# voletiv/mcvd-pytorch

Hardware: AMD Instinct MI355X
Metric: sampled frames/sec (whole node), SMMNIST 64x64 DDPM 100-step (higher is better)
Workload: dtype f32-equivalent: f32 storage and accumulation; 58 of 58 3x3 convs, 41 of 41 1x1 convs and the attention products (head dims 32..128) as SIX bf16 piece products of operands split EXACTLY into three bf16 pieces (all 24 bits, fp32 exponent range, less than one fp32 rounding per product; tests/test_gpu_p

## Files before the change

### include/mcvd_hip.h

```cpp
#ifndef MCVD_HIP_H
#define MCVD_HIP_H

#include <stddef.h>
#include <stdint.h>

#ifdef __cplusplus
extern "C" {
#endif

#define MCVD_OK 0
#define MCVD_EINVAL (-1)
#define MCVD_EHIP (-2)
#define MCVD_ESTATE (-3)
#define MCVD_ENOMEM (-4)
#define MCVD_ERANGE (-5)

#define MCVD_MAX_LEVELS 8

typedef struct mcvd_ctx mcvd_ctx;
typedef struct mcvd_model mcvd_model;

typedef struct mcvd_unet_desc {
    int32_t image_size;
    int32_t channels;
// ... 63 lines not shown
int mcvd_model_set_gamma_tables(mcvd_model* m, const float* k_cum_host, const float* theta_t_host, int n);
int mcvd_model_prepare_cond(mcvd_model* m, const float* cond, int B);
int mcvd_model_invalidate_cond(mcvd_model* m);
int mcvd_model_get_tuning(mcvd_model* m, int B, int* shapes, int* cots, int cap);
int mcvd_model_set_tuning(mcvd_model* m, int B, const int* shapes, const int* cots, int n);
int mcvd_model_graph_stats(mcvd_model* m, int64_t* captures, int64_t* replays);
int mcvd_model_num_launches(mcvd_model* m, int B);

int mcvd_model_profile_read(mcvd_model* m, int* kinds, int* ks, double* ms, double* flops, double* bytes, int cap);

int mcvd_model_op_info(mcvd_model* m, int i, int info[8]);

int mcvd_model_op_kernel(mcvd_model* m, int i);

long mcvd_model_fused_launches(mcvd_model* m, int what);

int mcvd_model_module_output(mcvd_model* m, int module, int B, float* dst_device, int64_t capacity, int* C, int* H);

int mcvd_sampler_run(mcvd_model* m, int kind, float* x_inout, const float* cond, const float* noise, uint64_t seed,
                     uint64_t sample_offset, int subsample_steps, int flags, double t_min, int B);
int mcvd_fpndm_run(mcvd_model* m, float* x_inout, const float* cond, int subsample_steps, int flags, int B);
int mcvd_sampler_update(mcvd_ctx* ctx, int kind, float* x_inout, const float* eps, const float* noise, float c_x0a,
                        float c_x0b, float c_mean0, float c_mean1, float c_noise, int clip, int64_t n);
int mcvd_randn(mcvd_ctx* ctx, float* out, uint64_t seed, uint64_t sample_offset, uint64_t draw, int B,
               int64_t per_sample);
int mcvd_pack_frames_u8(mcvd_ctx* ctx, const float* frames01, uint8_t* out, int B, int T, int C, int H, int W);
#define MCVD_METRIC_ROUND_BINARY 1
int mcvd_frame_metrics(mcvd_ctx* ctx, const float* pred01, const float* real01, int B, int T, int C, int H, int W, int flags, float* mse_out,
                       double* ssim_out, uint8_t* grey_out);
#define MCVD_F32 0
#define MCVD_F64 1
int mcvd_fvd_clips(mcvd_ctx* ctx, const float* const* parts, const int* part_frames, const int64_t* part_batch_stride, int nparts, int B, int C,
                   int H, int W, int row_start, int row_step, float* out);
int mcvd_feature_stats(mcvd_ctx* ctx, const void* feats, int dtype, int64_t N, int d, int64_t ld, int64_t row_start, int64_t row_step,
                       double* mean_out, double* sigma_out);
int mcvd_knn_radii(mcvd_ctx* ctx, const void* feats, int dtype, int64_t N, int d, int64_t ld, int k, double* radii2_out);
int mcvd_manifold_hits(mcvd_ctx* ctx, const void* query, int q_dtype, int64_t Nq, int64_t ldq, const void* ref, int r_dtype, int64_t Nr,
                       int64_t ldr, int d, const double* ref_radii2, uint8_t* hit_out);
int mcvd_knn_search(mcvd_ctx* ctx, const void* query, int q_dtype, int64_t ldq, const void* query2, int q2_dtype, int64_t ldq2, int64_t Nq,
                    const void* ref, int r_dtype, int64_t ldr, int64_t Nr, int d, int k, int64_t index_base, int merge, double* dist2_io,
                    int64_t* index_io);
int mcvd_hflip_u8(mcvd_ctx* ctx, const float* images01, float* out, int64_t n, int C, int H, int W);
int mcvd_nn_collect(mcvd_ctx* ctx, const float* held, const int64_t* held_index, const int64_t* new_index, const float* piece, int64_t n,
                    int64_t index_base, int64_t Nq, int k, int C, int H, int W, float* out);
typedef struct mcvd_lpips mcvd_lpips;
int mcvd_lpips_create(mcvd_ctx* ctx, mcvd_lpips** out);
void mcvd_lpips_destroy(mcvd_lpips* net);
int mcvd_lpips_set_param(mcvd_lpips* net, const char* name, const void* ptr, const int64_t* shape, int ndim, int on_device);
int mcvd_lpips_finalize(mcvd_lpips* net);
int mcvd_lpips_frames(mcvd_lpips* net, const float* pred01, const float* real01, int B, int T, int C, int H, int W, float* lpips_out,
                      uint8_t* resized_out, float* per_tap_out);
typedef struct mcvd_inception mcvd_inception;
int mcvd_inception_create(mcvd_ctx* ctx, mcvd_inception** out);
void mcvd_inception_destroy(mcvd_inception* net);
int mcvd_inception_set_param(mcvd_inception* net, const char* name, const void* ptr, const int64_t* shape, int ndim, int on_device);
int mcvd_inception_finalize(mcvd_inception* net);
int mcvd_inception_chunk(void);
int mcvd_inception_forward(mcvd_inception* net, const float* images01, int64_t n, int H, int W, int resize_input, int normalize_input,
                           int block_mask, float* out0, float* out1, float* out2, float* out3);
#define MCVD_DSM_L1 1
#define MCVD_DSM_GAMMA 2
int mcvd_dsm_loss(mcvd_model* m, const float* x, const int64_t* labels, const float* cond, const int32_t* cond_mask, const float* z,
                  uint64_t seed, uint64_t sample_offset, int flags, float* loss_rows, float* z_out, float* perturbed_out, int B);
int mcvd_gamma_noise(mcvd_ctx* ctx, float* out, const float* raw, float k, float theta, float kt, float sd, uint64_t seed,
                     uint64_t sample_offset, uint64_t draw, int B, int64_t per_sample);
int mcvd_lincomb(mcvd_ctx* ctx, float* out, const float* in0, const float* in1, const float* in2, const float* in3, float w0,
                 float w1, float w2, float w3, float scale, int nin, int64_t n);
int mcvd_pndm_transfer(mcvd_ctx* ctx, float* out, const float* x, const float* e, float d, float c1, float c2, int clip,
                       int64_t n);

int mcvd_upfirdn2d(mcvd_ctx* ctx, const float* in, const float* kernel_host, int kh, int kw, int up, int down, int pad0,
                   int pad1, float* out, int N, int C, int H, int W);
int mcvd_op_conv2d(mcvd_ctx* ctx, const float* x0, int C0, const float* x1, int C1, const float* w, const float* bias,
                   int Cout, int ks, const float* coef, int act, const float* res, float out_scale, float* y, int B, int H,
                   int W);
int mcvd_op_conv2d_strided(mcvd_ctx* ctx, const float* x, const float* w, const float* bias, int B, int Cin, int H, int W, int Cout, int ks,
                           int stride, int pad, int relu, float* y);
int mcvd_op_conv2d_rect(mcvd_ctx* ctx, const float* x, const float* w, const float* alpha, const float* beta, int B, int Cin, int H, int W,
                        int Cout, int kh, int kw, int stride, int pad_h, int pad_w, int relu, float* y, int c0, int Ctot);
int mcvd_op_pool3(mcvd_ctx* ctx, const float* x, float* y, int64_t NC, int H, int W, int mode);
int mcvd_op_global_avg(mcvd_ctx* ctx, const float* x, float* y, int64_t NC, int HW);
int mcvd_op_resize299(mcvd_ctx* ctx, const float* x, int64_t n, int H, int W, int normalize, float* y);
int mcvd_last_conv_kernel(void);
int mcvd_ctx_set_spade_inputs(mcvd_ctx* ctx, const float* gb, const float* coef2);
int mcvd_ctx_set_stats_buffer(mcvd_ctx* ctx, float* device_floats);
int mcvd_last_conv_stats_np(void);
int mcvd_op_gn_finalize(mcvd_ctx* ctx, const float* st0, int C0, int np0, const float* st1, int C1, int np1, int groups, float eps,
                        int mode, const float* p0, const float* p1, int emb_stride, int emb_off, float* coef_out, int B, int HW);
int mcvd_op_gn_coef(mcvd_ctx* ctx, const float* x0, int C0, const float* x1, int C1, int groups, float eps, int mode,
                    const float* p0, const float* p1, int emb_stride, int emb_off, float* coef_out, int B, int HW);
int mcvd_op_attention(mcvd_ctx* ctx, const float* qkv, float* out, int B, int C, int heads, int HW);
int mcvd_op_fir2(mcvd_ctx* ctx, const float* x, const float* coef, int act, int up, float* y, int B, int C, int H, int W);

#ifdef __cplusplus
}
#endif
#endif
```

### mcvd_pytorch_amd/_lib.py

```python
import ctypes as C
import os

import torch

_HERE = os.path.dirname(os.path.abspath(__file__))
LIB_PATH = os.environ.get("MCVD_LIB_PATH") or os.path.join(_HERE, "libmcvd_hip.so")

MAX_LEVELS = 8


class UNetDesc(C.Structure):
    _fields_ = [("image_size", C.c_int32), ("channels", C.c_int32), ("num_frames", C.c_int32),
                ("num_frames_cond", C.c_int32), ("ngf", C.c_int32), ("n_levels", C.c_int32),
                ("ch_mult", C.c_int32 * MAX_LEVELS), ("num_res_blocks", C.c_int32), ("n_attn", C.c_int32),
                ("attn_resolutions", C.c_int32 * MAX_LEVELS), ("n_head_channels", C.c_int32), ("spade", C.c_int32),
                ("spade_dim", C.c_int32), ("num_classes", C.c_int32), ("sigma_dist", C.c_int32),
                ("sigma_begin", C.c_float), ("sigma_end", C.c_float), ("cond_emb", C.c_int32), ("noise_in_cond", C.c_int32),
                ("gamma", C.c_int32)]


SAMPLER_DDPM, SAMPLER_DDIM = 0, 1
FLAG_DENOISE, FLAG_CLIP_BEFORE, FLAG_JUST_BETA, FLAG_GAMMA = 1, 2, 4, 8
METRIC_ROUND_BINARY = 1
DSM_L1, DSM_GAMMA = 1, 2
F32, F64 = 0, 1

_vp, _i, _f, _i64, _u64 = C.c_void_p, C.c_int, C.c_float, C.c_int64, C.c_uint64
_PROTOS = {
    "mcvd_version": (C.c_char_p, []),
    "mcvd_last_error": (C.c_char_p, [_vp]),
    "mcvd_ctx_create": (_i, [_i, _vp, C.POINTER(_vp)]),
    "mcvd_ctx_destroy": (None, [_vp]),
    "mcvd_ctx_device_shared": (_i, [_vp]),
    "mcvd_ctx_set_stream": (_i, [_vp, _vp]),
    "mcvd_ctx_set_option": (_i, [_vp, C.c_char_p, _i]),
    "mcvd_ctx_check_range": (_i, [_vp]),
    "mcvd_ctx_clear_range": (_i, [_vp]),
    "mcvd_ctx_selftest": (_i, [_vp]),
    "mcvd_ctx_set_debug_buffer": (_i, [_vp, _vp]),
    "mcvd_model_create": (_i, [_vp, C.POINTER(UNetDesc), C.POINTER(_vp)]),
    "mcvd_model_destroy": (None, [_vp]),
    "mcvd_model_num_params": (_i, [_vp]),
    "mcvd_model_param_info": (_i, [_vp, _i, C.POINTER(C.c_char_p), C.POINTER(_i64), C.POINTER(_i), C.POINTER(_i64)]),
    "mcvd_model_set_param": (_i, [_vp, C.c_char_p, _vp, C.POINTER(_i64), _i, _i]),
    "mcvd_model_blob_floats": (_i, [_vp, C.POINTER(_i64)]),
    "mcvd_model_export_blob": (_i, [_vp, _vp]),
    "mcvd_model_import_blob": (_i, [_vp, _vp]),
    "mcvd_model_broadcast_params": (_i, [_vp, _vp, _i]),
    "mcvd_model_finalize": (_i, [_vp]),
    "mcvd_model_get_schedule": (_i, [_vp, _vp, _vp, _vp, _i]),
    "mcvd_model_set_schedule": (_i, [_vp, _vp, _vp, _vp, _i]),
    "mcvd_model_set_temb_freqs": (_i, [_vp, _vp, _i]),
    "mcvd_unet_forward": (_i, [_vp, _vp, _vp, _vp, _vp, _i]),
    "mcvd_unet_forward_ft": (_i, [_vp, _vp, _vp, _vp, _vp, _i]),
    "mcvd_unet_forward_masked": (_i, [_vp, _vp, _vp, _vp, _vp, _vp, _i]),
    "mcvd_model_set_cond_noise": (_i, [_vp, _vp, _u64, _u64, _u64]),
    "mcvd_model_set_gamma_tables": (_i, [_vp, _vp, _vp, _i]),
    "mcvd_model_prepare_cond": (_i, [_vp, _vp, _i]),
    "mcvd_model_invalidate_cond": (_i, [_vp]),
    "mcvd_model_num_launches": (_i, [_vp, _i]),
    "mcvd_model_get_tuning": (_i, [_vp, _i, _vp, _vp, _i]),
    "mcvd_model_set_tuning": (_i, [_vp, _i, _vp, _vp, _i]),
    "mcvd_model_graph_stats": (_i, [_vp, C.POINTER(_i64), C.POINTER(_i64)]),
    "mcvd_last_conv_kernel": (_i, []),
    "mcvd_last_conv_stats_np": (_i, []),
    "mcvd_ctx_set_stats_buffer": (_i, [_vp, _vp]),
    "mcvd_ctx_set_spade_inputs": (_i, [_vp, _vp, _vp]),
    "mcvd_op_gn_finalize": (_i, [_vp, _vp, _i, _i, _vp, _i, _i, _i, _f, _i, _vp, _vp, _i, _i, _vp, _i, _i]),
    "mcvd_model_profile_read": (_i, [_vp, _vp, _vp, _vp, _vp, _vp, _i]),
    "mcvd_model_op_info": (_i, [_vp, _i, C.POINTER(_i)]),
    "mcvd_model_op_kernel": (_i, [_vp, _i]),
    "mcvd_model_fused_launches": (C.c_long, [_vp, _i]),
    "mcvd_model_module_output": (_i, [_vp, _i, _i, _vp, _i64, C.POINTER(_i), C.POINTER(_i)]),
    "mcvd_sampler_run": (_i, [_vp, _i, _vp, _vp, _vp, _u64, _u64, _i, _i, C.c_double, _i]),
    "mcvd_fpndm_run": (_i, [_vp, _vp, _vp, _i, _i, _i]),
    "mcvd_sampler_update": (_i, [_vp, _i, _vp, _vp, _vp, _f, _f, _f, _f, _f, _i, _i64]),
    "mcvd_randn": (_i, [_vp, _vp, _u64, _u64, _u64, _i, _i64]),
    "mcvd_pack_frames_u8": (_i, [_vp, _vp, _vp, _i, _i, _i, _i, _i]),
    "mcvd_frame_metrics": (_i, [_vp, _vp, _vp, _i, _i, _i, _i, _i, _i, _vp, _vp, _vp]),
    "mcvd_lpips_create": (_i, [_vp, C.POINTER(_vp)]),
    "mcvd_lpips_destroy": (None, [_vp]),
    "mcvd_lpips_set_param": (_i, [_vp, C.c_char_p, _vp, C.POINTER(_i64), _i, _i]),
    "mcvd_lpips_finalize": (_i, [_vp]),
    "mcvd_lpips_frames": (_i, [_vp, _vp, _vp, _i, _i, _i, _i, _i, _vp, _vp, _vp]),
    "mcvd_inception_create": (_i, [_vp, C.POINTER(_vp)]),
    "mcvd_inception_destroy": (None, [_vp]),
    "mcvd_inception_set_param": (_i, [_vp, C.c_char_p, _vp, C.POINTER(_i64), _i, _i]),
    "mcvd_inception_finalize": (_i, [_vp]),
    "mcvd_inception_chunk": (_i, []),
    "mcvd_inception_forward": (_i, [_vp, _vp, _i64, _i, _i, _i, _i, _i, _vp, _vp, _vp, _vp]),
    "mcvd_op_conv2d_rect": (_i, [_vp, _vp, _vp, _vp, _vp, _i, _i, _i, _i, _i, _i, _i, _i, _i, _i, _i, _vp, _i, _i]),
    "mcvd_op_pool3": (_i, [_vp, _vp, _vp, _i64, _i, _i, _i]),
    "mcvd_op_global_avg": (_i, [_vp, _vp, _vp, _i64, _i]),
    "mcvd_op_resize299": (_i, [_vp, _vp, _i64, _i, _i, _i, _vp]),
    "mcvd_fvd_clips": (_i, [_vp, C.POINTER(_vp), C.POINTER(_i), C.POINTER(_i64), _i, _i, _i, _i, _i, _i, _i, _vp]),
    "mcvd_feature_stats": (_i, [_vp, _vp, _i, _i64, _i, _i64, _i64, _i64, _vp, _vp]),
    "mcvd_knn_radii": (_i, [_vp, _vp, _i, _i64, _i, _i64, _i, _vp]),
    "mcvd_manifold_hits": (_i, [_vp, _vp, _i, _i64, _i64, _vp, _i, _i64, _i64, _i, _vp, _vp]),
    "mcvd_knn_search": (_i, [_vp, _vp, _i, _i64, _vp, _i, _i64, _i64, _vp, _i, _i64, _i64, _i, _i, _i64, _i, _vp, _vp]),
    "mcvd_hflip_u8": (_i, [_vp, _vp, _vp, _i64, _i, _i, _i]),
    "mcvd_nn_collect": (_i, [_vp, _vp, _vp, _vp, _vp, _i64, _i64, _i64, _i, _i, _i, _i, _vp]),
    "mcvd_op_conv2d_strided": (_i, [_vp, _vp, _vp, _vp, _i, _i, _i, _i, _i, _i, _i, _i, _i, _vp]),
    "mcvd_gamma_noise": (_i, [_vp, _vp, _vp, _f, _f, _f, _f, _u64, _u64, _u64, _i, _i64]),
    "mcvd_dsm_loss": (_i, [_vp, _vp, _vp, _vp, _vp, _vp, _u64, _u64, _i, _vp, _vp, _vp, _i]),
    "mcvd_lincomb": (_i, [_vp, _vp, _vp, _vp, _vp, _vp, _f, _f, _f, _f, _f, _i, _i64]),
    "mcvd_pndm_transfer": (_i, [_vp, _vp, _vp, _vp, _f, _f, _f, _i, _i64]),
    "mcvd_upfirdn2d": (_i, [_vp, _vp, _vp, _i, _i, _i, _i, _i, _i, _vp, _i, _i, _i, _i]),
    "mcvd_op_conv2d": (_i, [_vp, _vp, _i, _vp, _i, _vp, _vp, _i, _i, _vp, _i, _vp, _f, _vp, _i, _i, _i]),
    "mcvd_op_gn_coef": (_i, [_vp, _vp, _i, _vp, _i, _i, _f, _i, _vp, _vp, _i, _i, _vp, _i, _i]),
    "mcvd_op_attention": (_i, [_vp, _vp, _vp, _i, _i, _i, _i]),
    "mcvd_op_fir2": (_i, [_vp, _vp, _vp, _i, _i, _vp, _i, _i, _i, _i]),
}

EXPORTS = tuple(_PROTOS.keys())


def _load():
    if not os.path.exists(LIB_PATH):
        raise ImportError(
            f"{LIB_PATH} not found: the HIP extension is not built. Run `python mcvd_pytorch_amd/csrc/build.py` "
            "(needs hipcc; cross-compiles for gfx950 without a GPU). There is no CPU fallback.")
    lib = C.CDLL(LIB_PATH)
    for name, (res, args) in _PROTOS.items():
        fn = getattr(lib, name)
        fn.restype = res
        fn.argtypes = args
    return lib


lib = _load()


def last_error():
    return (lib.mcvd_last_error(None) or b"").decode()


def check(rc, what=""):
    if rc != 0:
        raise RuntimeError(f"libmcvd_hip: {what} failed (code {rc}): {last_error()}")
```

### mcvd_pytorch_amd/csrc/api.cpp

```cpp
#include <dlfcn.h>
#include <errno.h>
#include <fcntl.h>
#include <pthread.h>
#include <math.h>
#include <sys/file.h>
#include <sys/stat.h>
#include <unistd.h>
#include <stdio.h>
#include <stdlib.h>
#include <string.h>

#include <algorithm>
#include <cmath>
#include <mutex>
#include <new>
#include <vector>

#include "model.h"
#include "conv_kernels.h"
#include "inception.h"
#include "lpips.h"

using namespace mcvd;

// ... 263 lines not shown
        unsigned long long* dbg;
        explicit Saved(mcvd_ctx* c_) : c(c_), conv_shape(c_->conv_shape), naive_conv(c_->naive_conv), f16x2(c_->f16x2), f16x1(c_->f16x1), bf16x3(c_->bf16x3),
                                       spade_fuse(c_->spade_fuse), stats_buf(c_->stats_buf), spade_gb(c_->spade_gb), spade_coef2(c_->spade_coef2),
                                       dbg(c_->dbg) {
            c->naive_conv = 0; c->f16x2 = 0; c->f16x1 = 0; c->bf16x3 = 1; c->spade_fuse = 0;
            c->stats_buf = nullptr; c->spade_gb = nullptr; c->spade_coef2 = nullptr; c->dbg = nullptr;
        }
        ~Saved() {
            c->conv_shape = conv_shape; c->naive_conv = naive_conv; c->f16x2 = f16x2; c->f16x1 = f16x1; c->spade_fuse = spade_fuse;
            if (c->wino_selftest >= 0) c->bf16x3 = bf16x3;
            c->stats_buf = stats_buf; c->spade_gb = spade_gb; c->spade_coef2 = spade_coef2; c->dbg = dbg;
        }
    };
    const int shapes[3] = {CK_WINO, CK_WINO3, CK_WINO3P};
    int rc = 0, ran[3] = {-1, -1, -1};
    std::vector<float> out(3 * ny);
    {
        Saved saved(ctx);
        for (int k = 0; k < 3 && rc == 0; ++k) {
            ctx->conv_shape = shapes[k];
            rc = mcvd_op_conv2d(ctx, x, Cin, nullptr, 0, w, bias, Cout, 3, coef, 1, res, 0.70710678f, y + k * ny, B, H, H);
            ran[k] = last_conv_kernel();
        }
    }
    if (rc) return rc;
    MCVD_HIP_CHECK(hipMemcpyAsync(out.data(), y, 3 * ny * sizeof(float), hipMemcpyDeviceToHost, ctx->stream));
    MCVD_HIP_CHECK(hipStreamSynchronize(ctx->stream));
    float scale = 0.0f, d10 = 0.0f;
    size_t diff16 = 0;
    for (size_t i = 0; i < ny; ++i) {
        scale = std::max(scale, std::fabs(out[i]));
        d10 = std::max(d10, std::fabs(out[ny + i] - out[i]));
        diff16 += memcmp(&out[2 * ny + i], &out[ny + i], sizeof(float)) != 0;
    }
    const bool ok = ran[0] == shapes[0] && ran[1] == shapes[1] && ran[2] == shapes[2] && scale > 0.1f && d10 <= 1e-4f * scale && diff16 == 0 && std::isfinite(d10);
    if (ok) { ctx->wino_selftest = 1; return 0; }
    ctx->wino_selftest = -1;
    ctx->bf16x3 = 0;
    ++ctx->epoch;
    set_error("self-test of the hand-scheduled Winograd kernels FAILED on this device (kernels that ran: %d %d %d; |bf16x3 - fp32 MFMA| = %.3e at "
              "scale %.3e; %zu values of the persistent form differ from the per-item form): the option bf16x3 was switched off for this context",
              ran[0], ran[1], ran[2], (double)d10, (double)scale, diff16);
    return MCVD_ESELFTEST;
    API_CATCH
}

int mcvd_ctx_clear_range(mcvd_ctx* ctx) {
    API_TRY
    MCVD_REQUIRE(ctx, "ctx is NULL");
    if (ctx->range_flag) MCVD_HIP_CHECK(hipMemsetAsync(ctx->range_flag, 0, sizeof(int), ctx->stream));
    return 0;
    API_CATCH
}

int mcvd_ctx_set_option(mcvd_ctx* ctx, const char* key, int value) {
    MCVD_REQUIRE(ctx && key, "ctx/key is NULL");
    ++ctx->epoch;
    if (!strcmp(key, "naive_conv")) ctx->naive_conv = value;
    else if (!strcmp(key, "naive_attn")) ctx->naive_attn = value;
    else if (!strcmp(key, "fir_form")) ctx->fir_form = value;
    else if (!strcmp(key, "dbg_skip_finalize")) ctx->dbg_skip_finalize = value;
    else if (!strcmp(key, "gn_producer")) ctx->gn_producer = value;
    else if (!strcmp(key, "graph")) ctx->graph = value;
    else if (!strcmp(key, "conv_shape")) ctx->conv_shape = value;
    else if (!strcmp(key, "conv_shape1")) ctx->conv_shape1 = value;
    else if (!strcmp(key, "profile")) ctx->profile = value;
    else if (!strcmp(key, "conv_wdma")) ctx->conv_wdma = value;
    else if (!strcmp(key, "autotune")) ctx->autotune = value;
    else if (!strcmp(key, "side_stream")) ctx->side_stream = value;
    else if (!strcmp(key, "share_fence")) ctx->share_fence = value;
    else if (!strcmp(key, "winograd")) ctx->winograd = value;
    else if (!strcmp(key, "conv_dma1")) ctx->conv_dma1 = value;
    else if (!strcmp(key, "bf16x3")) ctx->bf16x3 = value;
    else if (!strcmp(key, "f16x2")) {
        if (ctx->f16x2 != value) (void)mcvd_ctx_clear_range(ctx);
        ctx->f16x2 = value;
    }
    else if (!strcmp(key, "f16x1")) {
        if (ctx->f16x1 != value) (void)mcvd_ctx_clear_range(ctx);
        ctx->f16x1 = value;
    }
    else if (!strcmp(key, "conv_cot")) ctx->conv_cot = value;
    else if (!strcmp(key, "persist_grid")) ctx->persist_grid = value;
    else if (!strcmp(key, "temb_table")) ctx->temb_table = value;
    else if (!strcmp(key, "im2col_lds")) ctx->im2col_lds = value;
    else if (!strcmp(key, "gn_stats")) ctx->gn_stats = value;
    else if (!strcmp(key, "spade_fuse")) ctx->spade_fuse = value;
    else if (!strcmp(key, "attn_presplit")) ctx->attn_presplit = value;
    else {
        set_error("unknown option '%s'", key);
        return MCVD_EINVAL;
    }
    return 0;
}

static void default_schedule(mcvd_model* m) {
    const int T = m->d.num_classes;
    m->betas.assign(T, 0.f);
    m->alphas.assign(T, 0.f);
    m->alphas_prev.assign(T, 0.f);
    if (m->d.sigma_dist == 0) {
        const float start = m->d.sigma_begin, end = m->d.sigma_end;
        const float step = (end - start) / (float)(T - 1);
        for (int i = 0; i < T; ++i) m->betas[i] = (i < T / 2) ? start + step * (float)i : end - step * (float)(T - 1 - i);
        float p = 1.0f;
        for (int i = T - 1; i >= 0; --i) {
            p = p * (1.0f - m->betas[i]);
            m->alphas[i] = p;
        }
        for (int i = 0; i < T; ++i) m->alphas_prev[i] = (i + 1 < T) ? m->alphas[i + 1] : 1.0f;
    } else {
        std::vector<float> f(T + 1);
        const float s = 0.008f;
        for (int i = 0; i <= T; ++i) {
            const float t = (float)(T - i) / (float)T;
            const float c = cosf((t + s) / (1.0f + s) * (float)(M_PI / 2));
            f[i] = c * c;
        }
        for (int i = 0; i < T; ++i) m->alphas[i] = f[i] / f[T];
        for (int i = 0; i < T; ++i) m->alphas_prev[i] = (i + 1 < T) ? m->alphas[i + 1] : 1.0f;
        for (int i = 0; i < T; ++i) m->betas[i] = 1.0f - m->alphas[i] / m->alphas_prev[i];
    }
    const int half = m->d.ngf / 2;
    m->freqs.assign(half, 0.f);
    const float e = (float)(-(log(10000.0) / (double)(half - 1)));
    for (int k = 0; k < half; ++k) m->freqs[k] = expf((float)k * e);
}

int mcvd_model_create(mcvd_ctx* ctx, const mcvd_unet_desc* desc, mcvd_model** out) {
    API_TRY
    MCVD_REQUIRE(desc && out, "model_create: NULL argument");
    MCVD_REQUIRE(desc->sigma_dist == 0 || desc->sigma_dist == 1, "desc: sigma_dist=%d", desc->sigma_dist);
    mcvd_model* m = new mcvd_model();
    m->ctx = ctx;
    m->d = *desc;
    if (m->build_plan()) {
        delete m;
        return MCVD_EINVAL;
    }
    default_schedule(m);
    if (ctx) {
        hipError_t e = hipMalloc((void**)&m->blob, (size_t)m->blob_floats * sizeof(float));
        if (e != hipSuccess) {
            set_error("hipMalloc(param blob, %lld floats): %s", (long long)m->blob_floats, hipGetErrorString(e));
            delete m;
            return MCVD_EHIP;
        }
        MCVD_HIP_CHECK(hipMemsetAsync(m->blob, 0, (size_t)m->blob_floats * sizeof(float), ctx->stream));
    }
    *out = m;
    return 0;
    API_CATCH
}

void mcvd_model_destroy(mcvd_model* m) {
    if (!m) return;
    if (m->ctx) (void)hipStreamSynchronize(m->ctx->stream);
    m->drop_graph();
    if (m->blob) (void)hipFree(m->blob);
    if (m->packed) (void)hipFree(m->packed);
    if (m->packed_h) (void)hipFree(m->packed_h);
    if (m->coef2_desc_dev) (void)hipFree(m->coef2_desc_dev);
    if (m->arena) (void)hipFree(m->arena);
    if (m->labels) (void)hipFree(m->labels);
    if (m->eps_buf) (void)hipFree(m->eps_buf);
    if (m->ksplit_buf) (void)hipFree(m->ksplit_buf);
// ... 898 lines not shown
    if (gam) {
        if (!m->gamma_dev) MCVD_HIP_CHECK(hipMalloc((void**)&m->gamma_dev, (size_t)2 * T * sizeof(float)));
        if (!m->gamma_dev_valid) {
            MCVD_HIP_CHECK(hipMemcpyAsync(m->gamma_dev, m->k_cum.data(), (size_t)T * sizeof(float), hipMemcpyHostToDevice, s));
            MCVD_HIP_CHECK(hipMemcpyAsync(m->gamma_dev + T, m->theta_t.data(), (size_t)T * sizeof(float), hipMemcpyHostToDevice, s));
            m->gamma_dev_valid = true;
        }
    }
    if (int rc = launch_dsm_perturb(x, z, labels, m->alphas_dev, gam ? m->gamma_dev : nullptr, gam ? m->gamma_dev + T : nullptr, T,
                                    gam ? 1 : 0, seed, sample_offset, B, per, zb, pb, s))
        return rc;
    struct MaskGuard { mcvd_model* m; ~MaskGuard() { m->cond_mask = nullptr; } } mask_guard{m};
    m->cond_mask = cond_mask;
    if (int rc = m->forward(pb, labels, cond, m->eps_buf, B)) return rc;
    if (int rc = launch_dsm_loss(zb, m->eps_buf, B, per, (flags & MCVD_DSM_L1) ? 1 : 0, part, loss_rows, s)) return rc;
    return (m->ctx->f16x2 || m->ctx->f16x1) ? mcvd_ctx_check_range(m->ctx) : 0;
    API_CATCH
}

int mcvd_gamma_noise(mcvd_ctx* ctx, float* out, const float* raw, float k, float theta, float kt, float sd, uint64_t seed,
                     uint64_t sample_offset, uint64_t draw, int B, int64_t per_sample) {
    MCVD_REQUIRE(ctx && out, "gamma_noise: NULL argument");
    return launch_gamma_noise(out, raw, k, theta, kt, sd, seed, sample_offset, draw, B, per_sample, ctx->stream);
}

int mcvd_randn(mcvd_ctx* ctx, float* out, uint64_t seed, uint64_t sample_offset, uint64_t draw, int B, int64_t per_sample) {
    MCVD_REQUIRE(ctx && out, "randn: NULL argument");
    return launch_randn(out, seed, sample_offset, draw, B, per_sample, ctx->stream);
}

int mcvd_upfirdn2d(mcvd_ctx* ctx, const float* in, const float* kernel_host, int kh, int kw, int up, int down, int pad0,
                   int pad1, float* out, int N, int C, int H, int W) {
    API_TRY
    MCVD_REQUIRE(ctx && in && kernel_host && out, "upfirdn2d: NULL argument");
    MCVD_REQUIRE(up >= 1 && down >= 1 && kh >= 1 && kw >= 1, "upfirdn2d: up/down/kernel");
    const int oh = (H * up + pad0 + pad1 - kh) / down + 1, ow = (W * up + pad0 + pad1 - kw) / down + 1;
    MCVD_REQUIRE(oh > 0 && ow > 0, "upfirdn2d: empty output");
    if (int rc = ctx->ensure_scratch((size_t)kh * kw * sizeof(float))) return rc;
    MCVD_HIP_CHECK(hipMemcpyAsync(ctx->scratch, kernel_host, (size_t)kh * kw * sizeof(float), hipMemcpyHostToDevice, ctx->stream));
    MCVD_HIP_CHECK(hipStreamSynchronize(ctx->stream));
    return launch_upfirdn2d(in, ctx->scratch, kh, kw, up, down, pad0, pad1, out, N * C, H, W, oh, ow, ctx->stream);
    API_CATCH
}

int mcvd_op_conv2d(mcvd_ctx* ctx, const float* x0, int C0, const float* x1, int C1, const float* w, const float* bias,
                   int Cout, int ks, const float* coef, int act, const float* res, float out_scale, float* y, int B, int H,
                   int W) {
    API_TRY
    MCVD_REQUIRE(ctx && x0 && w && bias && y, "op_conv2d: NULL argument");
    MCVD_REQUIRE(ks == 1 || ks == 3, "op_conv2d: ks=%d", ks);
    ConvArgs a{};
    a.x0 = x0; a.x1 = x1; a.C0 = C0; a.C1 = x1 ? C1 : 0;
    a.coef = coef; a.act = act; a.res = res; a.out_scale = out_scale; a.y = y;
    a.B = B; a.Cin = a.C0 + a.C1; a.Cout = Cout; a.H = H; a.W = W; a.ks = ks;
    a.cot = conv_cout_tile(Cout);
    a.CinP = round_up(a.Cin, conv_chunk(ks));
    a.CoutP = round_up(Cout, 32 * a.cot);
    const size_t wfloats = (size_t)a.CinP * ks * ks * a.CoutP;
    const ConvKernelDesc& k = conv_kernel(ctx->conv_shape);
    const bool wino = is_winograd(k.id) && conv_wino_supported(ks, H, W);
    const bool wino_h = wino && k.weights == CW_WPH;
    const bool wino_b = wino && k.weights == CW_WPB;
    const int np1 = (ks == 1 && k.family == CF_SPLIT1) ? k.pieces : 0;
    const size_t ufloats = wino ? (size_t)a.CinP * 16 * a.CoutP : 0;
    const size_t hfloats = wino_h ? (size_t)((conv_wino2h_weight_floats(a.CinP, a.CoutP) + 3) / 4 * 4)
                           : wino_b ? (size_t)((conv_wino3_weight_floats(a.CinP, a.CoutP) + 3) / 4 * 4)
                           : np1 ? (size_t)((conv1x1_h2_weight_floats(a.CinP, a.CoutP, np1) + 3) / 4 * 4) : 0;
    const size_t pfloats = wino ? (size_t)k.kparts * B * Cout * H * W : 0;
    if (int rc = ctx->ensure_scratch((wfloats + a.CoutP + ufloats + hfloats + pfloats) * sizeof(float))) return rc;
    MCVD_HIP_CHECK(hipMemsetAsync(ctx->scratch, 0, (wfloats + a.CoutP + ufloats + hfloats) * sizeof(float), ctx->stream));
    if (wino) {
        if (int rc = launch_pack_wino_weight(w, ctx->scratch + wfloats + a.CoutP, Cout, a.Cin, a.CinP, a.CoutP, ctx->stream)) return rc;
        a.wpw = ctx->scratch + wfloats + a.CoutP;
        if (wino_h) {
            if (int rc = launch_pack_wino2h_weight(w, ctx->scratch + wfloats + a.CoutP + ufloats, Cout, a.Cin, a.CinP, a.CoutP, ctx->stream)) return rc;
            a.wph = ctx->scratch + wfloats + a.CoutP + ufloats;
        }
        if (wino_b) {
            if (int rc = launch_pack_wino3_weight(w, ctx->scratch + wfloats + a.CoutP + ufloats, Cout, a.Cin, a.CinP, a.CoutP, ctx->stream)) return rc;
            a.wpb = ctx->scratch + wfloats + a.CoutP + ufloats;
        }
        if (pfloats) { a.part = ctx->scratch + wfloats + a.CoutP + ufloats + hfloats; a.part_floats = pfloats; }
    }
    if (int rc = launch_pack_conv_weight(w, ctx->scratch, Cout, a.Cin, ks, a.CinP, a.CoutP, 0, 0, ctx->stream)) return rc;
    if (np1) {
        if (int rc = launch_pack_conv1x1_h2(ctx->scratch, ctx->scratch + wfloats + a.CoutP, a.CinP, a.CoutP, ctx->stream, np1)) return rc;
        (np1 == 2 ? a.wph : a.wpb) = ctx->scratch + wfloats + a.CoutP;
    }
    MCVD_HIP_CHECK(hipMemcpyAsync(ctx->scratch + wfloats, bias, (size_t)Cout * sizeof(float), hipMemcpyDeviceToDevice, ctx->stream));
    a.wp = ctx->scratch;
    a.bias = ctx->scratch + wfloats;
    a.shape_hint = ctx->conv_shape;
    if (k.own_cot && ctx->conv_cot > 0) a.cot = ctx->conv_cot;
    a.wdma = ctx->conv_wdma;
    a.pgrid = ctx->persist_grid;
    a.dbg = ctx->dbg;
    a.stats = ctx->naive_conv ? nullptr : ctx->stats_buf;
    if (ctx->spade_gb) {
        MCVD_REQUIRE(wino && !ctx->naive_conv && coef && act, "op_conv2d: the SPADE prologue exists in the Winograd kernel only (conv_shape 4 / 8, "
                     "3x3, coef and act given)");
        a.gb = ctx->spade_gb;
        a.coef2 = ctx->spade_coef2;
        ConvArgs t = a;
        t.ksplit = k.family == CF_WINO ? k.kparts : 0;
        MCVD_REQUIRE(conv_wino_usable(t) || (t.ksplit = 0, conv_wino_usable(t)), "op_conv2d: shape not served by the Winograd kernel");
    }
    return ctx->naive_conv ? launch_conv_naive(a, ctx->stream) : launch_conv_mfma(a, ctx->stream);
    API_CATCH
}

int mcvd_last_conv_kernel(void) { return last_conv_kernel(); }

int mcvd_last_conv_stats_np(void) { return last_conv_stats_np(); }

int mcvd_op_gn_finalize(mcvd_ctx* ctx, const float* st0, int C0, int np0, const float* st1, int C1, int np1, int groups, float eps,
                        int mode, const float* p0, const float* p1, int emb_stride, int emb_off, float* coef_out, int B, int HW) {
    MCVD_REQUIRE(ctx && st0 && coef_out, "op_gn_finalize: NULL argument");
    GnArgs a{};
    a.C0 = C0; a.C1 = st1 ? C1 : 0; a.groups = groups; a.eps = eps; a.mode = mode; a.p0 = p0; a.p1 = p1;
    a.emb_stride = emb_stride; a.emb_off = emb_off; a.coef = coef_out; a.B = B; a.HW = HW;
    return launch_gn_finalize(a, st0, np0, st1, np1, ctx->stream);
}

int mcvd_model_graph_stats(mcvd_model* m, int64_t* captures, int64_t* replays) {
    MCVD_REQUIRE(m, "graph_stats: NULL model");
    if (captures) *captures = m->graph_captures;
    if (replays) *replays = m->graph_replays;
    return 0;
}

int mcvd_op_gn_coef(mcvd_ctx* ctx, const float* x0, int C0, const float* x1, int C1, int groups, float eps, int mode,
                    const float* p0, const float* p1, int emb_stride, int emb_off, float* coef_out, int B, int HW) {
    MCVD_REQUIRE(ctx && x0 && coef_out, "op_gn_coef: NULL argument");
    GnArgs a{};
    a.x0 = x0; a.x1 = x1; a.C0 = C0; a.C1 = x1 ? C1 : 0; a.groups = groups; a.eps = eps; a.mode = mode; a.p0 = p0; a.p1 = p1;
    a.emb_stride = emb_stride; a.emb_off = emb_off; a.coef = coef_out; a.B = B; a.HW = HW;
    return launch_gn_coef(a, ctx->stream);
}

int mcvd_op_attention(mcvd_ctx* ctx, const float* qkv, float* out, int B, int C, int heads, int HW) {
    MCVD_REQUIRE(ctx && qkv && out, "op_attention: NULL argument");
    const bool shared = ctx->share_fence && mcvd_ctx_shares_device(ctx);
    return launch_attention(ctx->naive_attn, shared ? 0 : ctx->f16x2, shared ? 0 : ctx->bf16x3, qkv, out, B, C, heads, HW, ctx->stream);
}

int mcvd_op_fir2(mcvd_ctx* ctx, const float* x, const float* coef, int act, int up, float* y, int B, int C, int H, int W) {
    MCVD_REQUIRE(ctx && x && y, "op_fir2: NULL argument");
    return launch_fir2(x, coef, act, up, y, B, C, H, W, nullptr, nullptr, nullptr, nullptr, ctx->stream, ctx->fir_form);
}

}
```

### mcvd_pytorch_amd/csrc/common.h

```cpp
#pragma once
#include <hip/hip_runtime.h>
#include <stdint.h>
#include <atomic>
#include <string>


namespace mcvd {

__device__ __forceinline__ float fma_unpacked(float x, float a, float b) {
    float r;
    asm("v_fma_f32 %0, %1, %2, %3" : "=v"(r) : "v"(x), "v"(a), "v"(b));
    return r;
}

void set_error(const char* fmt, ...);
const char* get_error();

#define MCVD_HIP_CHECK(expr)                                                                  \
    do {                                                                                      \
        hipError_t _e = (expr);                                                               \
        if (_e != hipSuccess) {                                                               \
            mcvd::set_error("%s failed: %s (%s:%d)", #expr, hipGetErrorString(_e), __FILE__, __LINE__); \
            return -2;                                                                        \
        }                                                                                     \
    } while (0)

#define MCVD_REQUIRE(cond, ...)            \
    do {                                   \
        if (!(cond)) {                     \
            mcvd::set_error(__VA_ARGS__);  \
            return -1;                     \
        }                                  \
    } while (0)

struct PerDeviceOnce {
    std::atomic<unsigned long long> mask{0};
    bool first_use() {
        int dev = 0;
        if (hipGetDevice(&dev) != hipSuccess || dev < 0 || dev >= 64) return true;
        const unsigned long long bit = 1ull << dev;
        return (mask.load(std::memory_order_acquire) & bit) == 0;
    }
    void done() {
        int dev = 0;
        if (hipGetDevice(&dev) == hipSuccess && dev >= 0 && dev < 64) mask.fetch_or(1ull << dev, std::memory_order_release);
    }
};

static inline int ceil_div(int a, int b) { return (a + b - 1) / b; }
static inline int round_up(int a, int b) { return ceil_div(a, b) * b; }

struct GnOut {
    float* coef;
    int groups;
    float eps;
    int mode;
    const float* p0;
    const float* p1;
    int emb_stride, emb_off;
};

struct ConvArgs {
    const float* x0;
    const float* x1;
    int C0, C1;
    const float* coef;
    int act;
    const float* wp;
    const float* wpw;
    const float* wph;
    const float* wpb;
    const float* bias;
    const float* res;
    float out_scale;
    float* y;
    int B, Cin, CinP, Cout, CoutP, H, W;
    int ks;
    int cot;
    int shape_hint;
    int ksplit;
    float* part;
    size_t part_floats;
    int wdma;
    int pgrid;
    unsigned long long* dbg;
    float* stats;
    const float* gb;
    const float* coef2;
    float* kv_img;
    int kv_C, kv_D;
    int im2col;
    GnOut gno;
};
int last_conv_gn_fused();
void set_last_conv_gn_fused(int v);
inline bool conv_part_fits(const ConvArgs& a) {
    return a.part != nullptr && (size_t)(a.ksplit < 2 ? 2 : a.ksplit) * a.B * a.Cout * a.H * a.W <= a.part_floats;
}
bool ksplit_reduce_gn_usable(const ConvArgs& a);
int launch_ksplit_reduce_gn(const ConvArgs& a, hipStream_t s);
bool conv1x1_h2_kv_supported(const ConvArgs& a, int cot);
void set_last_conv_stats_np(int np);
int last_conv_stats_np();
int conv_cout_tile(int Cout);
int conv_chunk(int ks);
int launch_conv_mfma(const ConvArgs& a, hipStream_t s);
int launch_conv_naive(const ConvArgs& a, hipStream_t s);
int last_conv_kernel();
bool conv_kernel_usable(int id, const ConvArgs& a);
int conv_kernel_launch(int id, const ConvArgs& a, hipStream_t s);
int launch_im2col3x3(const float* x0, int C0, const float* x1, int C1, float* col, int B, int H, int W, int K, hipStream_t s);
int launch_taps_shift_add(const float* z, const float* bias, const float* res, float scale, float* y, int B, int Cout, int H, int W, hipStream_t s);
int launch_pack_conv_gemm_form(const float* w, float* wp, int Cout, int Cin, int form, int CoutP, hipStream_t s);
bool conv_wino_supported(int ks, int H, int W);
int conv_wino_cout_tile(int Cout);
bool conv_wino_usable(const ConvArgs& a);
int launch_conv_wino(const ConvArgs& a, hipStream_t s);
int launch_wino_ksplit_reduce(const ConvArgs& a, hipStream_t s);
bool conv_wino3_usable(const ConvArgs& a);
int launch_conv_wino3(const ConvArgs& a, hipStream_t s);
long conv_wino3_weight_floats(int CinP, int CoutP);
bool conv_wino3p_usable(const ConvArgs& a);
int launch_conv_wino3p(const ConvArgs& a, hipStream_t s);
int launch_pack_wino3_weight(const float* w, float* wb, int Cout, int Cin, int CinP, int CoutP, hipStream_t s);
bool conv_wino2h_usable(const ConvArgs& a);
int launch_conv_wino2h(const ConvArgs& a, hipStream_t s);
long conv_wino2h_weight_floats(int CinP, int CoutP);
int launch_pack_wino2h_weight(const float* w, float* wh, int Cout, int Cin, int CinP, int CoutP, hipStream_t s);
bool conv_wino1h_usable(const ConvArgs& a);
int launch_conv_wino1h(const ConvArgs& a, hipStream_t s);
bool conv1x1_h2_supported(const ConvArgs& a, int cot, int np);
int launch_conv1x1_h2(const ConvArgs& a, int cot, hipStream_t s, int np);
long conv1x1_h2_weight_floats(int CinP, int CoutP, int np);
int launch_pack_conv1x1_h2(const float* wp, float* wh, int CinP, int CoutP, hipStream_t s, int np);
bool conv1x1_dma_supported(const ConvArgs& a, int ck, int pxw = 1);
int conv1x1_dma_cout_tile(int CoutP);
int launch_conv1x1_dma(const ConvArgs& a, int cot_req, int ck, hipStream_t s, int pxw = 1);
int launch_pack_wino_weight(const float* w, float* up, int Cout, int Cin, int CinP, int CoutP, hipStream_t s);
int launch_pack_conv_weight(const float* w, float* wp, int Cout, int Cin, int ks, int CinP, int CoutP, int nin,
                            int cout_off, hipStream_t s);

struct GnArgs {
    const float* x0;
    const float* x1;
    int C0, C1;
    int groups;
    float eps;
    int mode;
    const float* p0;
    const float* p1;
    int emb_stride, emb_off;
    float* coef;
    int B, HW;
};
int launch_gn_coef(const GnArgs& a, hipStream_t s);
int launch_gn_finalize(const GnArgs& a, const float* st0, int np0, const float* st1, int np1, hipStream_t s);

bool attention_mfma_supported(int C, int heads, int HW);
int launch_attention_mfma(const float* qkv, float* out, int B, int C, int heads, int HW, hipStream_t s);
int launch_attention_naive(const float* qkv, float* out, int B, int C, int heads, int HW, hipStream_t s);
bool attention_h2_supported(int C, int heads, int HW);
int launch_attention_h2(const float* qkv, float* out, int B, int C, int heads, int HW, hipStream_t s, int np);
bool attn_h2p_supported(int C, int heads, int HW);
int launch_attention_h2p(const float* qkv, const float* kv_img, float* out, int B, int C, int heads, int HW, hipStream_t s);
int launch_attention(int mode, int f16x2, int bf16x3, const float* qkv, float* out, int B, int C, int heads, int HW, hipStream_t s);

int launch_fir2(const float* x, const float* coef, int act, int up, float* y, int B, int C, int H, int W,
// ... 62 lines not shown
```

### mcvd_pytorch_amd/csrc/kernels/conv_wino3.cpp

```cpp
#include <stdlib.h>

#include "../common.h"

namespace mcvd {

typedef float f32x16 __attribute__((ext_vector_type(16)));
typedef float f32x4 __attribute__((ext_vector_type(4)));
typedef float f32x2 __attribute__((ext_vector_type(2)));
typedef __bf16 bf16x2 __attribute__((ext_vector_type(2)));
typedef unsigned u32x4 __attribute__((ext_vector_type(4)));

__device__ __forceinline__ float silu_w3(float v) { return v * __builtin_amdgcn_rcpf(1.0f + __expf(-v)); }

constexpr int W3_CK = 16;
constexpr int W3_T = 32;
constexpr int W3_NT = 512;
#ifndef MCVD_W3_PP
#define MCVD_W3_PP 24
#endif
constexpr int W3_PP = MCVD_W3_PP;
constexpr int W3_PW = 16 * 2 * 4 * W3_T;
constexpr int W3_VW = 3 * W3_PW;

__device__ __forceinline__ unsigned w3_cvt_pk(float lo, float hi) {
    const f32x2 v = {lo, hi};
    return __builtin_bit_cast(unsigned, __builtin_convertvector(v, bf16x2));
}
__device__ __forceinline__ void w3_split3(f32x2 v, unsigned& w1, unsigned& w2, unsigned& w3) {
    w1 = w3_cvt_pk(v.x, v.y);
    const f32x2 h = {__builtin_bit_cast(float, w1 << 16), __builtin_bit_cast(float, w1 & 0xffff0000u)};
    v = v - h;
    w2 = w3_cvt_pk(v.x, v.y);
    const f32x2 g = {__builtin_bit_cast(float, w2 << 16), __builtin_bit_cast(float, w2 & 0xffff0000u)};
    v = v - g;
    w3 = w3_cvt_pk(v.x, v.y);
}

template <int COT, int PRO, bool G8, int EXP = 0>
__global__ __launch_bounds__(512) __attribute__((amdgpu_num_vgpr(86))) void conv_wino3_kernel(ConvArgs a) {
    constexpr int NT = W3_NT, CK = W3_CK, T = W3_T, BCO = 32 * COT, PP = W3_PP, VW = W3_VW, PW = W3_PW;
    constexpr int PSZ = CK * 10 * PP;
    constexpr int PBUF = PSZ + 8;
    constexpr int NPL = G8 ? 1 : 3;
    constexpr int NPV = G8 ? 4 : 9;
    constexpr int NQ = 3 * COT;
    constexpr int NA = 2 * NQ;
    constexpr int VM_A = NQ + NPL;
    constexpr int PQ = 5;
    static_assert(NA <= 18 && NA > PQ, "named-register map below: v172-v180 patch, v184-v255 eighteen weight quads");
    extern __shared__ __attribute__((aligned(16))) float smem[];
    unsigned* sV = reinterpret_cast<unsigned*>(smem);
    float* sP = smem + 2 * VW;
    float* sCo = sP + 2 * PBUF;
    unsigned* sOff = reinterpret_cast<unsigned*>(sCo + (G8 ? 4 : 2) * a.Cin);

    {
        float top;
        asm volatile("" : "={v255}"(top));
    }
    asm volatile("" :: "s"(a.x0), "s"(a.x1), "s"(a.coef), "s"(a.wpb), "s"(a.B), "s"(a.H), "s"(a.W), "s"(a.Cin), "s"(a.CinP), "s"(a.C0),
                 "s"(a.C1), "s"(a.CoutP), "s"(a.ksplit), "s"(a.dbg), "s"(a.wdma));
    const unsigned long long t_start = a.dbg ? __builtin_amdgcn_s_memtime() : 0ull;
    const int tid = threadIdx.x, lane = tid & 63, wave = tid >> 6, l31 = lane & 31, half = lane >> 5;
    const int H = a.H, W = a.W, HW = H * W, Cin = a.Cin;
    const int rx_n = G8 ? 1 : W >> 4, ry_n = G8 ? 1 : H >> 3;
    const int nreg = G8 ? (a.B + 1) >> 1 : a.B * rx_n * ry_n;
    const int nct = a.CoutP / BCO;
    const int xcd = blockIdx.x & 7, slot = blockIdx.x >> 3;
    const int reg_id = (slot / nct) * 8 + xcd;
    const int cotile = slot - (slot / nct) * nct;
    if (reg_id >= nreg) return;
    const int b = G8 ? 2 * reg_id : reg_id / (rx_n * ry_n);
    const int rr = G8 ? 0 : reg_id - b * (rx_n * ry_n);
    const int oy0 = (rr / rx_n) * 8, ox0 = (rr % rx_n) * 16;
    const int co0 = cotile * BCO;
    const int rg = __builtin_amdgcn_readfirstlane(wave >> 2);

    const float* co_src[G8 ? 4 : 2];
#pragma unroll
    for (int k = 0; k < 2; ++k) {
        co_src[k] = a.coef + ((long)b * Cin + min(tid + k * NT, Cin - 1)) * 2;
        if (G8) co_src[2 + k] = a.coef + ((long)min(b + 1, a.B - 1) * Cin + min(tid + k * NT, Cin - 1)) * 2;
    }
    if (PRO) {
        asm volatile("global_load_dwordx2 v[172:173], %0, off\n\tglobal_load_dwordx2 v[174:175], %1, off"
                     :: "v"(co_src[0]), "v"(co_src[1]) : "memory");
        if constexpr (G8)
            asm volatile("global_load_dwordx2 v[176:177], %0, off\n\tglobal_load_dwordx2 v[178:179], %1, off"
                         :: "v"(co_src[2]), "v"(co_src[3]) : "memory");
    }

    const int s_tile = tid & 31, s_cp = (tid & 255) >> 5;
    const int s_ty = G8 ? (s_tile >> 2) & 3 : s_tile >> 3, s_tx = G8 ? (s_tile & 3) + 5 * (s_tile >> 4) : s_tile & 7;
    const int p_rd = ((s_cp * 10 + 2 * s_ty + rg) * PP + 2 * s_tx) * 2;
    const int v_wr = ((8 * rg * 2 + (s_cp & 1)) * 4 + (s_cp >> 1)) * T + s_tile;

    unsigned p_pk[NPL];
#pragma unroll
    for (int sl = 0; sl < NPL; ++sl) {
        p_pk[sl] = (unsigned)PSZ | ((unsigned)CK << 12);
        unsigned off = 0;
        if (G8) {
            const int e = tid, ci = e >> 5, img = (e >> 4) & 1, r = (e >> 1) & 7, c = (e & 1) * 4;
            const bool valid = b + img < a.B;
            const int cp = (ci >> 2) * 2 + (ci & 1), ce = (ci >> 1) & 1;
            p_pk[sl] = (unsigned)(((cp * 10 + r + 1) * PP + img * 10 + c + 1) * 2 + ce) | ((unsigned)(ci + (valid ? 0 : CK)) << 12) |
                       ((unsigned)(valid ? img : 0) << 20);
            off = (unsigned)(ci * HW + r * 8 + c) * 4u;
        } else if (sl < 2) {
            const int e = sl * NT + tid;
            if (e < CK * 40) {
                const int ci = e / 40, rem = e - ci * 40, r = rem >> 2, c = (rem & 3) * 4;
                const int y = oy0 - 1 + r;
                const bool inside = y >= 0 && y < H;
                const int cp = (ci >> 2) * 2 + (ci & 1), ce = (ci >> 1) & 1;
                p_pk[sl] = (unsigned)(((cp * 10 + r) * PP + c + 1) * 2 + ce) | ((unsigned)(ci + (inside ? 0 : CK)) << 12);
                off = (unsigned)(ci * HW + min(max(y, 0), H - 1) * W + ox0 + c) * 4u;
            }
        } else if (tid < CK * 20) {
            const int e = tid, ci = e / 20, rem = e - ci * 20, r = rem >> 1, c = (rem & 1) * 17;
            const int y = oy0 - 1 + r, x = ox0 - 1 + c;
            const bool inside = y >= 0 && y < H && x >= 0 && x < W;
            const int cp = (ci >> 2) * 2 + (ci & 1), ce = (ci >> 1) & 1;
            p_pk[sl] = (unsigned)(((cp * 10 + r) * PP + c) * 2 + ce) | ((unsigned)(ci + (inside ? 0 : CK)) << 12);
            off = (unsigned)(ci * HW + min(max(y, 0), H - 1) * W + min(max(x, 0), W - 1)) * 4u;
        }
        sOff[sl * NT + tid] = off;
    }

    const int wave_u = __builtin_amdgcn_readfirstlane(wave);
    const unsigned* wr_base = reinterpret_cast<const unsigned*>(a.wpb) + ((long)cotile * (a.CinP / CK) * 16 + 2 * wave_u) * (NQ * 256);
    const unsigned wr_voff = (unsigned)lane * 16u;

#define W3_QUADS(X, q, A1, A2) X(0, "v[184:187]", q, A1, A2) X(1, "v[188:191]", q, A1, A2) X(2, "v[192:195]", q, A1, A2) X(3, "v[196:199]", q, A1, A2) X(4, "v[200:203]", q, A1, A2) X(5, "v[204:207]", q, A1, A2) X(6, "v[208:211]", q, A1, A2) X(7, "v[212:215]", q, A1, A2) X(8, "v[216:219]", q, A1, A2) X(9, "v[220:223]", q, A1, A2) X(10, "v[224:227]", q, A1, A2) X(11, "v[228:231]", q, A1, A2) X(12, "v[232:235]", q, A1, A2) X(13, "v[236:239]", q, A1, A2) X(14, "v[240:243]", q, A1, A2) X(15, "v[244:247]", q, A1, A2) X(16, "v[248:251]", q, A1, A2) X(17, "v[252:255]", q, A1, A2)
#define W3_LD1(K, R, q, P, UNUSED) if ((q) == K) asm volatile("global_load_dwordx4 " R ", %0, %1" :: "v"(wr_voff), "s"(P) : "memory");
#define W3_MF1(K, R, q, ACC, BV) if ((q) == K) asm volatile("v_mfma_f32_32x32x16_bf16 %0, " R ", %1, %0" : "+v"(ACC) : "v"(BV));
#define W3_LOAD_A(ch, i)                                                                                        \
    {                                                                                                           \
        const unsigned* ua = wr_base + (long)(ch) * (16 * NQ * 256) + (i) * (NQ * 256);                         \
        _Pragma("unroll") for (int qq = 0; qq < NQ; ++qq) { W3_QUADS(W3_LD1, (i) * NQ + qq, ua + qq * 256, 0) } \
    }
                \
#define W3_LOAD_A_PIECE(ch, i, pc)                                                                              \
    {                                                                                                           \
        const unsigned* ua = wr_base + (long)(ch) * (16 * NQ * 256) + (i) * (NQ * 256);                         \
        _Pragma("unroll") for (int ct = 0; ct < COT; ++ct) { W3_QUADS(W3_LD1, (i) * NQ + ct * 3 + (pc), ua + (ct * 3 + (pc)) * 256, 0) } \
    }
#define W3_LD1D(K, R, q, P, DEP) if ((q) == K) asm volatile("global_load_dwordx4 " R ", %0, %1" :: "v"(wr_voff), "s"(P), "v"(DEP) : "memory");
#define W3_LOAD_A_RANGE(ch, Q0, Q1, DEP)                                                                        \
    {                                                                                                           \
        const unsigned* ua = wr_base + (long)(ch) * (16 * NQ * 256);                                            \
        _Pragma("unroll") for (int qq = (Q0); qq < (Q1); ++qq) { W3_QUADS(W3_LD1D, qq, ua + qq * 256, DEP) }    \
    }
#define W3_WAIT(N) asm volatile("s_waitcnt vmcnt(%1)\n\ts_mov_b32 %0, 0" : "=s"(vtok) : "n"(N) : "memory");
#define W3_READ_OFF(OFS) { _Pragma("unroll") for (int sl = 0; sl < NPL; ++sl) OFS[sl] = sOff[sl * NT + tid]; }
#define W3_LOAD_P(ch, DEP, OFS) W3_LOAD_PR(ch, DEP, OFS, "v[172:175]", "v[176:179]", "v180")
#define W3_LOAD_PR(ch, DEP, OFS, RA, RB, RH)                                                                    \
    {                                                                                                           \
        const int cb = min((ch) * CK, Cin - 1);                                                                 \
        const unsigned lim4 = (unsigned)((Cin - cb) * HW - 4) * 4u, lim1 = (unsigned)((Cin - cb) * HW - 1) * 4u; \
        const bool second = cb >= a.C0;                                                                         \
        const float* srcb = second ? a.x1 + ((long)b * a.C1 + (cb - a.C0)) * HW : a.x0 + ((long)b * a.C0 + cb) * HW; \
        const unsigned istride = (unsigned)((second ? a.C1 : a.C0) * HW) * 4u;       \
         \
        if constexpr (G8) {                                                                                     \
            const unsigned o0 = min(OFS[0], lim4) + ((p_pk[0] >> 20) & 1u) * istride;                           \
            asm volatile("global_load_dwordx4 " RA ", %0, %1" :: "v"(o0), "s"(srcb), "v"(DEP) : "memory");     \
        } else {                                                                                                \
            const unsigned o0 = min(OFS[0], lim4), o1 = min(OFS[NPL > 1 ? 1 : 0], lim4), o2 = min(OFS[NPL > 2 ? 2 : 0], lim1); \
            asm volatile("global_load_dwordx4 " RA ", %0, %3\n\tglobal_load_dwordx4 " RB ", %1, %3\n\tglobal_load_dword " RH ", %2, %3" \
                         :: "v"(o0), "v"(o1), "v"(o2), "s"(srcb), "v"(DEP) : "memory");                           \
        }                                                                                                       \
    }
                                                                    \
#define W3_READ_C(ch, cfv)                                                                                      \
    {                                                                                                           \
        _Pragma("unroll") for (int sl = 0; sl < NPL; ++sl) {                                                    \
            cfv[sl] = f32x2{1.0f, 0.0f};                                                                        \
            if (PRO >= 1) {                                                                                     \
                const int cch = min((ch) * CK + (int)((p_pk[sl] >> 12) & (CK - 1)), Cin - 1) + (G8 ? (int)((p_pk[sl] >> 20) & 1u) * Cin : 0); \
                cfv[sl] = *reinterpret_cast<const f32x2*>(sCo + cch * 2);                                       \
            }                                                                                                   \
        }                                                                                                       \
    }
#define W3_NOHOOK(e, v)
#define W3_WRITE_P(ch, PV, cfv) W3_WRITE_PR(ch, PV, cfv, "v172", "v173", "v174", "v175", "v176", "v177", "v178", "v179", "v180", W3_NOHOOK)
     \
#define W3_WRITE_PR(ch, PV, cfv, A0, A1, A2, A3, B0, B1, B2, B3, H0, HOOK)                                      \
    {                                                                                                           \
        float* sPw = sP + (((ch) & 1) ? PBUF : 0);                                                              \
        const int nvalid = Cin - (ch) * CK;                                                                     \
         \
        if constexpr (G8) {                                                                                     \
            asm("v_fma_f32 %0, " A0 ", %4, %5\n\tv_fma_f32 %1, " A1 ", %4, %5\n\tv_fma_f32 %2, " A2 ", %4, %5\n\tv_fma_f32 %3, " A3 ", %4, %5" \
                : "=&v"(PV[0]), "=&v"(PV[1]), "=&v"(PV[2]), "=&v"(PV[3]) : "v"(cfv[0].x), "v"(cfv[0].y), "s"(vtok)); \
        } else {                                                                                                \
            asm("v_fma_f32 %0, " A0 ", %9, %10\n\tv_fma_f32 %1, " A1 ", %9, %10\n\tv_fma_f32 %2, " A2 ", %9, %10\n\tv_fma_f32 %3, " A3 ", %9, %10\n\t" \
                "v_fma_f32 %4, " B0 ", %11, %12\n\tv_fma_f32 %5, " B1 ", %11, %12\n\tv_fma_f32 %6, " B2 ", %11, %12\n\tv_fma_f32 %7, " B3 ", %11, %12\n\t" \
                "v_fma_f32 %8, " H0 ", %13, %14"                                                                  \
                : "=&v"(PV[0]), "=&v"(PV[1]), "=&v"(PV[2]), "=&v"(PV[3]), "=&v"(PV[4]), "=&v"(PV[5]), "=&v"(PV[6]), "=&v"(PV[7]), "=&v"(PV[NPV > 8 ? 8 : 0]) \
                : "v"(cfv[0].x), "v"(cfv[0].y), "v"(cfv[NPL > 1 ? 1 : 0].x), "v"(cfv[NPL > 1 ? 1 : 0].y), "v"(cfv[NPL > 2 ? 2 : 0].x), \
                  "v"(cfv[NPL > 2 ? 2 : 0].y), "s"(vtok));                                                        \
        }                                                                                                       \
        _Pragma("unroll") for (int e = 0; e < NPV; ++e) {                                                       \
            const int sl = e >> 2;                               \
            float v = PV[e];                                                                                    \
            if (PRO >= 2) v = silu_w3(v);                                                                       \
            sPw[(p_pk[sl] & 0xfff) + 2 * (e & 3)] = ((int)((p_pk[sl] >> 12) & 0xff) < min(nvalid, CK)) ? v : 0.0f; \
            HOOK(e, v)                                                                                          \
        }                                                                                                       \
    }
          \
#define W3_READ_R(ch, RW)                                                                                       \
    {                                                                                                           \
        const f32x2* sPr = reinterpret_cast<const f32x2*>(sP + (((ch) & 1) ? PBUF : 0) + p_rd);                 \
        _Pragma("unroll") for (int j = 0; j < 4; ++j) { RW[0][j] = sPr[j]; RW[1][j] = sPr[PP + j]; RW[2][j] = sPr[2 * PP + j]; } \
    }
#define W3_WRITE_V(ch, RG, RW)                                                                                  \
    {                                                                                                           \
// ... 5 lines not shown
            else { mx[j] = r1 - r0; my[j] = r0 - r2; }                                                          \
        }                                                                                                       \
        _Pragma("unroll") for (int row = 0; row < 2; ++row) {                                                   \
            const f32x2 m0 = row ? my[0] : mx[0], m1 = row ? my[1] : mx[1], m2 = row ? my[2] : mx[2], m3 = row ? my[3] : mx[3]; \
            const f32x2 v0 = m0 - m2, v1 = m1 + m2, v2 = m2 - m1, v3 = m1 - m3;                                 \
            _Pragma("unroll") for (int q = 0; q < 4; ++q) {                                                     \
                unsigned w1, w2, w3;                                                                            \
                w3_split3(q == 0 ? v0 : q == 1 ? v1 : q == 2 ? v2 : v3, w1, w2, w3);                            \
                vdst[(row * 4 + q) * 256] = w1;                                                                 \
                vdst[(row * 4 + q) * 256 + PW] = w2;                                                            \
                vdst[(row * 4 + q) * 256 + 2 * PW] = w3;                                                        \
            }                                                                                                   \
        }                                                                                                       \
    }
#define W3_LOAD_B(i, BQ)                                                                                        \
    {                                                                                                           \
        const unsigned* q = sVc + (((2 * wave + (i)) * 2 + half) * 4) * T + l31;                                \
        _Pragma("unroll") for (int jp = 0; jp < 4; ++jp) {                                                      \
            BQ[0][jp] = q[jp * T]; BQ[1][jp] = q[PW + jp * T]; BQ[2][jp] = q[2 * PW + jp * T];                  \
        }                                                                                                       \
    }
#define W3_PRODUCT(i, PA, PB)                                                                                   \
    { _Pragma("unroll") for (int ct = 0; ct < COT; ++ct) { W3_QUADS(W3_MF1, 3 * ((i) * COT + ct) + (PA), acc[i][ct], bq[i][PB]) } }
          \
#define W3_MFMA_PHASE(ch, NEXT)                                                                                 \
    {                                                                                                           \
        const unsigned* sVc = sV + (((ch) & 1) ? VW : 0);                                                       \
        u32x4 bq[2][3];                                                                                         \
        W3_TS(7)                                                                                                \
        if (!(EXP & 8)) { W3_LOAD_B(0, bq[0]) W3_LOAD_B(1, bq[1]) }                                             \
        else { _Pragma("unroll") for (int p = 0; p < 3; ++p) { bq[0][p] = u32x4{1, 2, 3, 4}; bq[1][p] = u32x4{5, 6, 7, 8}; } } \
        _Pragma("unroll") for (int i = 0; i < 2; ++i) {                                                         \
            if (NEXT && !(EXP & 4)) W3_WAIT(VM_A)                                                               \
            if (!(EXP & 16)) {                                                                                  \
                 \
                W3_PRODUCT(i, 2, 0)                                                                             \
                if (NEXT && !(EXP & 4)) W3_LOAD_A_PIECE((ch) + 1, i, 2)                                         \
                W3_PRODUCT(i, 1, 1) W3_PRODUCT(i, 0, 2) W3_PRODUCT(i, 1, 0)                                     \
                if (NEXT && !(EXP & 4)) W3_LOAD_A_PIECE((ch) + 1, i, 1)                                         \
                W3_PRODUCT(i, 0, 1) W3_PRODUCT(i, 0, 0)                                                         \
                if (NEXT && !(EXP & 4)) W3_LOAD_A_PIECE((ch) + 1, i, 0)                                         \
            } else {                                                                                            \
                _Pragma("unroll") for (int ct = 0; ct < COT; ++ct)                                              \
                    acc[i][ct][0] += __builtin_bit_cast(float, bq[i][0][0] ^ bq[i][1][1] ^ bq[i][2][2] ^ bq[i][1][3]); \
                if (NEXT && !(EXP & 4)) W3_LOAD_A((ch) + 1, i)                                                  \
            }                                                                                                   \
            W3_TS(4 + i)                                                                                        \
        }                                                                                                       \
    }
                                                                                         \
#define W3_VALU_PHASE(ch, RG)                                                                                   \
    {                                                                                                           \
        {                                                                                                       \
            f32x2 cfv[NPL];                                                                                     \
            unsigned ofs[NPL];                                                                                  \
            W3_TS(7)                                                                                            \
            if (!(EXP & 2)) W3_READ_C((ch) + 2, cfv)                                                            \
            if (!(EXP & 4)) W3_READ_OFF(ofs)                                                                    \
            if (!(EXP & 4)) W3_WAIT(NA)                                                                         \
            W3_TS(0)                                                                                            \
            float pv[NPV];                                                                                      \
            _Pragma("unroll") for (int e = 0; e < NPV; ++e) pv[e] = 0.0f;                                       \
            if (!(EXP & 2)) W3_WRITE_P((ch) + 2, pv, cfv)                                                       \
            W3_TS(1)                                                                                            \
            if (!(EXP & 4)) W3_LOAD_P((ch) + 3, pv[0], ofs)                                                     \
            W3_TS(2)                                                                                            \
        }                                                                                                       \
        if (!(EXP & 1)) {                                                                                       \
            f32x2 rw[3][4];                                                                                     \
            W3_READ_R((ch) + 1, rw)                                                                             \
            W3_WRITE_V((ch) + 1, RG, rw)                                                                        \
        }                                                                                                       \
        W3_TS(3)                                                                                                \
    }

    f32x16 acc[2][COT];
#pragma unroll
    for (int i = 0; i < 2; ++i)
#pragma unroll
        for (int ct = 0; ct < COT; ++ct)
#pragma unroll
            for (int r = 0; r < 16; ++r) acc[i][ct][r] = 0.0f;

    const bool rec = a.dbg != nullptr && wave == (a.wdma & 7);
    const bool sub = (a.wdma & 64) != 0;
    unsigned long long sp[5] = {0, 0, 0, 0, 0};
    unsigned long long tk0 = 0, tprev = 0, dt[2] = {0, 0}, rt0 = 0;
    if (rec) {
        rt0 = __builtin_amdgcn_s_memrealtime();
        tk0 = tprev = t_start;
    }
#define W3_STAMP(i)                                                                                             \
    if (rec) {                                                                                                  \
        const unsigned long long now = __builtin_amdgcn_s_memtime();                                            \
        dt[i] += now - tprev;                                                                                   \
        tprev = now;                                                                                            \
    }
#ifdef MCVD_DIAG
    const bool tsub = rec && (a.wdma & 128) != 0;
    unsigned long long ts[8] = {0, 0, 0, 0, 0, 0, 0, 0}, tsp = 0;
#define W3_TS(i)                                                                                                \
    if (tsub) {                                                                                                 \
        const unsigned long long now = __builtin_amdgcn_s_memtime();                                            \
        ts[i] += now - tsp;                                                                                     \
        tsp = now;                                                                                              \
    }
#else
#define W3_TS(i)
#endif

    const int nch_all = a.CinP / CK;
    const int ksp = a.ksplit >= 2 ? a.ksplit : 1, kh = ksp >= 2 ? (int)blockIdx.y : 0;
    const int c_begin = kh * (nch_all / ksp), c_end = c_begin + nch_all / ksp;

    int vtok = 0;
    {
        const float nodep = 0.0f;
        unsigned ofs[NPL];
        W3_READ_OFF(ofs)
        if (rec) sp[3] = __builtin_amdgcn_s_memtime() - tk0;
        W3_LOAD_PR(c_begin, nodep, ofs, "v[184:187]", "v[188:191]", "v192")
        W3_LOAD_PR(c_begin + 1, nodep, ofs, "v[194:197]", "v[198:201]", "v202")
        if (G8)
            for (int i = tid; i < 2 * PBUF; i += NT) sP[i] = 0.0f;
        if (rec) sp[0] = __builtin_amdgcn_s_memtime() - tk0;
        W3_WAIT(0)
        if (rec) sp[1] = __builtin_amdgcn_s_memtime() - tk0;
        float cdep = 0.0f;
        if (PRO) {
            f32x2 cpre[G8 ? 4 : 2];
            asm volatile("v_mov_b32 %0, v172\n\tv_mov_b32 %1, v173\n\tv_mov_b32 %2, v174\n\tv_mov_b32 %3, v175"
                         : "=v"(cpre[0].x), "=v"(cpre[0].y), "=v"(cpre[1].x), "=v"(cpre[1].y) : "s"(vtok));
            if constexpr (G8)
                asm volatile("v_mov_b32 %0, v176\n\tv_mov_b32 %1, v177\n\tv_mov_b32 %2, v178\n\tv_mov_b32 %3, v179"
                             : "=v"(cpre[2].x), "=v"(cpre[2].y), "=v"(cpre[3].x), "=v"(cpre[3].y) : "s"(vtok));
#pragma unroll
            for (int k = 0; k < 2; ++k)
                if (tid + k * NT < Cin) {
                    *reinterpret_cast<f32x2*>(sCo + (tid + k * NT) * 2) = cpre[k];
                    if constexpr (G8) *reinterpret_cast<f32x2*>(sCo + (Cin + tid + k * NT) * 2) = cpre[2 + k];
                }
            cdep = cpre[0].x + cpre[1].x + (G8 ? cpre[2].x + cpre[3].x : 0.0f);
        }
        W3_LOAD_P(c_begin + 2, cdep, ofs)
        if (PRO || G8) __syncthreads();
        if (rec) sp[4] = __builtin_amdgcn_s_memtime() - tk0;
        {
            constexpr int QR = (NA - PQ + 2 * NPV - 1) / (2 * NPV);
#define W3_HOOK0(e, v) W3_LOAD_A_RANGE(c_begin, PQ + (e) * QR, (PQ + ((e) + 1) * QR < NA ? PQ + ((e) + 1) * QR : NA), v)
#define W3_HOOK1(e, v) W3_LOAD_A_RANGE(c_begin, (PQ + (NPV + (e)) * QR < NA ? PQ + (NPV + (e)) * QR : NA), (PQ + (NPV + (e) + 1) * QR < NA ? PQ + (NPV + (e) + 1) * QR : NA), v)
            float pv0[NPV], pv1[NPV];
            f32x2 cf0[NPL], cf1[NPL];
            W3_READ_C(c_begin, cf0)
            W3_READ_C(c_begin + 1, cf1)
            W3_WRITE_PR(c_begin, pv0, cf0, "v184", "v185", "v186", "v187", "v188", "v189", "v190", "v191", "v192", W3_HOOK0)
            W3_WRITE_PR(c_begin + 1, pv1, cf1, "v194", "v195", "v196", "v197", "v198", "v199", "v200", "v201", "v202", W3_HOOK1)
#undef W3_HOOK0
#undef W3_HOOK1
            const float dep = pv0[0] + pv1[0];
            W3_LOAD_A_RANGE(c_begin, 0, PQ, dep)
        }
    }
    __syncthreads();
    if (rec) sp[2] = __builtin_amdgcn_s_memtime() - tk0;
    {
        f32x2 rw[3][4];
        W3_READ_R(c_begin, rw)
        W3_WRITE_V(c_begin, rg, rw)
    }
    __syncthreads();
    W3_STAMP(0)

    W3_WAIT(0)
    const int ph = rg;
    if (ph == 0) {
        for (int c = c_begin; c + 1 < c_end; ++c) {
            W3_VALU_PHASE(c, rg)
            W3_MFMA_PHASE(c, true)
            asm volatile("s_waitcnt lgkmcnt(0)\n\ts_barrier" ::: "memory");
            W3_TS(6)
        }
    } else {
        for (int c = c_begin; c + 1 < c_end; ++c) {
            W3_MFMA_PHASE(c, true)
            W3_VALU_PHASE(c, rg)
            asm volatile("s_waitcnt lgkmcnt(0)\n\ts_barrier" ::: "memory");
            W3_TS(6)
        }
    }
    W3_WAIT(0)
    {
        const int c = c_end - 1;
        W3_MFMA_PHASE(c, false)
    }
    asm volatile("s_waitcnt vmcnt(0)" ::: "memory");
    if constexpr (COT == 3)
        asm volatile("s_nop 15\n\ts_nop 15" : "+v"(acc[0][0]), "+v"(acc[0][1]), "+v"(acc[0][2]), "+v"(acc[1][0]), "+v"(acc[1][1]), "+v"(acc[1][2]) :: "memory");
    else if constexpr (COT == 2)
        asm volatile("s_nop 15\n\ts_nop 15" : "+v"(acc[0][0]), "+v"(acc[0][1]), "+v"(acc[1][0]), "+v"(acc[1][1]) :: "memory");
    else
        asm volatile("s_nop 15\n\ts_nop 15" : "+v"(acc[0][0]), "+v"(acc[1][0]) :: "memory");

    float* sM = smem;
    const int e_tile = tid & 31, e_col0 = tid >> 5;
    const int e_ty = G8 ? (e_tile >> 2) & 3 : e_tile >> 3, e_tx = G8 ? e_tile & 3 : e_tile & 7;
    const int e_b = min(b + (G8 ? e_tile >> 4 : 0), a.B - 1);
    const bool e_valid = !G8 || b + (e_tile >> 4) < a.B;
    const long pix = (long)(oy0 + 2 * e_ty) * W + ox0 + 2 * e_tx;
    const bool fin = ksp == 1;
    float* const ydst = fin ? a.y : a.part + (long)kh * a.B * a.Cout * HW;
    float e_bias[COT][2];
    f32x2 e_r0[COT][2], e_r1[COT][2];
#pragma unroll
    for (int ct = 0; ct < COT; ++ct)
#pragma unroll
        for (int t2 = 0; t2 < 2; ++t2) {
            const int co = co0 + ct * 32 + e_col0 + 16 * t2;
            e_bias[ct][t2] = fin ? a.bias[co] : 0.0f;
            e_r0[ct][t2] = e_r1[ct][t2] = f32x2{0.0f, 0.0f};
            if (a.res && fin) {
                const long o = ((long)e_b * a.Cout + min(co, a.Cout - 1)) * HW + pix;
                e_r0[ct][t2] = *reinterpret_cast<const f32x2*>(a.res + o);
                e_r1[ct][t2] = *reinterpret_cast<const f32x2*>(a.res + o + W);
            }
        }
    asm volatile("s_waitcnt lgkmcnt(0)\n\ts_barrier" ::: "memory");
    W3_STAMP(1)
#pragma unroll
    for (int ct = 0; ct < COT; ++ct) {
#pragma unroll
        for (int i = 0; i < 2; ++i)
#pragma unroll
            for (int r = 0; r < 16; ++r) {
                const int col = (r & 3) + 8 * (r >> 2) + 4 * half;
                sM[((2 * wave + i) * 32 + col) * T + l31] = acc[i][ct][r];
            }
        asm volatile("s_waitcnt lgkmcnt(0)\n\ts_barrier" ::: "memory");
#pragma unroll
        for (int t2 = 0; t2 < 2; ++t2) {
            const int e_col = e_col0 + 16 * t2;
            const int co = co0 + ct * 32 + e_col;
            const f32x2 r0 = e_r0[ct][t2], r1 = e_r1[ct][t2];
            float mm[16];
#pragma unroll
            for (int xi = 0; xi < 16; ++xi) mm[xi] = sM[(xi * 32 + e_col) * T + e_tile];
            float t0[4], t1[4];
#pragma unroll
            for (int l = 0; l < 4; ++l) {
                t0[l] = mm[0 * 4 + l] + mm[1 * 4 + l] + mm[2 * 4 + l];
                t1[l] = mm[1 * 4 + l] - mm[2 * 4 + l] - mm[3 * 4 + l];
            }
            const float y00 = t0[0] + t0[1] + t0[2], y01 = t0[1] - t0[2] - t0[3];
            const float y10 = t1[0] + t1[1] + t1[2], y11 = t1[1] - t1[2] - t1[3];
            const float bvv = e_bias[ct][t2];
            const float osc = fin ? a.out_scale : 1.0f;
            const float v00 = (y00 + bvv + r0.x) * osc, v01 = (y01 + bvv + r0.y) * osc;
            const float v10 = (y10 + bvv + r1.x) * osc, v11 = (y11 + bvv + r1.y) * osc;
            if (co < a.Cout && e_valid) {
                const long o = ((long)e_b * a.Cout + co) * HW + pix;
                *reinterpret_cast<float2*>(ydst + o) = make_float2(v00, v01);
                *reinterpret_cast<float2*>(ydst + o + W) = make_float2(v10, v11);
            }
            if (a.stats && fin) {
                float pil;
                {
                    const int pv = __builtin_bit_cast(int, v00);
                    const int s0 = __builtin_amdgcn_readlane(pv, 0), s2 = __builtin_amdgcn_readlane(pv, 32);
                    if (G8) {
                        const int s1 = __builtin_amdgcn_readlane(pv, 16), s3 = __builtin_amdgcn_readlane(pv, 48);
                        pil = __builtin_bit_cast(float, (lane & 32) ? ((lane & 16) ? s3 : s2) : ((lane & 16) ? s1 : s0));
                    } else {
                        pil = __builtin_bit_cast(float, (lane & 32) ? s2 : s0);
                    }
                }
                const float d0 = v00 - pil, d1 = v01 - pil, d2 = v10 - pil, d3 = v11 - pil;
                float sm = (d0 + d1) + (d2 + d3);
                float qm = (d0 * d0 + d1 * d1) + (d2 * d2 + d3 * d3);
#define W3_MERGE(CTRL, ROWMASK)                                                                                     \
                {                                                                                                   \
                    sm += __builtin_bit_cast(float, __builtin_amdgcn_update_dpp(0, __builtin_bit_cast(int, sm), CTRL, ROWMASK, 0xf, false)); \
                    qm += __builtin_bit_cast(float, __builtin_amdgcn_update_dpp(0, __builtin_bit_cast(int, qm), CTRL, ROWMASK, 0xf, false)); \
                }
                W3_MERGE(0xB1, 0xf)
                W3_MERGE(0x4E, 0xf)
                W3_MERGE(0x124, 0xf)
                W3_MERGE(0x128, 0xf)
                if (!G8) W3_MERGE(0x142, 0xa)
#undef W3_MERGE
                const bool writer = G8 ? (e_tile & 15) == 0 : e_tile == 31;
                if (writer && co < a.Cout && e_valid) {
                    constexpr float NPIX = G8 ? 64.0f : 128.0f;
                    float* q = a.stats + (((long)e_b * a.Cout + co) * (rx_n * ry_n) + rr) * 2;
                    q[0] = sm + NPIX * pil;
                    q[1] = fmaxf(qm - sm * sm * (1.0f / NPIX), 0.0f);
                }
            }
        }
        if (ct + 1 < COT) asm volatile("s_waitcnt lgkmcnt(0)\n\ts_barrier" ::: "memory");
    }
    if (rec) {
        const unsigned long long now = __builtin_amdgcn_s_memtime();
        if (lane == 0) {
            unsigned long long* d = a.dbg + ((long)blockIdx.y * gridDim.x + blockIdx.x) * 8;
            unsigned hwid, xcc;
            asm volatile("s_getreg_b32 %0, hwreg(HW_REG_HW_ID)" : "=s"(hwid));
            asm volatile("s_getreg_b32 %0, hwreg(HW_REG_XCC_ID)" : "=s"(xcc));
            d[0] = dt[0]; d[1] = dt[1]; d[2] = rt0; d[3] = __builtin_amdgcn_s_memrealtime();
            d[4] = ((unsigned long long)xcc << 32) | hwid;
            d[5] = now - tprev;
            d[6] = (unsigned long long)(c_end - c_begin);
            d[7] = now - tk0;
            if (sub) { d[1] = sp[3]; d[2] = sp[0]; d[3] = sp[1]; d[4] = sp[4]; d[5] = sp[2]; }
#ifdef MCVD_DIAG
            if (tsub) { d[0] = ts[0]; d[1] = ts[1]; d[2] = ts[2]; d[3] = ts[3]; d[4] = ts[4]; d[5] = ts[5]; d[7] = ts[6]; }
#endif
        }
    }
#undef W3_STAMP
#undef W3_TS
#undef W3_LOAD_A
#undef W3_LOAD_A_PIECE
#undef W3_QUADS
#undef W3_LD1
#undef W3_MF1
#undef W3_PRODUCT
#undef W3_LOAD_P
#undef W3_LOAD_PR
#undef W3_WRITE_PR
#undef W3_LD1D
#undef W3_LOAD_A_RANGE
#undef W3_WAIT
#undef W3_WRITE_P
#undef W3_WRITE_V
#undef W3_READ_R
#undef W3_READ_C
#undef W3_READ_OFF
#undef W3_LOAD_B
#undef W3_MFMA_PHASE
#undef W3_VALU_PHASE
}

static size_t wino3_lds_bytes(int Cin, bool g8) {
    return (size_t)(2 * W3_VW + 2 * (W3_CK * 10 * W3_PP + 8) + (g8 ? 4 : 2) * Cin + (g8 ? 1 : 3) * W3_NT) * sizeof(float);
}

int launch_wino_ksplit_reduce(const ConvArgs& a, hipStream_t s);

template <int COT, int PRO, bool G8, int EXP>
static int wino3_launch_k(const ConvArgs& k, dim3 grid, size_t lds, hipStream_t s) {
    static PerDeviceOnce raised;
    if (raised.first_use()) {
        MCVD_HIP_CHECK(hipFuncSetAttribute(reinterpret_cast<const void*>(&conv_wino3_kernel<COT, PRO, G8, EXP>),
                                           hipFuncAttributeMaxDynamicSharedMemorySize, 160 * 1024));
        raised.done();
    }
    hipLaunchKernelGGL((conv_wino3_kernel<COT, PRO, G8, EXP>), grid, dim3(W3_NT), lds, s, k);
    return 0;
}

template <int COT, int PRO, bool G8>
static int wino3_launch2(const ConvArgs& a, hipStream_t s) {
    constexpr int BCO = 32 * COT;
    const size_t lds = wino3_lds_bytes(a.Cin, G8);
    const int nreg = G8 ? (a.B + 1) / 2 : a.B * (a.H / 8) * (a.W / 16);
    const int ksp = a.ksplit >= 2 ? a.ksplit : 1;
    dim3 grid(((nreg + 7) / 8) * 8 * (a.CoutP / BCO), ksp);
    ConvArgs k = a;
    int rc = 0;
    if (k.dbg) k.wdma = 0;
#ifdef MCVD_DIAG
    if (k.dbg) {
        const char* w = getenv("MCVD_DBG_WAVE");
        k.wdma = w ? atoi(w) : 0;
    }
    const char* exp_s = getenv("MCVD_WINO3_EXP");
    const int e = exp_s ? atoi(exp_s) : 0;
    if (COT == 3 && PRO == 2 && !G8 && e != 0) {
        switch (e) {
            case 1: rc = wino3_launch_k<3, 2, false, 1>(k, grid, lds, s); break;
            case 2: rc = wino3_launch_k<3, 2, false, 2>(k, grid, lds, s); break;
            case 3: rc = wino3_launch_k<3, 2, false, 3>(k, grid, lds, s); break;
            case 4: rc = wino3_launch_k<3, 2, false, 4>(k, grid, lds, s); break;
            case 16: rc = wino3_launch_k<3, 2, false, 16>(k, grid, lds, s); break;
            case 15: rc = wino3_launch_k<3, 2, false, 15>(k, grid, lds, s); break;
            case 27: rc = wino3_launch_k<3, 2, false, 27>(k, grid, lds, s); break;
            case 11: rc = wino3_launch_k<3, 2, false, 11>(k, grid, lds, s); break;
            default: mcvd::set_error("MCVD_WINO3_EXP=%d is not a built ablation", e); return -1;
        }
    } else
#endif
    {
        rc = wino3_launch_k<COT, PRO, G8, 0>(k, grid, lds, s);
    }
    if (rc) return rc;
    MCVD_HIP_CHECK(hipGetLastError());
    if (ksp >= 2) return launch_wino_ksplit_reduce(a, s);
    if (a.stats) set_last_conv_stats_np(G8 ? 1 : (a.H / 8) * (a.W / 16));
    return 0;
}

template <int COT, bool G8>
static int wino3_launch1(const ConvArgs& a, hipStream_t s) {
    if (!a.coef && !a.act) return wino3_launch2<COT, 0, G8>(a, s);
    if (!a.act) return wino3_launch2<COT, 1, G8>(a, s);
    return wino3_launch2<COT, 2, G8>(a, s);
}

template <int COT>
static int wino3_launch(const ConvArgs& a, hipStream_t s) {
    return (a.H == 8 && a.W == 8) ? wino3_launch1<COT, true>(a, s) : wino3_launch1<COT, false>(a, s);
}

bool conv_wino3_usable(const ConvArgs& a) {
    const bool g8 = a.H == 8 && a.W == 8;
    return a.ks == 3 && ((a.H % 8 == 0 && a.W % 16 == 0 && a.H >= 8 && a.W >= 16) || g8) && a.wpb && !a.gb && a.Cin <= 1024 &&
           a.CinP % W3_CK == 0 && (a.C1 == 0 || a.C0 % W3_CK == 0) && a.H * a.W <= 16384 &&
           (long)a.B * (a.C0 > a.C1 ? a.C0 : a.C1) * a.H * a.W < (1L << 29) && wino3_lds_bytes(a.Cin, g8) <= 160 * 1024 &&
           (a.ksplit < 2 || ((a.ksplit == 2 || a.ksplit == 4 || a.ksplit == 8) && (a.CinP / W3_CK) % a.ksplit == 0 &&
                             a.CinP / W3_CK >= 2 * a.ksplit && conv_part_fits(a)));
}

int launch_conv_wino3(const ConvArgs& a, hipStream_t s) {
    MCVD_REQUIRE(conv_wino3_usable(a), "winograd bf16x3 conv: unsupported (ks=%d H=%d W=%d Cin=%d C0=%d ksplit=%d, packed weight pieces %s)",
                 a.ks, a.H, a.W, a.Cin, a.C0, a.ksplit, a.wpb ? "present" : "missing");
    const int cot = conv_wino_cout_tile(a.Cout);
    MCVD_REQUIRE(a.CoutP % (32 * cot) == 0, "winograd bf16x3 conv: CoutP=%d vs tile %d", a.CoutP, 32 * cot);
    switch (cot) {
        case 1: return wino3_launch<1>(a, s);
        case 2: return wino3_launch<2>(a, s);
        default: return wino3_launch<3>(a, s);
    }
}

__device__ __forceinline__ unsigned short w3_bf16_rne(float v) {
    unsigned u = __float_as_uint(v);
    u += 0x7fffu + ((u >> 16) & 1u);
    return (unsigned short)(u >> 16);
}
__device__ __forceinline__ float w3_bf16_f32(unsigned short h) { return __uint_as_float((unsigned)h << 16); }

__global__ void pack_wino3_weight_kernel(const float* w, unsigned short* dst, int Cout, int Cin, int CinP, int CoutP, int COT) {
    const long n = (long)Cout * Cin;
    const int BCO = 32 * COT, nch = CinP / 16;
    for (long i = blockIdx.x * (long)blockDim.x + threadIdx.x; i < n; i += (long)gridDim.x * blockDim.x) {
        const int ci = (int)(i % Cin), co = (int)(i / Cin);
        const float* g = w + i * 9;
        float t[4][3];
#pragma unroll
        for (int j = 0; j < 3; ++j) {
            t[0][j] = g[0 * 3 + j];
            t[1][j] = 0.5f * (g[0 * 3 + j] + g[1 * 3 + j] + g[2 * 3 + j]);
            t[2][j] = 0.5f * (g[0 * 3 + j] - g[1 * 3 + j] + g[2 * 3 + j]);
            t[3][j] = g[2 * 3 + j];
        }
        const int cotile = co / BCO, ct = (co % BCO) / 32, cc = ci & 15, h = cc & 1, el = cc >> 1;
        const int lane = h * 32 + (co & 31);
        const long base = ((((long)cotile * nch + (ci >> 4)) * 16) * COT + ct) * 1536 + (lane * 4 + (el >> 1)) * 2 + (el & 1);
#pragma unroll
        for (int r = 0; r < 4; ++r) {
            float u[4];
            u[0] = t[r][0];
            u[1] = 0.5f * (t[r][0] + t[r][1] + t[r][2]);
            u[2] = 0.5f * (t[r][0] - t[r][1] + t[r][2]);
            u[3] = t[r][2];
#pragma unroll
            for (int c = 0; c < 4; ++c) {
                const unsigned short h1 = w3_bf16_rne(u[c]);
                const float r1 = u[c] - w3_bf16_f32(h1);
                const unsigned short h2 = w3_bf16_rne(r1);
                const float r2 = r1 - w3_bf16_f32(h2);
                const unsigned short h3 = w3_bf16_rne(r2);
                const long o = base + (long)(r * 4 + c) * COT * 1536;
                dst[o] = h1;
                dst[o + 512] = h2;
                dst[o + 1024] = h3;
// ... 20 lines not shown
```

### mcvd_pytorch_amd/csrc/kernels/conv_wino3p.cpp

```cpp
#include <stdlib.h>

#include "../common.h"

namespace mcvd {

typedef float f32x16 __attribute__((ext_vector_type(16)));
typedef float f32x4 __attribute__((ext_vector_type(4)));
typedef float f32x2 __attribute__((ext_vector_type(2)));
typedef __bf16 bf16x2 __attribute__((ext_vector_type(2)));
typedef unsigned u32x4 __attribute__((ext_vector_type(4)));

__device__ __forceinline__ float silu_w3p(float v) { return v * __builtin_amdgcn_rcpf(1.0f + __expf(-v)); }

constexpr int WP_CK = 16;
constexpr int WP_T = 32;
constexpr int WP_NT = 512;
#ifndef MCVD_W3_PP
#define MCVD_W3_PP 24
#endif
constexpr int WP_PP = MCVD_W3_PP;
constexpr int WP_PW = 16 * 2 * 4 * WP_T;
constexpr int WP_VW = 3 * WP_PW;
constexpr int WP_NPL = 3;
constexpr int WP_MINCH = 4;

__device__ __forceinline__ unsigned wp_cvt_pk(float lo, float hi) {
    const f32x2 v = {lo, hi};
    return __builtin_bit_cast(unsigned, __builtin_convertvector(v, bf16x2));
}
__device__ __forceinline__ void wp_split3(f32x2 v, unsigned& w1, unsigned& w2, unsigned& w3) {
    w1 = wp_cvt_pk(v.x, v.y);
    const f32x2 h = {__builtin_bit_cast(float, w1 << 16), __builtin_bit_cast(float, w1 & 0xffff0000u)};
    v = v - h;
    w2 = wp_cvt_pk(v.x, v.y);
    const f32x2 g = {__builtin_bit_cast(float, w2 << 16), __builtin_bit_cast(float, w2 & 0xffff0000u)};
    v = v - g;
    w3 = wp_cvt_pk(v.x, v.y);
}

template <int COT, int PRO>
__global__ __launch_bounds__(512) __attribute__((amdgpu_num_vgpr(86))) void conv_wino3p_kernel(ConvArgs a) {
    constexpr int NT = WP_NT, CK = WP_CK, T = WP_T, BCO = 32 * COT, PP = WP_PP, VW = WP_VW, PW = WP_PW;
    constexpr int PSZ = CK * 10 * PP;
    constexpr int PBUF = 4096;
    static_assert(PBUF >= PSZ + 8 && PBUF >= 4 * 32 * WP_T, "patch buffer: patch + dump space, and 4 positions x 32 couts x 32 tiles of the epilogue");
    constexpr int NPL = WP_NPL, NPV = 9;
    constexpr int NQ = 3 * COT;
    constexpr int NA = 2 * NQ;
    constexpr int VM_A = NQ + NPL;
    constexpr int PQ = 5;
    constexpr long WSTR = 16L * NQ * 256;
    static_assert(NA <= 18 && NA > PQ, "named-register map below: v172-v180 patch, v184-v255 eighteen weight quads");
    extern __shared__ __attribute__((aligned(16))) float smem[];
    unsigned* sV = reinterpret_cast<unsigned*>(smem);
    float* sP = smem + 2 * VW;
    float* sCo = sP + 2 * PBUF;
    unsigned* sOff = reinterpret_cast<unsigned*>(sCo + 2 * a.Cin);
    {
        float top;
        asm volatile("" : "={v255}"(top));
    }
    asm volatile("" :: "s"(a.x0), "s"(a.x1), "s"(a.coef), "s"(a.wpb), "s"(a.B), "s"(a.H), "s"(a.W), "s"(a.Cin), "s"(a.CinP), "s"(a.C0),
                 "s"(a.C1), "s"(a.CoutP), "s"(a.ksplit), "s"(a.dbg), "s"(a.wdma));
    const unsigned long long t_start = a.dbg ? __builtin_amdgcn_s_memtime() : 0ull;
    const int tid = threadIdx.x, lane = tid & 63, wave = tid >> 6, l31 = lane & 31, half = lane >> 5;
    const int H = a.H, W = a.W, HW = H * W, Cin = a.Cin;
    const int rx_n = W >> 4, rpi = rx_n * (H >> 3);
    const int nct = a.CoutP / BCO;
    const int ksp = a.ksplit >= 2 ? a.ksplit : 1;
    const int nch = (a.CinP / CK) / ksp;
    const int ips = rpi * nct * ksp;
    const int n_items = a.B * ips;
    const int it0 = (int)((long)blockIdx.x * n_items / gridDim.x), it1 = (int)((long)(blockIdx.x + 1) * n_items / gridDim.x);
    if (it0 >= it1) return;
    const int rg = __builtin_amdgcn_readfirstlane(wave >> 2);
    const int wave_u = __builtin_amdgcn_readfirstlane(wave);
#ifdef MCVD_DIAG
    if ((a.wdma >> 8) != 0 && (blockIdx.x & 1)) {
        const unsigned long long until = __builtin_amdgcn_s_memtime() + ((unsigned long long)(a.wdma >> 8) << 8);
        while (__builtin_amdgcn_s_memtime() < until) __builtin_amdgcn_s_sleep(8);
    }
#endif

    const int s_tile = tid & 31, s_cp = (tid & 255) >> 5;
    const int s_ty = s_tile >> 3, s_tx = s_tile & 7;
    const int p_rd = ((s_cp * 10 + 2 * s_ty + rg) * PP + 2 * s_tx) * 2;
    const int v_wr = ((8 * rg * 2 + (s_cp & 1)) * 4 + (s_cp >> 1)) * T + s_tile;

    unsigned p_pk[NPL];
#pragma unroll
    for (int sl = 0; sl < NPL; ++sl) {
        p_pk[sl] = (unsigned)PSZ | ((unsigned)CK << 12);
        if (sl < 2) {
            const int e = sl * NT + tid;
            if (e < CK * 40) {
                const int ci = e / 40, rem = e - ci * 40, r = rem >> 2, c = (rem & 3) * 4;
                const int cp = (ci >> 2) * 2 + (ci & 1), ce = (ci >> 1) & 1;
                p_pk[sl] = (unsigned)(((cp * 10 + r) * PP + c + 1) * 2 + ce) | ((unsigned)ci << 12);
            }
        } else if (tid < CK * 20) {
            const int e = tid, ci = e / 20, rem = e - ci * 20, r = rem >> 1, c = (rem & 1) * 17;
            const int cp = (ci >> 2) * 2 + (ci & 1), ce = (ci >> 1) & 1;
            p_pk[sl] = (unsigned)(((cp * 10 + r) * PP + c) * 2 + ce) | ((unsigned)ci << 12);
        }
    }
#define WP_SLOT_TABLE(tab, oy0, ox0, OUT)                                                                       \
    {                                                                                                           \
        int tid_s;        \
        asm volatile("v_mov_b32 %0, %1" : "=v"(tid_s) : "v"(tid));                                              \
        _Pragma("unroll") for (int sl = 0; sl < NPL; ++sl) {                                                    \
            unsigned off = 1u;                                                                                  \
            if (sl < 2) {                                                                                       \
                const int e = sl * NT + tid_s;                                                                  \
                if (e < CK * 40) {                                                                              \
                    const int ci = e / 40, rem = e - ci * 40, r = rem >> 2, c = (rem & 3) * 4;                  \
                    const int y = (oy0) - 1 + r;                                                                \
                    const bool inside = y >= 0 && y < H;                                                        \
                    off = (unsigned)(ci * HW + min(max(y, 0), H - 1) * W + (ox0) + c) * 4u + (inside ? 0u : 1u); \
                }                                                                                               \
            } else if (tid_s < CK * 20) {                                                                       \
                const int e = tid_s, ci = e / 20, rem = e - ci * 20, r = rem >> 1, c = (rem & 1) * 17;          \
                const int y = (oy0) - 1 + r, x = (ox0) - 1 + c;                                                 \
                const bool inside = y >= 0 && y < H && x >= 0 && x < W;                                         \
                off = (unsigned)(ci * HW + min(max(y, 0), H - 1) * W + min(max(x, 0), W - 1)) * 4u + (inside ? 0u : 1u); \
            }                                                                                                   \
            sOff[((tab) * NPL + sl) * NT + tid] = off;                                                          \
            OUT[sl] = off;                                                                                      \
        }                                                                                                       \
    }

    const unsigned wr_voff = (unsigned)lane * 16u;

#define WP_QUADS(X, q, A1, A2) X(0, "v[184:187]", q, A1, A2) X(1, "v[188:191]", q, A1, A2) X(2, "v[192:195]", q, A1, A2) X(3, "v[196:199]", q, A1, A2) X(4, "v[200:203]", q, A1, A2) X(5, "v[204:207]", q, A1, A2) X(6, "v[208:211]", q, A1, A2) X(7, "v[212:215]", q, A1, A2) X(8, "v[216:219]", q, A1, A2) X(9, "v[220:223]", q, A1, A2) X(10, "v[224:227]", q, A1, A2) X(11, "v[228:231]", q, A1, A2) X(12, "v[232:235]", q, A1, A2) X(13, "v[236:239]", q, A1, A2) X(14, "v[240:243]", q, A1, A2) X(15, "v[244:247]", q, A1, A2) X(16, "v[248:251]", q, A1, A2) X(17, "v[252:255]", q, A1, A2)
#define WP_LD1(K, R, q, P, UNUSED) if ((q) == K) asm volatile("global_load_dwordx4 " R ", %0, %1" :: "v"(wr_voff), "s"(P) : "memory");
#define WP_MF1(K, R, q, ACC, BV) if ((q) == K) asm volatile("v_mfma_f32_32x32x16_bf16 %0, " R ", %1, %0" : "+v"(ACC) : "v"(BV));
#define WP_LOAD_A_PIECE(WPTR, i, pc)                                                                            \
    {                                                                                                           \
        const unsigned* ua = (WPTR) + (i) * (NQ * 256);                                                         \
        _Pragma("unroll") for (int ct = 0; ct < COT; ++ct) { WP_QUADS(WP_LD1, (i) * NQ + ct * 3 + (pc), ua + (ct * 3 + (pc)) * 256, 0) } \
    }
#define WP_LD1D(K, R, q, P, DEP) if ((q) == K) asm volatile("global_load_dwordx4 " R ", %0, %1" :: "v"(wr_voff), "s"(P), "v"(DEP) : "memory");
#define WP_LOAD_A_RANGE(WPTR, Q0, Q1, DEP)                                                                      \
    {                                                                                                           \
        const unsigned* ua = (WPTR);                                                                            \
        _Pragma("unroll") for (int qq = (Q0); qq < (Q1); ++qq) { WP_QUADS(WP_LD1D, qq, ua + qq * 256, DEP) }    \
    }
#define WP_WAIT(N) asm volatile("s_waitcnt vmcnt(%1)\n\ts_mov_b32 %0, 0" : "=s"(vtok) : "n"(N) : "memory");
#define WP_LOAD_P(bb, ch, DEP, OFS) WP_LOAD_PR(bb, ch, DEP, OFS, "v[172:175]", "v[176:179]", "v180")
#define WP_LOAD_PR(bb, ch, DEP, OFS, RA, RB, RH)                                                                \
    {                                                                                                           \
        const int cb = min((ch) * CK, Cin - 1);                                                                 \
        const unsigned lim4 = (unsigned)((Cin - cb) * HW - 4) * 4u, lim1 = (unsigned)((Cin - cb) * HW - 1) * 4u; \
        const bool second = cb >= a.C0;                                                                         \
        const float* srcb = second ? a.x1 + ((long)(bb) * a.C1 + (cb - a.C0)) * HW : a.x0 + ((long)(bb) * a.C0 + cb) * HW; \
        const unsigned o0 = min(OFS[0] & ~3u, lim4), o1 = min(OFS[1] & ~3u, lim4), o2 = min(OFS[2] & ~3u, lim1); \
        asm volatile("global_load_dwordx4 " RA ", %0, %3\n\tglobal_load_dwordx4 " RB ", %1, %3\n\tglobal_load_dword " RH ", %2, %3" \
                     :: "v"(o0), "v"(o1), "v"(o2), "s"(srcb), "v"(DEP) : "memory");                               \
    }
#define WP_READ_C(ch, cfv)                                                                                      \
    {                                                                                                           \
        _Pragma("unroll") for (int sl = 0; sl < NPL; ++sl) {                                                    \
            cfv[sl] = f32x2{1.0f, 0.0f};                                                                        \
            if (PRO >= 1) {                                                                                     \
                const int cch = min((ch) * CK + (int)((p_pk[sl] >> 12) & (CK - 1)), Cin - 1);                   \
                cfv[sl] = *reinterpret_cast<const f32x2*>(sCo + cch * 2);                                       \
            }                                                                                                   \
        }                                                                                                       \
    }
#define WP_NOHOOK(e, v)
#define WP_WRITE_P(par, ch, FL, PV, cfv) WP_WRITE_PR(par, ch, FL, PV, cfv, "v172", "v173", "v174", "v175", "v176", "v177", "v178", "v179", "v180", WP_NOHOOK)
#define WP_WRITE_PR(par, ch, FL, PV, cfv, A0, A1, A2, A3, B0, B1, B2, B3, H0, HOOK)                             \
    {                                                                                                           \
        float* sPw = sP + ((par) ? PBUF : 0);                                                                   \
        const int nvalid = min(Cin - (ch) * CK, CK);                                                            \
        asm("v_fma_f32 %0, " A0 ", %9, %10\n\tv_fma_f32 %1, " A1 ", %9, %10\n\tv_fma_f32 %2, " A2 ", %9, %10\n\tv_fma_f32 %3, " A3 ", %9, %10\n\t" \
            "v_fma_f32 %4, " B0 ", %11, %12\n\tv_fma_f32 %5, " B1 ", %11, %12\n\tv_fma_f32 %6, " B2 ", %11, %12\n\tv_fma_f32 %7, " B3 ", %11, %12\n\t" \
            "v_fma_f32 %8, " H0 ", %13, %14"                                                                      \
            : "=&v"(PV[0]), "=&v"(PV[1]), "=&v"(PV[2]), "=&v"(PV[3]), "=&v"(PV[4]), "=&v"(PV[5]), "=&v"(PV[6]), "=&v"(PV[7]), "=&v"(PV[8]) \
            : "v"(cfv[0].x), "v"(cfv[0].y), "v"(cfv[1].x), "v"(cfv[1].y), "v"(cfv[2].x), "v"(cfv[2].y), "s"(vtok)); \
        _Pragma("unroll") for (int e = 0; e < NPV; ++e) {                                                       \
            const int sl = e >> 2;                               \
            float v = PV[e];                                                                                    \
            if (PRO >= 2) v = silu_w3p(v);                                                                      \
            const bool keep = (((FL) >> sl) & 1u) == 0u && (int)((p_pk[sl] >> 12) & 0xff) < nvalid;             \
            sPw[(p_pk[sl] & 0xfff) + 2 * (e & 3)] = keep ? v : 0.0f;                                            \
            HOOK(e, v)                                                                                          \
        }                                                                                                       \
    }
#define WP_READ_R(par, RW)                                                                                      \
    {                                                                                                           \
        const f32x2* sPr = reinterpret_cast<const f32x2*>(sP + ((par) ? PBUF : 0) + p_rd);                      \
        _Pragma("unroll") for (int j = 0; j < 4; ++j) { RW[0][j] = sPr[j]; RW[1][j] = sPr[PP + j]; RW[2][j] = sPr[2 * PP + j]; } \
    }
#define WP_WRITE_V(par, RG, RW)                                                                                 \
    {                                                                                                           \
        unsigned* vdst = sV + ((par) ? VW : 0) + v_wr;                                                          \
        f32x2 mx[4], my[4];                                                                                     \
        _Pragma("unroll") for (int j = 0; j < 4; ++j) {                                                         \
            const f32x2 r0 = RW[0][j], r1 = RW[1][j], r2 = RW[2][j];                                            \
            if ((RG) == 0) { mx[j] = r0 - r2; my[j] = r1 + r2; }                                                \
            else { mx[j] = r1 - r0; my[j] = r0 - r2; }                                                          \
        }                                                                                                       \
        _Pragma("unroll") for (int row = 0; row < 2; ++row) {                                                   \
            const f32x2 m0 = row ? my[0] : mx[0], m1 = row ? my[1] : mx[1], m2 = row ? my[2] : mx[2], m3 = row ? my[3] : mx[3]; \
            const f32x2 v0 = m0 - m2, v1 = m1 + m2, v2 = m2 - m1, v3 = m1 - m3;                                 \
            _Pragma("unroll") for (int q = 0; q < 4; ++q) {                                                     \
                unsigned w1, w2, w3;                                                                            \
                wp_split3(q == 0 ? v0 : q == 1 ? v1 : q == 2 ? v2 : v3, w1, w2, w3);                            \
                vdst[(row * 4 + q) * 256] = w1;                                                                 \
                vdst[(row * 4 + q) * 256 + PW] = w2;                                                            \
                vdst[(row * 4 + q) * 256 + 2 * PW] = w3;                                                        \
            }                                                                                                   \
        }                                                                                                       \
    }
#define WP_LOAD_B(i, BQ)                                                                                        \
    {                                                                                                           \
        const unsigned* q = sVc + (((2 * wave + (i)) * 2 + half) * 4) * T + l31;                                \
        _Pragma("unroll") for (int jp = 0; jp < 4; ++jp) {                                                      \
            BQ[0][jp] = q[jp * T]; BQ[1][jp] = q[PW + jp * T]; BQ[2][jp] = q[2 * PW + jp * T];                  \
        }                                                                                                       \
    }
#define WP_PRODUCT(i, PA, PB)                                                                                   \
    { _Pragma("unroll") for (int ct = 0; ct < COT; ++ct) { WP_QUADS(WP_MF1, 3 * ((i) * COT + ct) + (PA), acc[i][ct], bq[i][PB]) } }
#define WP_MFMA_PHASE(par, WNX)                                                                                 \
    {                                                                                                           \
        const unsigned* sVc = sV + ((par) ? VW : 0);                                                            \
        u32x4 bq[2][3];                                                                                         \
        WP_LOAD_B(0, bq[0]) WP_LOAD_B(1, bq[1])                                                                 \
        _Pragma("unroll") for (int i = 0; i < 2; ++i) {                                                         \
            WP_WAIT(VM_A)                                                                                       \
            WP_PRODUCT(i, 2, 0)                                                                                 \
            WP_LOAD_A_PIECE(WNX, i, 2)                                                                          \
            WP_PRODUCT(i, 1, 1) WP_PRODUCT(i, 0, 2) WP_PRODUCT(i, 1, 0)                                         \
            WP_LOAD_A_PIECE(WNX, i, 1)                                                                          \
            WP_PRODUCT(i, 0, 1) WP_PRODUCT(i, 0, 0)                                                             \
            WP_LOAD_A_PIECE(WNX, i, 0)                                                                          \
        }                                                                                                       \
    }
#define WP_VALU_PHASE(par, CH2, CH3, TAB3, RG)                                                                  \
    {                                                                                                           \
        {                                                                                                       \
            f32x2 cfv[NPL];                                                                                     \
            unsigned ofs[NPL];                                                                                  \
            WP_READ_C(CH2, cfv)                                                                                 \
            _Pragma("unroll") for (int sl = 0; sl < NPL; ++sl) ofs[sl] = sOff[((TAB3) * NPL + sl) * NT + tid];  \
            WP_WAIT(NA)                                                                                         \
            float pv[NPV];                                                                                      \
            _Pragma("unroll") for (int e = 0; e < NPV; ++e) pv[e] = 0.0f;                                       \
            WP_WRITE_P(par, CH2, pfl, pv, cfv)                                                                  \
            pfl = (ofs[0] & 1u) | ((ofs[1] & 1u) << 1) | ((ofs[2] & 1u) << 2);                                  \
            WP_LOAD_P(b, CH3, pv[0], ofs)                                                                       \
        }                                                                                                       \
        {                                                                                                       \
            f32x2 rw[3][4];                                                                                     \
            WP_READ_R((par) ^ 1, rw)                                                                            \
            WP_WRITE_V((par) ^ 1, RG, rw)                                                                       \
        }                                                                                                       \
    }

    f32x16 acc[2][COT];
#pragma unroll
    for (int i = 0; i < 2; ++i)
#pragma unroll
        for (int ct = 0; ct < COT; ++ct)
#pragma unroll
            for (int r = 0; r < 16; ++r) acc[i][ct][r] = 0.0f;

    const bool rec = a.dbg != nullptr && wave == (a.wdma & 7);
    unsigned long long tprev = t_start, dt[3] = {0, 0, 0}, rt0 = 0;
    if (rec) rt0 = __builtin_amdgcn_s_memrealtime();
#define WP_STAMP(i)                                                                                             \
    if (rec) {                                                                                                  \
        const unsigned long long now = __builtin_amdgcn_s_memtime();                                            \
        dt[i] += now - tprev;                                                                                   \
        tprev = now;                                                                                            \
    }

    const unsigned* const wpb_u = reinterpret_cast<const unsigned*>(a.wpb);
    const bool fin = ksp == 1;
    int vtok = 0;
    unsigned pfl = 0;
    int chunks_done = 0;

    int it = it0;
    while (it < it1) {
        const int b = it / ips;
        const int run_end = min(it1, (b + 1) * ips);
        {
            const int q0 = it - b * ips, kh = q0 % ksp, q1 = q0 / ksp, cotile = q1 % nct, rr = q1 / nct;
            const int oy0 = (rr / rx_n) * 8, ox0 = (rr % rx_n) * 16, cbeg = kh * nch;
            const unsigned* w0 = wpb_u + (((long)cotile * (nch * ksp) + cbeg) * 16 + 2 * wave_u) * (NQ * 256);
            const float* co_src[2];
#pragma unroll
            for (int k = 0; k < 2; ++k) co_src[k] = a.coef + ((long)b * Cin + min(tid + k * NT, Cin - 1)) * 2;
            if (PRO)
                asm volatile("global_load_dwordx2 v[172:173], %0, off\n\tglobal_load_dwordx2 v[174:175], %1, off"
                             :: "v"(co_src[0]), "v"(co_src[1]) : "memory");
            const float nodep = 0.0f;
            unsigned ofs[NPL];
            WP_SLOT_TABLE(it & 1, oy0, ox0, ofs)
            const unsigned fl0 = (ofs[0] & 1u) | ((ofs[1] & 1u) << 1) | ((ofs[2] & 1u) << 2);
            WP_LOAD_PR(b, cbeg, nodep, ofs, "v[184:187]", "v[188:191]", "v192")
            WP_LOAD_PR(b, cbeg + 1, nodep, ofs, "v[194:197]", "v[198:201]", "v202")
            WP_WAIT(0)
            float cdep = 0.0f;
            if (PRO) {
                f32x2 cpre[2];
                asm volatile("v_mov_b32 %0, v172\n\tv_mov_b32 %1, v173\n\tv_mov_b32 %2, v174\n\tv_mov_b32 %3, v175"
                             : "=v"(cpre[0].x), "=v"(cpre[0].y), "=v"(cpre[1].x), "=v"(cpre[1].y) : "s"(vtok));
#pragma unroll
                for (int k = 0; k < 2; ++k)
                    if (tid + k * NT < Cin) *reinterpret_cast<f32x2*>(sCo + (tid + k * NT) * 2) = cpre[k];
                cdep = cpre[0].x + cpre[1].x;
            }
            WP_LOAD_P(b, cbeg + 2, cdep, ofs)
            pfl = fl0;
            if (PRO) asm volatile("s_waitcnt lgkmcnt(0)\n\ts_barrier" ::: "memory");
            {
                constexpr int QR = (NA - PQ + 2 * NPV - 1) / (2 * NPV);
#define WP_HOOK0(e, v) WP_LOAD_A_RANGE(w0, PQ + (e) * QR, (PQ + ((e) + 1) * QR < NA ? PQ + ((e) + 1) * QR : NA), v)
#define WP_HOOK1(e, v) WP_LOAD_A_RANGE(w0, (PQ + (NPV + (e)) * QR < NA ? PQ + (NPV + (e)) * QR : NA), (PQ + (NPV + (e) + 1) * QR < NA ? PQ + (NPV + (e) + 1) * QR : NA), v)
                float pv0[NPV], pv1[NPV];
                f32x2 cf0[NPL], cf1[NPL];
                WP_READ_C(cbeg, cf0)
                WP_READ_C(cbeg + 1, cf1)
                WP_WRITE_PR(0, cbeg, fl0, pv0, cf0, "v184", "v185", "v186", "v187", "v188", "v189", "v190", "v191", "v192", WP_HOOK0)
                WP_WRITE_PR(1, cbeg + 1, fl0, pv1, cf1, "v194", "v195", "v196", "v197", "v198", "v199", "v200", "v201", "v202", WP_HOOK1)
#undef WP_HOOK0
#undef WP_HOOK1
                const float dep = pv0[0] + pv1[0];
                WP_LOAD_A_RANGE(w0, 0, PQ, dep)
            }
            asm volatile("s_waitcnt lgkmcnt(0)\n\ts_barrier" ::: "memory");
            {
                f32x2 rw[3][4];
                WP_READ_R(0, rw)
                WP_WRITE_V(0, rg, rw)
            }
            asm volatile("s_waitcnt lgkmcnt(0)\n\ts_barrier" ::: "memory");
            WP_WAIT(0)
        }
        WP_STAMP(0)
        int par = 0;
        for (; it < run_end; ++it) {
            const int q0 = it - b * ips, kh = q0 % ksp, q1 = q0 / ksp, cotile = q1 % nct, rr = q1 / nct;
            const int nx = it + 1 < run_end ? it + 1 : it;
            const int n0 = nx - b * ips, nkh = n0 % ksp, n1 = n0 / ksp, ncotile = n1 % nct, nrr = n1 / nct;
            const int cbeg = kh * nch, ncbeg = nkh * nch;
            const unsigned* wb_cur = wpb_u + (((long)cotile * (nch * ksp) + cbeg) * 16 + 2 * wave_u) * (NQ * 256);
            const unsigned* wb_nx = wpb_u + (((long)ncotile * (nch * ksp) + ncbeg) * 16 + 2 * wave_u) * (NQ * 256);
            const int tab_cur = it & 1, tab_nx = nx & 1;
            {
                unsigned dummy[NPL];
                WP_SLOT_TABLE(tab_nx, (nrr / rx_n) * 8, (nrr % rx_n) * 16, dummy)
                (void)dummy;
            }
#define WP_CHUNK_SCALARS                                                                                        \
            const int l2 = c + 2, l3 = c + 3;                                                                   \
            const int ch2 = l2 < nch ? cbeg + l2 : ncbeg + l2 - nch;                                            \
            const int ch3 = l3 < nch ? cbeg + l3 : ncbeg + l3 - nch;                                            \
            const int tab3 = l3 < nch ? tab_cur : tab_nx;                                                       \
            const unsigned* wnx = c + 1 < nch ? wb_cur + (long)(c + 1) * WSTR : wb_nx;
            if (rg == 0) {
                for (int c = 0; c < nch; ++c) {
                    WP_CHUNK_SCALARS
                    WP_VALU_PHASE(par, ch2, ch3, tab3, rg)
                    WP_MFMA_PHASE(par, wnx)
                    asm volatile("s_waitcnt lgkmcnt(0)\n\ts_barrier" ::: "memory");
                    par ^= 1;
                }
                asm volatile("s_waitcnt vmcnt(0) ; staging-first loop left" ::: "memory");
            } else {
                for (int c = 0; c < nch; ++c) {
                    WP_CHUNK_SCALARS
                    WP_MFMA_PHASE(par, wnx)
                    WP_VALU_PHASE(par, ch2, ch3, tab3, rg)
                    asm volatile("s_waitcnt lgkmcnt(0)\n\ts_barrier" ::: "memory");
                    par ^= 1;
                }
                asm volatile("s_waitcnt vmcnt(0) ; matrix-first loop left" ::: "memory");
            }
#undef WP_CHUNK_SCALARS
            chunks_done += nch;
            if constexpr (COT == 3)
                asm volatile("s_nop 15\n\ts_nop 15" : "+v"(acc[0][0]), "+v"(acc[0][1]), "+v"(acc[0][2]), "+v"(acc[1][0]), "+v"(acc[1][1]), "+v"(acc[1][2]) :: "memory");
            else if constexpr (COT == 2)
                asm volatile("s_nop 15\n\ts_nop 15" : "+v"(acc[0][0]), "+v"(acc[0][1]), "+v"(acc[1][0]), "+v"(acc[1][1]) :: "memory");
            else
                asm volatile("s_nop 15\n\ts_nop 15" : "+v"(acc[0][0]), "+v"(acc[1][0]) :: "memory");
            WP_STAMP(1)

            float* sM0 = smem + ((par ^ 1) ? VW : 0);
            float* sM1 = sP + (par ? PBUF : 0);
            int tid_e;
            asm volatile("v_mov_b32 %0, %1" : "=v"(tid_e) : "v"(tid));
            const int e_tile = tid_e & 31, e_col0 = tid_e >> 5;
            const int e_ty = e_tile >> 3, e_tx = e_tile & 7;
            const int oy0 = (rr / rx_n) * 8, ox0 = (rr % rx_n) * 16, co0 = cotile * BCO;
            const long pix = (long)(oy0 + 2 * e_ty) * W + ox0 + 2 * e_tx;
            float* const ydst = fin ? a.y : a.part + (long)kh * a.B * a.Cout * HW;
            float e_bias[COT][2];
            f32x2 e_r0[COT][2], e_r1[COT][2];
#define WP_EPI_FETCH(ct)                                                                                        \
            {                                                                                                   \
                _Pragma("unroll") for (int t2 = 0; t2 < 2; ++t2) {                                              \
                    const int co = co0 + (ct) * 32 + e_col0 + 16 * t2;                                          \
                    e_bias[ct][t2] = fin ? a.bias[co] : 0.0f;                          \
                    e_r0[ct][t2] = e_r1[ct][t2] = f32x2{0.0f, 0.0f};                                            \
                    if (a.res && fin) {                                                                         \
                        const long o = ((long)b * a.Cout + min(co, a.Cout - 1)) * HW + pix;                     \
                        e_r0[ct][t2] = *reinterpret_cast<const f32x2*>(a.res + o);                              \
                        e_r1[ct][t2] = *reinterpret_cast<const f32x2*>(a.res + o + W);                          \
                    }                                                                                           \
                }                                                                                               \
            }
            WP_EPI_FETCH(0)
            float* const sMw = wave_u < 6 ? sM0 + (2 * wave_u) * (32 * T) : sM1 + (2 * wave_u - 12) * (32 * T);
#pragma unroll
            for (int ct = 0; ct < COT; ++ct) {
#pragma unroll
                for (int i = 0; i < 2; ++i)
#pragma unroll
                    for (int r = 0; r < 16; ++r) {
                        const int col = (r & 3) + 8 * (r >> 2) + 4 * half;
                        sMw[(i * 32 + col) * T + l31] = acc[i][ct][r];
                    }
                if (ct + 1 < COT) WP_EPI_FETCH(ct + 1 < COT ? ct + 1 : ct)
                asm volatile("s_waitcnt lgkmcnt(0)\n\ts_barrier" ::: "memory");
#pragma unroll
                for (int t2 = 0; t2 < 2; ++t2) {
                    const int e_col = e_col0 + 16 * t2;
                    const int co = co0 + ct * 32 + e_col;
                    const f32x2 r0 = e_r0[ct][t2], r1 = e_r1[ct][t2];
                    float mm[16];
#pragma unroll
                    for (int xi = 0; xi < 16; ++xi) mm[xi] = xi < 12 ? sM0[(xi * 32 + e_col) * T + e_tile] : sM1[((xi - 12) * 32 + e_col) * T + e_tile];
                    float t0[4], t1[4];
#pragma unroll
                    for (int l = 0; l < 4; ++l) {
                        t0[l] = mm[0 * 4 + l] + mm[1 * 4 + l] + mm[2 * 4 + l];
                        t1[l] = mm[1 * 4 + l] - mm[2 * 4 + l] - mm[3 * 4 + l];
                    }
                    const float y00 = t0[0] + t0[1] + t0[2], y01 = t0[1] - t0[2] - t0[3];
                    const float y10 = t1[0] + t1[1] + t1[2], y11 = t1[1] - t1[2] - t1[3];
                    const float bvv = e_bias[ct][t2];
                    const float osc = fin ? a.out_scale : 1.0f;
                    const float v00 = (y00 + bvv + r0.x) * osc, v01 = (y01 + bvv + r0.y) * osc;
                    const float v10 = (y10 + bvv + r1.x) * osc, v11 = (y11 + bvv + r1.y) * osc;
                    if (co < a.Cout) {
                        const long o = ((long)b * a.Cout + co) * HW + pix;
                        *reinterpret_cast<float2*>(ydst + o) = make_float2(v00, v01);
                        *reinterpret_cast<float2*>(ydst + o + W) = make_float2(v10, v11);
                    }
                    if (a.stats && fin) {
                        float pil;
                        {
                            const int pv = __builtin_bit_cast(int, v00);
                            const int s0 = __builtin_amdgcn_readlane(pv, 0), s2 = __builtin_amdgcn_readlane(pv, 32);
                            pil = __builtin_bit_cast(float, (lane & 32) ? s2 : s0);
                        }
                        const float d0 = v00 - pil, d1 = v01 - pil, d2 = v10 - pil, d3 = v11 - pil;
                        float sm = (d0 + d1) + (d2 + d3);
                        float qm = (d0 * d0 + d1 * d1) + (d2 * d2 + d3 * d3);
#define WP_MERGE(CTRL, ROWMASK)                                                                                     \
                        {                                                                                           \
                            sm += __builtin_bit_cast(float, __builtin_amdgcn_update_dpp(0, __builtin_bit_cast(int, sm), CTRL, ROWMASK, 0xf, false)); \
                            qm += __builtin_bit_cast(float, __builtin_amdgcn_update_dpp(0, __builtin_bit_cast(int, qm), CTRL, ROWMASK, 0xf, false)); \
                        }
                        WP_MERGE(0xB1, 0xf)
                        WP_MERGE(0x4E, 0xf)
                        WP_MERGE(0x124, 0xf)
                        WP_MERGE(0x128, 0xf)
                        WP_MERGE(0x142, 0xa)
#undef WP_MERGE
                        if (e_tile == 31 && co < a.Cout) {
                            float* q = a.stats + (((long)b * a.Cout + co) * rpi + rr) * 2;
                            q[0] = sm + 128.0f * pil;
                            q[1] = fmaxf(qm - sm * sm * (1.0f / 128.0f), 0.0f);
                        }
                    }
                }
                asm volatile("s_waitcnt lgkmcnt(0)\n\ts_barrier" ::: "memory");
            }
#pragma unroll
            for (int i = 0; i < 2; ++i)
#pragma unroll
                for (int ct = 0; ct < COT; ++ct)
#pragma unroll
                    for (int r = 0; r < 16; ++r) acc[i][ct][r] = 0.0f;
            WP_STAMP(2)
        }
    }
    if (rec) {
        const unsigned long long now = __builtin_amdgcn_s_memtime();
        if (lane == 0) {
            unsigned long long* d = a.dbg + (long)blockIdx.x * 8;
            unsigned hwid, xcc;
            asm volatile("s_getreg_b32 %0, hwreg(HW_REG_HW_ID)" : "=s"(hwid));
            asm volatile("s_getreg_b32 %0, hwreg(HW_REG_XCC_ID)" : "=s"(xcc));
            d[0] = dt[0]; d[1] = dt[1]; d[2] = rt0; d[3] = __builtin_amdgcn_s_memrealtime();
            d[4] = ((unsigned long long)xcc << 32) | hwid;
            d[5] = dt[2];
            d[6] = (unsigned long long)chunks_done | ((unsigned long long)(it1 - it0) << 32);
            d[7] = now - t_start;
        }
    }
#undef WP_STAMP
#undef WP_EPI_FETCH
#undef WP_SLOT_TABLE
#undef WP_QUADS
#undef WP_LD1
#undef WP_MF1
#undef WP_LOAD_A_PIECE
#undef WP_LD1D
#undef WP_LOAD_A_RANGE
#undef WP_WAIT
#undef WP_LOAD_P
#undef WP_LOAD_PR
#undef WP_READ_C
#undef WP_NOHOOK
#undef WP_WRITE_P
#undef WP_WRITE_PR
#undef WP_READ_R
#undef WP_WRITE_V
#undef WP_LOAD_B
#undef WP_PRODUCT
#undef WP_MFMA_PHASE
#undef WP_VALU_PHASE
}

static size_t wino3p_lds_bytes(int Cin) {
    return (size_t)(2 * WP_VW + 2 * 4096 + 2 * Cin + 2 * WP_NPL * WP_NT) * sizeof(float);
}

static int wino3p_num_cus() {
    static std::atomic<int> cus[64];
    int dev = 0;
    if (hipGetDevice(&dev) != hipSuccess || dev < 0 || dev >= 64) return 256;
    int n = cus[dev].load(std::memory_order_acquire);
    if (n > 0) return n;
    if (hipDeviceGetAttribute(&n, hipDeviceAttributeMultiprocessorCount, dev) != hipSuccess || n <= 0) n = 256;
    cus[dev].store(n, std::memory_order_release);
    return n;
}

template <int COT, int PRO>
static int wino3p_launch2(const ConvArgs& a, hipStream_t s) {
    constexpr int BCO = 32 * COT;
    static PerDeviceOnce raised;
    if (raised.first_use()) {
        MCVD_HIP_CHECK(hipFuncSetAttribute(reinterpret_cast<const void*>(&conv_wino3p_kernel<COT, PRO>),
                                           hipFuncAttributeMaxDynamicSharedMemorySize, 160 * 1024));
        raised.done();
    }
    const int ksp = a.ksplit >= 2 ? a.ksplit : 1;
    const long n_items = (long)a.B * (a.H / 8) * (a.W / 16) * (a.CoutP / BCO) * ksp;
    const int cus = a.pgrid > 0 ? a.pgrid : wino3p_num_cus();
    dim3 grid((unsigned)(n_items < cus ? n_items : cus));
    ConvArgs k = a;
    if (k.dbg) k.wdma = 0;
#ifdef MCVD_DIAG
    if (k.dbg) {
        const char* w = getenv("MCVD_DBG_WAVE");
        k.wdma = w ? atoi(w) : 0;
    }
    k.wdma &= 0xff;
    if (const char* st = getenv("MCVD_W3P_STAGGER")) k.wdma |= atoi(st) << 8;
#else
    k.wdma &= 0xff;
#endif
    hipLaunchKernelGGL((conv_wino3p_kernel<COT, PRO>), grid, dim3(WP_NT), wino3p_lds_bytes(a.Cin), s, k);
    MCVD_HIP_CHECK(hipGetLastError());
    if (ksp >= 2) return launch_wino_ksplit_reduce(a, s);
    if (a.stats) set_last_conv_stats_np((a.H / 8) * (a.W / 16));
    return 0;
}

template <int COT>
static int wino3p_launch1(const ConvArgs& a, hipStream_t s) {
    if (!a.coef && !a.act) return wino3p_launch2<COT, 0>(a, s);
    if (!a.act) return wino3p_launch2<COT, 1>(a, s);
    return wino3p_launch2<COT, 2>(a, s);
}

bool conv_wino3p_usable(const ConvArgs& a) {
    const int nchunks = a.CinP / WP_CK;
    return a.ks == 3 && a.H % 8 == 0 && a.W % 16 == 0 && a.H >= 8 && a.W >= 16 && a.wpb && !a.gb && a.Cin <= 1024 &&
           a.CinP % WP_CK == 0 && (a.C1 == 0 || a.C0 % WP_CK == 0) && a.H * a.W <= 16384 &&
           (long)a.B * (a.C0 > a.C1 ? a.C0 : a.C1) * a.H * a.W < (1L << 29) && wino3p_lds_bytes(a.Cin) <= 160 * 1024 &&
           (long)a.B * (a.H / 8) * (a.W / 16) * (a.CoutP / 32) * 8 < (1L << 31) &&
           (a.ksplit >= 2 ? ((a.ksplit == 2 || a.ksplit == 4 || a.ksplit == 8) && nchunks % a.ksplit == 0 && nchunks / a.ksplit >= WP_MINCH &&
                             conv_part_fits(a))
                          : nchunks >= WP_MINCH);
}

int launch_conv_wino3p(const ConvArgs& a, hipStream_t s) {
    MCVD_REQUIRE(conv_wino3p_usable(a), "persistent winograd bf16x3 conv: unsupported (ks=%d H=%d W=%d Cin=%d C0=%d ksplit=%d, packed weight pieces %s)",
                 a.ks, a.H, a.W, a.Cin, a.C0, a.ksplit, a.wpb ? "present" : "missing");
    const int cot = conv_wino_cout_tile(a.Cout);
    MCVD_REQUIRE(a.CoutP % (32 * cot) == 0, "persistent winograd bf16x3 conv: CoutP=%d vs tile %d", a.CoutP, 32 * cot);
    switch (cot) {
        case 1: return wino3p_launch1<1>(a, s);
        case 2: return wino3p_launch1<2>(a, s);
        default: return wino3p_launch1<3>(a, s);
    }
}

}
```

### mcvd_pytorch_amd/csrc/model.cpp

```cpp
#include "model.h"
#include "conv_kernels.h"

#include <math.h>
#include <stdarg.h>
#include <stdio.h>
#include <string.h>

#include <algorithm>
#include <tuple>

namespace mcvd {

static thread_local char g_err[1024] = "";
void set_error(const char* fmt, ...) {
    va_list ap;
    va_start(ap, fmt);
    vsnprintf(g_err, sizeof(g_err), fmt, ap);
    va_end(ap);
}
const char* get_error() { return g_err; }

static int gn_groups(int ch) {
    int g = std::min(ch / 4, 32);
    while (g > 1 && ch % g != 0) --g;
// ... 654 lines not shown
    if (op.alt_kind == CK_GEMM3_TAPS) {
        g.Cout = 9 * a.Cout;
        g.bias = packed + op.alt_bias;
        g.res = nullptr; g.out_scale = 1.0f; g.stats = nullptr;
        g.y = buf;
    } else {
        g.Cin = op.alt_CinP;
        g.im2col = 1;
        bool lds_form = ctx->im2col_lds != 0;
        if (lds_form) {
            lds_form = false;
            for (int c = 4; c >= 1 && !lds_form; --c) lds_form = conv1x1_h2_supported(g, c, 3);
        }
        if (!lds_form) {
            g.im2col = 0;
            g.x0 = buf; g.x1 = nullptr;
            g.C0 = op.alt_CinP; g.C1 = 0;
        }
    }
    int cot = a.cot;
    if (cot < 1 || cot > 4 || !conv1x1_h2_supported(g, cot, 3))
        for (cot = 4; cot > 1 && !conv1x1_h2_supported(g, cot, 3); --cot) {}
    g.cot = cot;
    return g;
}

int mcvd_model::launch_gemm_form(const Op& op, const ConvArgs& a, float* buf, hipStream_t s) {
    const ConvArgs g = gemm_form_args(op, a, buf);
    if (op.alt_kind == CK_GEMM3_IM2COL && !g.im2col)
        if (int rc = launch_im2col3x3(a.x0, a.C0, a.x1, a.C1, buf, a.B, a.H, a.W, op.alt_CinP, s)) return rc;
    if (int rc = launch_conv_mfma(g, s)) return rc;
    if (op.alt_kind == CK_GEMM3_TAPS) return launch_taps_shift_add(buf, a.bias, a.res, a.out_scale, a.y, a.B, a.Cout, a.H, a.W, s);
    return 0;
}

int mcvd_model::launch_op(const Op& op, const float* x, const void* lab, const float* cond, float* out, int B) {
    hipStream_t s = op_stream ? op_stream : ctx->stream;
    switch (op.kind) {
        case OP_TEMB: {
            if (temb_row_live) return 0;
            const float* w0 = blob + params[find_param("unet.all_modules.0.weight")].off;
            const float* b0 = blob + params[find_param("unet.all_modules.0.bias")].off;
            const float* w1 = blob + params[find_param("unet.all_modules.1.weight")].off;
            const float* b1 = blob + params[find_param("unet.all_modules.1.bias")].off;
            const float* emb = d.cond_emb ? blob + params[find_param("unet.all_modules.2.weight")].off : nullptr;
            return launch_temb_mlp(lab, labels_f32, packed + freqs_off, w0, b0, w1, b1, resolve(op.dst, x, cond, out, B),
                                   (uniform_labels && !d.cond_emb) ? 1 : B, d.ngf, T, emb, cond_mask, s);
        }
        case OP_DENSE:
            if (temb_row_live) return 0;
            return launch_dense_all(resolve(op.src0, x, cond, out, B), packed + dense_wt, packed + dense_bias,
                                    resolve(op.dst, x, cond, out, B), (uniform_labels && !d.cond_emb) ? 1 : B, T, NE, s);
        case OP_GN:
            return launch_gn(op, x, lab, cond, out, B);
        case OP_CONV: {
            ConvArgs a{};
            a.x0 = resolve(op.src0, x, cond, out, B);
            a.x1 = resolve(op.src1, x, cond, out, B);
            a.C0 = op.src0.C;
            a.C1 = op.src1.kind == REF_NONE ? 0 : op.src1.C;
            MCVD_REQUIRE(a.x0 && (a.C1 == 0 || a.x1), "forward: module %d needs a conditioning tensor (cond is NULL)", op.module);
            a.coef = op.coef.kind == REF_NONE ? nullptr : resolve(op.coef, x, cond, out, B);
            a.act = op.act;
            a.wp = packed + op.wp;
            a.wpw = op.wpw >= 0 ? packed + op.wpw : nullptr;
            a.wph = (op.wph >= 0 && packed_h_valid) ? packed_h + op.wph : nullptr;
            a.wpb = op.wpb >= 0 ? packed + op.wpb : nullptr;
            a.bias = packed + op.bias;
            a.res = op.res.kind == REF_NONE ? nullptr : resolve(op.res, x, cond, out, B);
            a.out_scale = op.out_scale;
            a.y = resolve(op.dst, x, cond, out, B);
            a.B = B;
            a.Cin = a.C0 + a.C1;
            a.CinP = op.CinP;
            a.Cout = op.Cout;
            a.CoutP = op.CoutP;
            a.H = op.H;
            a.W = op.W;
            a.ks = op.ks;
            a.cot = op.cot;
            a.shape_hint = (op.ks == 1 && ctx->conv_shape1 >= 0) ? ctx->conv_shape1 : ctx->conv_shape;
            a.wdma = ctx->conv_wdma;
            a.pgrid = ctx->persist_grid;
            a.part = (op.ks == 3 && op.H * op.W <= 256) ? ksplit_buf : nullptr;
            a.part_floats = a.part ? ksplit_floats : 0;
            const size_t oi = (size_t)(&op - ops.data());
            if (conv_kernel(a.shape_hint).family == CF_SPLIT1) {
                const int np = pieces(a.shape_hint);
                for (int c = 4; c >= 1 && !conv1x1_h2_supported(a, a.cot, np); --c)
                    if (conv1x1_h2_supported(a, c, np)) a.cot = c;
            }
            if (a.shape_hint < 0 && tuned_B == B && oi < tuned_shape.size() && tuned_shape[oi] >= 0) {
                a.shape_hint = tuned_shape[oi];
                a.cot = tuned_cot[oi];
                const bool raw_in = conv_input_raw(op);
                if ((!ctx->f16x1 || raw_in) && without_f16x1(a.shape_hint) != a.shape_hint) a.shape_hint = without_f16x1(a.shape_hint);
                if ((!ctx->f16x2 || raw_in) && without_f16x2(a.shape_hint) != a.shape_hint) {
                    a.shape_hint = without_f16x2(a.shape_hint);
                    if (conv_kernel(a.shape_hint).own_cot && !conv_kernel_usable(a.shape_hint, a)) a.cot = op.cot;
                }
                if (!ctx->bf16x3 && without_bf16x3(a.shape_hint) != a.shape_hint) {
                    a.shape_hint = without_bf16x3(a.shape_hint);
                    a.cot = op.cot;
                }
            }
            if (op.gb.kind != REF_NONE) {
                a.gb = resolve(op.gb, x, cond, out, B);
                a.coef2 = op.coef2.kind == REF_NONE ? nullptr : resolve(op.coef2, x, cond, out, B);
                if (a.shape_hint == CK_RETIRED_SPADE_WINO || a.shape_hint == CK_RETIRED_SPADE_WINO_K2) a.shape_hint = CK_AUTO;
                const bool want_fused = ctx->spade_fuse && !ctx->naive_conv && ctx->winograd;
                ConvArgs t = a;
                t.shape_hint = a.shape_hint == CK_WINO_K2 ? CK_WINO_K2 : CK_WINO;
                t.ksplit = k_parts(t.shape_hint);
                bool fused = want_fused && conv_wino_usable(t);
                if (!fused && t.ksplit == 2) { t.ksplit = 0; t.shape_hint = CK_WINO; fused = want_fused && conv_wino_usable(t); }
                if (fused) {
                    a.shape_hint = t.shape_hint;
                    ++fused_launches[2];
                } else {
                    float* tmp = resolve(op.tmp, x, cond, out, B);
                    if (int rc = launch_spade_apply(a.x0, a.C0, a.x1, a.C1, a.coef, a.gb, a.coef2, tmp, B, op.H * op.W, s)) return rc;
                    a.x0 = tmp; a.x1 = nullptr; a.C0 = a.Cin; a.C1 = 0; a.coef = nullptr; a.act = 0; a.gb = nullptr; a.coef2 = nullptr;
                }
            }
            a.stats = (ctx->gn_stats && op.stats.kind != REF_NONE && !ctx->naive_conv && (op.ks == 3 || ctx->gn_stats >= 2 || conv_kernel(a.shape_hint).family == CF_SPLIT1))
                          ? resolve(op.stats, x, cond, out, B) : nullptr;
            if (ran_kernel.size() != ops.size()) ran_kernel.assign(ops.size(), -1);
            if (kv_live.size() != ops.size()) kv_live.assign(ops.size(), 0);
            if (gn_done.size() != ops.size()) gn_done.assign(ops.size(), 0);
            if (op.gn_next >= 0) {
                gn_done[op.gn_next] = 0;
                const Op& g = ops[op.gn_next];
                if (ctx->gn_producer && ctx->gn_stats && a.stats && op.ks == 3 && !ctx->dbg_skip_finalize) {
                    a.gno.coef = resolve(g.coef, x, cond, out, B);
                    a.gno.groups = g.groups;
                    a.gno.eps = g.eps;
                    a.gno.mode = g.gn_mode;
                    if (g.gn_mode == 1) {
                        a.gno.p0 = resolve(ops[1].dst, x, cond, out, B);
                        a.gno.emb_stride = (uniform_labels && !d.cond_emb) ? 0 : NE;
                        a.gno.emb_off = g.emb_off;
                    } else if (g.gn_mode == 2) {
                        a.gno.p0 = blob + g.p0;
                        a.gno.p1 = blob + g.p1;
                    }
                }
            }
            if (op.attn_op >= 0) {
                kv_live[op.attn_op] = 0;
                const Op& at = ops[op.attn_op];
                const bool want = ctx->attn_presplit && !ctx->naive_conv && ctx->bf16x3 && !ctx->f16x2 && (ctx->naive_attn == 0 || ctx->naive_attn == 4) &&
                                  !(ctx->share_fence && mcvd_ctx_shares_device(ctx)) && attn_h2p_supported(at.Cout, at.heads, at.H * at.W) && a.shape_hint == CK_GEMM1_BF16X3;
                if (want) {
                    ConvArgs t = a;
                    t.kv_img = resolve(op.kv, x, cond, out, B);
                    t.kv_C = at.Cout;
                    t.kv_D = at.Cout / at.heads;
                    if (conv1x1_h2_kv_supported(t, t.cot)) {
                        a = t;
                        kv_live[op.attn_op] = 1;
                    }
                }
            }
            if (ctx->naive_conv) {
                stats_np[oi] = 0;
                ran_kernel[oi] = -2;
// ... 52 lines not shown
                    MCVD_REQUIRE(!d.gamma, "forward: a gamma model draws its conditioning noise per row (k_cum[labels]); pass z through "
                                           "mcvd_model_set_cond_noise or use mcvd_sampler_run");
                    if (int rc = launch_randn(cond_z, cond_noise_seed, cond_noise_offset, (1ull << 32) + cond_noise_draw, B, per, s)) return rc;
                }
                ++cond_noise_draw;
                z = cond_z;
            }
            return launch_cond_noise(cond, z, alphas_dev, static_cast<const int64_t*>(lab), d.num_classes,
                                     resolve(op.dst, x, cond, out, B), B, per, s);
        }
        case OP_COEF2: {
            const int self = (int)(&op - ops.data());
            if (coef2_desc_dev && coef2_count > 1) {
                if (self != coef2_first) return 0;
                return launch_coef2_all(resolve(ops[1].dst, x, cond, out, B), (uniform_labels && !d.cond_emb) ? 0 : NE, coef2_desc_dev,
                                        coef2_count, coef2_cmax, arena, B, s);
            }
            return launch_coef2(resolve(ops[1].dst, x, cond, out, B), (uniform_labels && !d.cond_emb) ? 0 : NE, op.emb_off,
                                resolve(op.dst, x, cond, out, B), B, op.Cout, s);
        }
        case OP_APPLY:
            return launch_spade_apply(resolve(op.src0, x, cond, out, B), op.src0.C, resolve(op.src1, x, cond, out, B),
                                      op.src1.kind == REF_NONE ? 0 : op.src1.C, resolve(op.coef, x, cond, out, B),
                                      resolve(op.gb, x, cond, out, B),
                                      op.coef2.kind == REF_NONE ? nullptr : resolve(op.coef2, x, cond, out, B),
                                      resolve(op.dst, x, cond, out, B), B, op.H * op.W, s);
        case OP_ATTN:
        {
            const bool shared = ctx->share_fence && mcvd_ctx_shares_device(ctx);
            const size_t ai = (size_t)(&op - ops.data());
            if (ai < kv_live.size() && kv_live[ai]) {
                kv_live[ai] = 0;
                ++fused_launches[0];
                return launch_attention_h2p(resolve(op.src0, x, cond, out, B), resolve(op.kv, x, cond, out, B), resolve(op.dst, x, cond, out, B), B,
                                            op.Cout, op.heads, op.H * op.W, s);
            }
            return launch_attention(ctx->naive_attn, shared ? 0 : ctx->f16x2, shared ? 0 : ctx->bf16x3, resolve(op.src0, x, cond, out, B), resolve(op.dst, x, cond, out, B), B,
                                    op.Cout, op.heads, op.H * op.W, s);
        }
        default:
            set_error("forward: unknown op kind %d", (int)op.kind);
            return -1;
    }
}

int mcvd_model::autotune(int B) {
    hipStream_t s = ctx->stream;
    tuned_shape.assign(ops.size(), -1);
    tuned_cot.assign(ops.size(), 0);
    hipEvent_t e0, e1;
    MCVD_HIP_CHECK(hipEventCreate(&e0));
    MCVD_HIP_CHECK(hipEventCreate(&e1));
    MCVD_HIP_CHECK(hipMemsetAsync(arena, 0x3c, (size_t)arena_per_sample * B * sizeof(float), s));
    struct Key { int ks, H, cin, cout, coef, res; bool operator<(const Key& o) const {
        return std::tie(ks, H, cin, cout, coef, res) < std::tie(o.ks, o.H, o.cin, o.cout, o.coef, o.res); } };
    std::map<Key, std::pair<int, int>> best;
    float* scratch_io = arena;
    for (size_t i = 0; i < ops.size(); ++i) {
        const Op& op = ops[i];
        if (op.kind != OP_CONV) continue;
        const int cin = op.src0.C + (op.src1.kind == REF_NONE ? 0 : op.src1.C);
        Key k{op.ks, op.H, cin, op.Cout, (op.coef.kind != REF_NONE ? 1 : 0) + (op.gb.kind != REF_NONE ? 2 : 0) + (op.coef2.kind != REF_NONE ? 4 : 0),
              op.res.kind != REF_NONE};
        auto it = best.find(k);
        if (it == best.end()) {
            ConvArgs a{};
            a.x0 = resolve(op.src0, scratch_io, scratch_io, scratch_io, B);
            a.x1 = resolve(op.src1, scratch_io, scratch_io, scratch_io, B);
            a.C0 = op.src0.C;
            a.C1 = op.src1.kind == REF_NONE ? 0 : op.src1.C;
            a.coef = op.coef.kind == REF_NONE ? nullptr : resolve(op.coef, scratch_io, scratch_io, scratch_io, B);
            a.act = op.act;
            a.wp = packed + op.wp;
            a.wpw = op.wpw >= 0 ? packed + op.wpw : nullptr;
            a.wph = (op.wph >= 0 && packed_h_valid) ? packed_h + op.wph : nullptr;
            a.wpb = op.wpb >= 0 ? packed + op.wpb : nullptr;
            a.bias = packed + op.bias;
            a.res = op.res.kind == REF_NONE ? nullptr : resolve(op.res, scratch_io, scratch_io, scratch_io, B);
            a.out_scale = op.out_scale;
            a.y = resolve(op.dst, scratch_io, scratch_io, scratch_io, B);
            a.B = B; a.Cin = cin; a.CinP = op.CinP; a.Cout = op.Cout; a.CoutP = op.CoutP; a.H = op.H; a.W = op.W; a.ks = op.ks;
            a.wdma = ctx->conv_wdma;
            a.pgrid = ctx->persist_grid;
            a.part = (op.ks == 3 && op.H * op.W <= 256) ? ksplit_buf : nullptr;
            a.part_floats = a.part ? ksplit_floats : 0;
            const bool spade_fused = op.gb.kind != REF_NONE && ctx->spade_fuse && ctx->winograd;
            if (spade_fused) {
                a.gb = resolve(op.gb, scratch_io, scratch_io, scratch_io, B);
                a.coef2 = op.coef2.kind == REF_NONE ? nullptr : resolve(op.coef2, scratch_io, scratch_io, scratch_io, B);
            } else if (op.gb.kind != REF_NONE) {
                a.x0 = resolve(op.tmp, scratch_io, scratch_io, scratch_io, B);
                a.x1 = nullptr; a.C0 = cin; a.C1 = 0; a.coef = nullptr; a.act = 0;
            }
            float best_ms = 1e30f;
            std::pair<int, int> choice{-1, op.cot};
            auto time_candidate = [&](int shape, int cot) -> int {
                a.cot = cot;
                a.shape_hint = shape;
                if (launch_conv_mfma(a, s)) return 0;
                MCVD_HIP_CHECK(hipEventRecord(e0, s));
                for (int r = 0; r < 3; ++r)
                    if (int rc = launch_conv_mfma(a, s)) return rc;
                MCVD_HIP_CHECK(hipEventRecord(e1, s));
                MCVD_HIP_CHECK(hipEventSynchronize(e1));
                float ms = 0.f;
                MCVD_HIP_CHECK(hipEventElapsedTime(&ms, e0, e1));
                if (ms < best_ms) { best_ms = ms; choice = {shape, cot}; }
                return 0;
            };
            auto offer = [&](int id, int cot) -> int {
                a.cot = cot;
                return conv_kernel_usable(id, a) ? time_candidate(id, cot) : 0;
            };
            const int cots[2] = {op.cot, 1};
            for (int ci = 0; ci < (op.cot == 1 ? 1 : 2); ++ci) {
                for (int shape = CK_TILE256; shape <= CK_WINO; ++shape) {
                    if (spade_fused && conv_kernel_usable(CK_WINO, a) && shape != CK_WINO) continue;
                    if (shape == CK_TILE_SPLITK && (op.ks != 3 || !ctx->conv_wdma)) continue;
                    if (shape == CK_WINO && (ci > 0 || !ctx->winograd || !conv_kernel_usable(CK_WINO, a))) continue;
                    const int bpx = shape == CK_TILE256 ? 256 : shape == CK_TILE128 ? 128 : 64;
                    const bool fits = bpx % op.W == 0 && (bpx / op.W <= op.H ? op.H % (bpx / op.W) == 0 : (bpx / op.W) % op.H == 0);
                    if (shape != CK_WINO && !fits) continue;
                    if (int rc = time_candidate(shape, cots[ci])) return rc;
                }
            }
            a.cot = op.cot;
            if (op.alt_kind && !spade_fused && op.gb.kind == REF_NONE) {
                ConvArgs t = a;
                t.shape_hint = op.alt_kind;
                t.stats = (ctx->gn_stats && op.stats.kind != REF_NONE) ? resolve(op.stats, scratch_io, scratch_io, scratch_io, B) : nullptr;
                float* buf = resolve(op.alt_buf, scratch_io, scratch_io, scratch_io, B);
                for (int c = 4; c >= 1; --c) {
                    t.cot = c;
                    if (!gemm_form_usable(op, t)) break;
                    if (gemm_form_args(op, t, buf).cot != c) continue;
                    if (launch_gemm_form(op, t, buf, s)) continue;
                    MCVD_HIP_CHECK(hipEventRecord(e0, s));
                    for (int r = 0; r < 3; ++r)
                        if (int rc = launch_gemm_form(op, t, buf, s)) return rc;
                    MCVD_HIP_CHECK(hipEventRecord(e1, s));
                    MCVD_HIP_CHECK(hipEventSynchronize(e1));
                    float ms = 0.f;
                    MCVD_HIP_CHECK(hipEventElapsedTime(&ms, e0, e1));
                    if (ms < best_ms) { best_ms = ms; choice = {op.alt_kind, c}; }
                }
            }
            if (op.ks == 3 && ctx->winograd)
                if (int rc = offer(CK_WINO_K2, op.cot)) return rc;
            const bool g8 = op.H == 8 && op.W == 8;
            const long pairs = op.ks == 3 ? (g8 ? (B + 1) / 2 : (long)B * (op.H / 8) * (op.W / 16)) * (op.CoutP / (32 * conv_wino_cout_tile(op.Cout))) : 0;
            const bool few_pairs = op.ks == 3 && 2 * pairs < 1024;
            if (op.ks == 3 && ctx->winograd && ctx->bf16x3 && !spade_fused) {
                for (int id : {CK_WINO3, CK_WINO3_K2, CK_WINO3P, CK_WINO3P_K2})
                    if (int rc = offer(id, op.cot)) return rc;
                if (few_pairs) {
                    for (int id : {CK_WINO3_K4, CK_WINO3P_K4})
                        if (int rc = offer(id, op.cot)) return rc;
                    if (4 * pairs < 1024)
                        if (int rc = offer(CK_WINO3_K8, op.cot)) return rc;
                }
            }
            const bool f16_ok = ctx->f16x2 && !conv_input_raw(op);
            if (op.ks == 3 && ctx->winograd && f16_ok && !spade_fused) {
                for (int id : {CK_WINO2H, CK_WINO2H_K2})
                    if (int rc = offer(id, op.cot)) return rc;
                if (few_pairs)
// ... 288 lines not shown
```

### mcvd_pytorch_amd/csrc/model.h

```cpp
#pragma once
#include <atomic>
#include <map>
#include <string>
#include <vector>

#include "../../include/mcvd_hip.h"
#include "common.h"

struct mcvd_ctx {
    int device = 0;
    int shared_device = 0;
    hipStream_t stream = nullptr;
    int naive_conv = 0;
    int naive_attn = 0;
    int gn_producer = 1;
    int dbg_skip_finalize = 0;
    int fir_form = 0;
    int graph = 0;
    hipStream_t cap = nullptr;
    std::atomic<unsigned> epoch{0};
    int conv_shape = -1;
    int conv_shape1 = -1;
    int winograd = 1;
    int persist_grid = 0;
    int temb_table = 1;
    int im2col_lds = 1;
    int wino_selftest = 0;
    int conv_cot = 0;
    int bf16x3 = 1;
    int f16x2 = 0;
    int f16x1 = 0;
    int conv_dma1 = 1;
    int conv_wdma = 1;
    int share_fence = 0;
    int side_stream = 0;
    hipStream_t side = nullptr;
    hipEvent_t ev_fork = nullptr, ev_join = nullptr;
    int spade_fuse = 0;
    int attn_presplit = 1;
    int gn_stats = 1;
    int autotune = 1;
    int profile = 0;
    unsigned long long* dbg = nullptr;
    const float* spade_gb = nullptr;
    const float* spade_coef2 = nullptr;
    float* stats_buf = nullptr;
    int* range_flag = nullptr;
    float* scratch = nullptr;
    size_t scratch_bytes = 0;
    int ensure_scratch(size_t bytes);
};

bool mcvd_ctx_shares_device(const mcvd_ctx* c);

namespace mcvd {

struct ParamInfo {
    std::string name;
    int64_t shape[4] = {0, 0, 0, 0};
    int ndim = 0;
    int64_t off = 0;
    int64_t numel = 0;
    bool set = false;
};

enum RefKind { REF_NONE = 0, REF_ARENA, REF_X, REF_COND, REF_OUT };
struct TRef {
    RefKind kind = REF_NONE;
    int64_t off = 0;
    int C = 0;
};

enum OpKind { OP_TEMB, OP_DENSE, OP_GN, OP_CONV, OP_FIR, OP_ATTN, OP_NEAREST, OP_COEF2, OP_APPLY, OP_CONDNOISE };

struct Op {
    OpKind kind;
    int module = -1;
    TRef src0, src1, dst, res;
    int H = 0, W = 0;
    int Cout = 0, ks = 0;
    int groups = 0;
    float eps = 0.f;
    int gn_mode = 0;
    int64_t p0 = -1, p1 = -1;
    int emb_off = 0;
    TRef coef;
    int act = 0;
    int64_t wp = -1, bias = -1;
    int64_t wpw = -1;
    int64_t wph = -1;
    int64_t wpb = -1;
    int CinP = 0, CoutP = 0, cot = 0;
    float out_scale = 1.f;
    int alt_kind = 0;
    int64_t alt_wp = -1, alt_wpb = -1, alt_bias = -1;
    int alt_CinP = 0, alt_CoutP = 0;
    TRef alt_buf;
    int up = 0;
    int heads = 0;
    TRef kv;
    int attn_op = -1;
    TRef gb, coef2;
    TRef tmp;
    TRef dst2;
    bool side = false;
    bool join = false;
// ... 152 lines not shown
```

Measured before the change: 259.2.

## Add transposed-MFMA Winograd epilogue with swizzled LDS and vectorized stores

Adds a new epilogue variant to the Winograd 3x3 conv kernels. It swaps the MFMA operand order so the accumulators come out transposed, writes them to LDS as swizzled 16-byte vectors, reads them back with batched ds_read_b64, and emits 16-byte output stores with a simplified stats reduction. The goal is to cut LDS bank conflicts, scalar LDS traffic and narrow global stores in the output transform. A runtime option (on by default) keeps the old epilogue selectable, and a partials-copy API is added for testing. The price is more template instantiations and hand-written asm whose lane mapping could be wrong.

```diff
diff --git a/include/mcvd_hip.h b/include/mcvd_hip.h
--- a/include/mcvd_hip.h
+++ b/include/mcvd_hip.h
@@ -169,6 +169,7 @@
 int mcvd_op_global_avg(mcvd_ctx* ctx, const float* x, float* y, int64_t NC, int HW);
 int mcvd_op_resize299(mcvd_ctx* ctx, const float* x, int64_t n, int H, int W, int normalize, float* y);
 int mcvd_last_conv_kernel(void);
+int mcvd_op_conv2d_partials(mcvd_ctx* ctx, float* dst, int64_t n_floats);
 int mcvd_ctx_set_spade_inputs(mcvd_ctx* ctx, const float* gb, const float* coef2);
 int mcvd_ctx_set_stats_buffer(mcvd_ctx* ctx, float* device_floats);
 int mcvd_last_conv_stats_np(void);
diff --git a/mcvd_pytorch_amd/_lib.py b/mcvd_pytorch_amd/_lib.py
--- a/mcvd_pytorch_amd/_lib.py
+++ b/mcvd_pytorch_amd/_lib.py
@@ -63,6 +63,7 @@
     "mcvd_model_set_tuning": (_i, [_vp, _i, _vp, _vp, _i]),
     "mcvd_model_graph_stats": (_i, [_vp, C.POINTER(_i64), C.POINTER(_i64)]),
     "mcvd_last_conv_kernel": (_i, []),
+    "mcvd_op_conv2d_partials": (_i, [_vp, _vp, _i64]),
     "mcvd_last_conv_stats_np": (_i, []),
     "mcvd_ctx_set_stats_buffer": (_i, [_vp, _vp]),
     "mcvd_ctx_set_spade_inputs": (_i, [_vp, _vp, _vp]),
diff --git a/mcvd_pytorch_amd/csrc/api.cpp b/mcvd_pytorch_amd/csrc/api.cpp
--- a/mcvd_pytorch_amd/csrc/api.cpp
+++ b/mcvd_pytorch_amd/csrc/api.cpp
@@ -369,6 +369,7 @@
     }
     else if (!strcmp(key, "conv_cot")) ctx->conv_cot = value;
     else if (!strcmp(key, "persist_grid")) ctx->persist_grid = value;
+    else if (!strcmp(key, "wino_epi")) ctx->wino_epi = value != 0;
     else if (!strcmp(key, "temb_table")) ctx->temb_table = value;
     else if (!strcmp(key, "im2col_lds")) ctx->im2col_lds = value;
     else if (!strcmp(key, "gn_stats")) ctx->gn_stats = value;
@@ -1433,6 +1434,8 @@
         }
         if (pfloats) { a.part = ctx->scratch + wfloats + a.CoutP + ufloats + hfloats; a.part_floats = pfloats; }
     }
+    ctx->last_part = a.part;
+    ctx->last_part_floats = a.part ? pfloats : 0;
     if (int rc = launch_pack_conv_weight(w, ctx->scratch, Cout, a.Cin, ks, a.CinP, a.CoutP, 0, 0, ctx->stream)) return rc;
     if (np1) {
         if (int rc = launch_pack_conv1x1_h2(ctx->scratch, ctx->scratch + wfloats + a.CoutP, a.CinP, a.CoutP, ctx->stream, np1)) return rc;
@@ -1445,6 +1448,7 @@
     if (k.own_cot && ctx->conv_cot > 0) a.cot = ctx->conv_cot;
     a.wdma = ctx->conv_wdma;
     a.pgrid = ctx->persist_grid;
+    a.old_epi = !ctx->wino_epi;
     a.dbg = ctx->dbg;
     a.stats = ctx->naive_conv ? nullptr : ctx->stats_buf;
     if (ctx->spade_gb) {
@@ -1460,6 +1464,16 @@
     API_CATCH
 }
 
+int mcvd_op_conv2d_partials(mcvd_ctx* ctx, float* dst, int64_t n_floats) {
+    API_TRY
+    MCVD_REQUIRE(ctx && dst, "op_conv2d_partials: NULL argument");
+    MCVD_REQUIRE(ctx->last_part && n_floats >= 0 && (size_t)n_floats <= ctx->last_part_floats,
+                 "op_conv2d_partials: %lld floats asked, the last mcvd_op_conv2d left %zu", (long long)n_floats, ctx->last_part_floats);
+    MCVD_HIP_CHECK(hipMemcpyAsync(dst, ctx->last_part, (size_t)n_floats * sizeof(float), hipMemcpyDeviceToDevice, ctx->stream));
+    return 0;
+    API_CATCH
+}
+
 int mcvd_last_conv_kernel(void) { return last_conv_kernel(); }
 
 int mcvd_last_conv_stats_np(void) { return last_conv_stats_np(); }
diff --git a/mcvd_pytorch_amd/csrc/common.h b/mcvd_pytorch_amd/csrc/common.h
--- a/mcvd_pytorch_amd/csrc/common.h
+++ b/mcvd_pytorch_amd/csrc/common.h
@@ -83,6 +83,7 @@
     size_t part_floats;
     int wdma;
     int pgrid;
+    int old_epi;
     unsigned long long* dbg;
     float* stats;
     const float* gb;
diff --git a/mcvd_pytorch_amd/csrc/kernels/conv_wino3.cpp b/mcvd_pytorch_amd/csrc/kernels/conv_wino3.cpp
--- a/mcvd_pytorch_amd/csrc/kernels/conv_wino3.cpp
+++ b/mcvd_pytorch_amd/csrc/kernels/conv_wino3.cpp
@@ -36,7 +36,7 @@
     w3 = w3_cvt_pk(v.x, v.y);
 }
 
-template <int COT, int PRO, bool G8, int EXP = 0>
+template <int COT, int PRO, bool G8, bool EPT, int EXP = 0>
 __global__ __launch_bounds__(512) __attribute__((amdgpu_num_vgpr(86))) void conv_wino3_kernel(ConvArgs a) {
     constexpr int NT = W3_NT, CK = W3_CK, T = W3_T, BCO = 32 * COT, PP = W3_PP, VW = W3_VW, PW = W3_PW;
     constexpr int PSZ = CK * 10 * PP;
@@ -134,7 +134,11 @@
 
 #define W3_QUADS(X, q, A1, A2) X(0, "v[184:187]", q, A1, A2) X(1, "v[188:191]", q, A1, A2) X(2, "v[192:195]", q, A1, A2) X(3, "v[196:199]", q, A1, A2) X(4, "v[200:203]", q, A1, A2) X(5, "v[204:207]", q, A1, A2) X(6, "v[208:211]", q, A1, A2) X(7, "v[212:215]", q, A1, A2) X(8, "v[216:219]", q, A1, A2) X(9, "v[220:223]", q, A1, A2) X(10, "v[224:227]", q, A1, A2) X(11, "v[228:231]", q, A1, A2) X(12, "v[232:235]", q, A1, A2) X(13, "v[236:239]", q, A1, A2) X(14, "v[240:243]", q, A1, A2) X(15, "v[244:247]", q, A1, A2) X(16, "v[248:251]", q, A1, A2) X(17, "v[252:255]", q, A1, A2)
 #define W3_LD1(K, R, q, P, UNUSED) if ((q) == K) asm volatile("global_load_dwordx4 " R ", %0, %1" :: "v"(wr_voff), "s"(P) : "memory");
-#define W3_MF1(K, R, q, ACC, BV) if ((q) == K) asm volatile("v_mfma_f32_32x32x16_bf16 %0, " R ", %1, %0" : "+v"(ACC) : "v"(BV));
+#define W3_MF1(K, R, q, ACC, BV)                                                                                 \
+    if ((q) == K) {                                                                                              \
+        if constexpr (EPT) asm volatile("v_mfma_f32_32x32x16_bf16 %0, %1, " R ", %0" : "+v"(ACC) : "v"(BV));    \
+        else asm volatile("v_mfma_f32_32x32x16_bf16 %0, " R ", %1, %0" : "+v"(ACC) : "v"(BV));                  \
+    }
 #define W3_LOAD_A(ch, i)                                                                                        \
     {                                                                                                           \
         const unsigned* ua = wr_base + (long)(ch) * (16 * NQ * 256) + (i) * (NQ * 256);                         \
@@ -306,7 +310,7 @@
 #pragma unroll
             for (int r = 0; r < 16; ++r) acc[i][ct][r] = 0.0f;
 
-    const bool rec = a.dbg != nullptr && wave == (a.wdma & 7);
+    const bool rec = a.dbg != nullptr && wave_u == (a.wdma & 7);
     const bool sub = (a.wdma & 64) != 0;
     unsigned long long sp[5] = {0, 0, 0, 0, 0};
     unsigned long long tk0 = 0, tprev = 0, dt[2] = {0, 0}, rt0 = 0;
@@ -425,102 +429,229 @@
     else
         asm volatile("s_nop 15\n\ts_nop 15" : "+v"(acc[0][0]), "+v"(acc[1][0]) :: "memory");
 
-    float* sM = smem;
-    const int e_tile = tid & 31, e_col0 = tid >> 5;
-    const int e_ty = G8 ? (e_tile >> 2) & 3 : e_tile >> 3, e_tx = G8 ? e_tile & 3 : e_tile & 7;
-    const int e_b = min(b + (G8 ? e_tile >> 4 : 0), a.B - 1);
-    const bool e_valid = !G8 || b + (e_tile >> 4) < a.B;
-    const long pix = (long)(oy0 + 2 * e_ty) * W + ox0 + 2 * e_tx;
-    const bool fin = ksp == 1;
-    float* const ydst = fin ? a.y : a.part + (long)kh * a.B * a.Cout * HW;
-    float e_bias[COT][2];
-    f32x2 e_r0[COT][2], e_r1[COT][2];
-#pragma unroll
-    for (int ct = 0; ct < COT; ++ct)
-#pragma unroll
-        for (int t2 = 0; t2 < 2; ++t2) {
-            const int co = co0 + ct * 32 + e_col0 + 16 * t2;
-            e_bias[ct][t2] = fin ? a.bias[co] : 0.0f;
-            e_r0[ct][t2] = e_r1[ct][t2] = f32x2{0.0f, 0.0f};
+    if constexpr (!EPT) {
+        float* sM = smem;
+        const int e_tile = tid & 31, e_col0 = tid >> 5;
+        const int e_ty = G8 ? (e_tile >> 2) & 3 : e_tile >> 3, e_tx = G8 ? e_tile & 3 : e_tile & 7;
+        const int e_b = min(b + (G8 ? e_tile >> 4 : 0), a.B - 1);
+        const bool e_valid = !G8 || b + (e_tile >> 4) < a.B;
+        const long pix = (long)(oy0 + 2 * e_ty) * W + ox0 + 2 * e_tx;
+        const bool fin = ksp == 1;
+        float* const ydst = fin ? a.y : a.part + (long)kh * a.B * a.Cout * HW;
+        float e_bias[COT][2];
+        f32x2 e_r0[COT][2], e_r1[COT][2];
+#pragma unroll
+        for (int ct = 0; ct < COT; ++ct)
+#pragma unroll
+            for (int t2 = 0; t2 < 2; ++t2) {
+                const int co = co0 + ct * 32 + e_col0 + 16 * t2;
+                e_bias[ct][t2] = fin ? a.bias[co] : 0.0f;
+                e_r0[ct][t2] = e_r1[ct][t2] = f32x2{0.0f, 0.0f};
+                if (a.res && fin) {
+                    const long o = ((long)e_b * a.Cout + min(co, a.Cout - 1)) * HW + pix;
+                    e_r0[ct][t2] = *reinterpret_cast<const f32x2*>(a.res + o);
+                    e_r1[ct][t2] = *reinterpret_cast<const f32x2*>(a.res + o + W);
+                }
+            }
+        asm volatile("s_waitcnt lgkmcnt(0)\n\ts_barrier" ::: "memory");
+        W3_STAMP(1)
+#pragma unroll
+        for (int ct = 0; ct < COT; ++ct) {
+#pragma unroll
+            for (int i = 0; i < 2; ++i)
+#pragma unroll
+                for (int r = 0; r < 16; ++r) {
+                    const int col = (r & 3) + 8 * (r >> 2) + 4 * half;
+                    sM[((2 * wave + i) * 32 + col) * T + l31] = acc[i][ct][r];
+                }
+            asm volatile("s_waitcnt lgkmcnt(0)\n\ts_barrier" ::: "memory");
+#pragma unroll
+            for (int t2 = 0; t2 < 2; ++t2) {
+                const int e_col = e_col0 + 16 * t2;
+                const int co = co0 + ct * 32 + e_col;
+                const f32x2 r0 = e_r0[ct][t2], r1 = e_r1[ct][t2];
+                float mm[16];
+#pragma unroll
+                for (int xi = 0; xi < 16; ++xi) mm[xi] = sM[(xi * 32 + e_col) * T + e_tile];
+                float t0[4], t1[4];
+#pragma unroll
+                for (int l = 0; l < 4; ++l) {
+                    t0[l] = mm[0 * 4 + l] + mm[1 * 4 + l] + mm[2 * 4 + l];
+                    t1[l] = mm[1 * 4 + l] - mm[2 * 4 + l] - mm[3 * 4 + l];
+                }
+                const float y00 = t0[0] + t0[1] + t0[2], y01 = t0[1] - t0[2] - t0[3];
+                const float y10 = t1[0] + t1[1] + t1[2], y11 = t1[1] - t1[2] - t1[3];
+                const float bvv = e_bias[ct][t2];
+                const float osc = fin ? a.out_scale : 1.0f;
+                const float v00 = (y00 + bvv + r0.x) * osc, v01 = (y01 + bvv + r0.y) * osc;
+                const float v10 = (y10 + bvv + r1.x) * osc, v11 = (y11 + bvv + r1.y) * osc;
+                if (co < a.Cout && e_valid) {
+                    const long o = ((long)e_b * a.Cout + co) * HW + pix;
+                    *reinterpret_cast<float2*>(ydst + o) = make_float2(v00, v01);
+                    *reinterpret_cast<float2*>(ydst + o + W) = make_float2(v10, v11);
+                }
+                if (a.stats && fin) {
+                    float pil;
+                    {
+                        const int pv = __builtin_bit_cast(int, v00);
+                        const int s0 = __builtin_amdgcn_readlane(pv, 0), s2 = __builtin_amdgcn_readlane(pv, 32);
+                        if (G8) {
+                            const int s1 = __builtin_amdgcn_readlane(pv, 16), s3 = __builtin_amdgcn_readlane(pv, 48);
+                            pil = __builtin_bit_cast(float, (lane & 32) ? ((lane & 16) ? s3 : s2) : ((lane & 16) ? s1 : s0));
+                        } else {
+                            pil = __builtin_bit_cast(float, (lane & 32) ? s2 : s0);
+                        }
+                    }
+                    const float d0 = v00 - pil, d1 = v01 - pil, d2 = v10 - pil, d3 = v11 - pil;
+                    float sm = (d0 + d1) + (d2 + d3);
+                    float qm = (d0 * d0 + d1 * d1) + (d2 * d2 + d3 * d3);
+#define W3_MERGE(CTRL, ROWMASK)                                                                                     \
+                    {                                                                                                   \
+                        sm += __builtin_bit_cast(float, __builtin_amdgcn_update_dpp(0, __builtin_bit_cast(int, sm), CTRL, ROWMASK, 0xf, false)); \
+                        qm += __builtin_bit_cast(float, __builtin_amdgcn_update_dpp(0, __builtin_bit_cast(int, qm), CTRL, ROWMASK, 0xf, false)); \
+                    }
+                    W3_MERGE(0xB1, 0xf)
+                    W3_MERGE(0x4E, 0xf)
+                    W3_MERGE(0x124, 0xf)
+                    W3_MERGE(0x128, 0xf)
+                    if (!G8) W3_MERGE(0x142, 0xa)
+#undef W3_MERGE
+                    const bool writer = G8 ? (e_tile & 15) == 0 : e_tile == 31;
+                    if (writer && co < a.Cout && e_valid) {
+                        constexpr float NPIX = G8 ? 64.0f : 128.0f;
+                        float* q = a.stats + (((long)e_b * a.Cout + co) * (rx_n * ry_n) + rr) * 2;
+                        q[0] = sm + NPIX * pil;
+                        q[1] = fmaxf(qm - sm * sm * (1.0f / NPIX), 0.0f);
+                    }
+                }
+            }
+            if (ct + 1 < COT) asm volatile("s_waitcnt lgkmcnt(0)\n\ts_barrier" ::: "memory");
+        }
+    } else {
+        float* sM = smem;
+        const int e_pair = tid & 15, e_col = tid >> 4;
+        const int e_ty = G8 ? (e_pair >> 1) & 3 : e_pair >> 2, e_tx = G8 ? 2 * (e_pair & 1) : 2 * (e_pair & 3);
+        const int e_b = min(b + (G8 ? e_pair >> 3 : 0), a.B - 1);
+        const bool e_valid = !G8 || b + (e_pair >> 3) < a.B;
+        const long pix = (long)(oy0 + 2 * e_ty) * W + ox0 + 2 * e_tx;
+        const bool fin = ksp == 1;
+        float* const ydst = fin ? a.y : a.part + (long)kh * a.B * a.Cout * HW;
+        const unsigned e_rd = (unsigned)(uintptr_t)(__attribute__((address_space(3))) float*)sM +
+                              (unsigned)(e_col * 32 + (((e_pair >> 1) ^ (e_col & 7)) << 2) + 2 * (e_pair & 1)) * 4u;
+        float e_bias[COT];
+        f32x4 e_r0[COT], e_r1[COT];
+#pragma unroll
+        for (int ct = 0; ct < COT; ++ct) {
+            const int co = co0 + ct * 32 + e_col;
+            e_bias[ct] = fin ? a.bias[co] : 0.0f;
+            e_r0[ct] = e_r1[ct] = f32x4{0.0f, 0.0f, 0.0f, 0.0f};
             if (a.res && fin) {
                 const long o = ((long)e_b * a.Cout + min(co, a.Cout - 1)) * HW + pix;
-                e_r0[ct][t2] = *reinterpret_cast<const f32x2*>(a.res + o);
-                e_r1[ct][t2] = *reinterpret_cast<const f32x2*>(a.res + o + W);
+                e_r0[ct] = *reinterpret_cast<const f32x4*>(a.res + o);
+                e_r1[ct] = *reinterpret_cast<const f32x4*>(a.res + o + W);
             }
         }
-    asm volatile("s_waitcnt lgkmcnt(0)\n\ts_barrier" ::: "memory");
-    W3_STAMP(1)
-#pragma unroll
-    for (int ct = 0; ct < COT; ++ct) {
-#pragma unroll
-        for (int i = 0; i < 2; ++i)
-#pragma unroll
-            for (int r = 0; r < 16; ++r) {
-                const int col = (r & 3) + 8 * (r >> 2) + 4 * half;
-                sM[((2 * wave + i) * 32 + col) * T + l31] = acc[i][ct][r];
+        asm volatile("s_waitcnt lgkmcnt(0)\n\ts_barrier" ::: "memory");
+        W3_STAMP(1)
+#pragma unroll
+        for (int ct = 0; ct < COT; ++ct) {
+#pragma unroll
+            for (int i = 0; i < 2; ++i)
+#pragma unroll
+                for (int g = 0; g < 4; ++g) {
+                    const f32x4 v = {acc[i][ct][4 * g], acc[i][ct][4 * g + 1], acc[i][ct][4 * g + 2], acc[i][ct][4 * g + 3]};
+                    *reinterpret_cast<f32x4*>(sM + ((2 * wave + i) * 32 + l31) * 32 + (((2 * g + half) ^ (l31 & 7)) << 2)) = v;
+                }
+            asm volatile("s_waitcnt lgkmcnt(0)\n\ts_barrier" ::: "memory");
+            {
+                const int co = co0 + ct * 32 + e_col;
+                f32x2 mm[16];
+                asm volatile(
+                    "ds_read_b64 %0, %16\n\t"
+                    "ds_read_b64 %1, %16 offset:4096\n\t"
+                    "ds_read_b64 %2, %16 offset:8192\n\t"
+                    "ds_read_b64 %3, %16 offset:12288\n\t"
+                    "ds_read_b64 %4, %16 offset:16384\n\t"
+                    "ds_read_b64 %5, %16 offset:20480\n\t"
+                    "ds_read_b64 %6, %16 offset:24576\n\t"
+                    "ds_read_b64 %7, %16 offset:28672\n\t"
+                    "ds_read_b64 %8, %16 offset:32768\n\t"
+                    "ds_read_b64 %9, %16 offset:36864\n\t"
+                    "ds_read_b64 %10, %16 offset:40960\n\t"
+                    "ds_read_b64 %11, %16 offset:45056\n\t"
+                    "ds_read_b64 %12, %16 offset:49152\n\t"
+                    "ds_read_b64 %13, %16 offset:53248\n\t"
+                    "ds_read_b64 %14, %16 offset:57344\n\t"
+                    "ds_read_b64 %15, %16 offset:61440\n\t"
+                    "s_waitcnt lgkmcnt(0)"
+                    : "=&v"(mm[0]), "=&v"(mm[1]), "=&v"(mm[2]), "=&v"(mm[3]), "=&v"(mm[4]), "=&v"(mm[5]), "=&v"(mm[6]), "=&v"(mm[7]), "=&v"(mm[8]), "=&v"(mm[9]), "=&v"(mm[10]), "=&v"(mm[11]), "=&v"(mm[12]), "=&v"(mm[13]), "=&v"(mm[14]), "=&v"(mm[15])
+                    : "v"(e_rd) : "memory");
+                const float bvv = e_bias[ct];
+                const float osc = fin ? a.out_scale : 1.0f;
+                float vv[2][4];
+#pragma unroll
+                for (int k = 0; k < 2; ++k) {
+                    float t0[4], t1[4];
+#pragma unroll
+                    for (int l = 0; l < 4; ++l) {
+                        t0[l] = mm[0 * 4 + l][k] + mm[1 * 4 + l][k] + mm[2 * 4 + l][k];
+                        t1[l] = mm[1 * 4 + l][k] - mm[2 * 4 + l][k] - mm[3 * 4 + l][k];
+                    }
+                    const float y00 = t0[0] + t0[1] + t0[2], y01 = t0[1] - t0[2] - t0[3];
+                    const float y10 = t1[0] + t1[1] + t1[2], y11 = t1[1] - t1[2] - t1[3];
+                    vv[k][0] = (y00 + bvv + e_r0[ct][2 * k]) * osc;
+                    vv[k][1] = (y01 + bvv + e_r0[ct][2 * k + 1]) * osc;
+                    vv[k][2] = (y10 + bvv + e_r1[ct][2 * k]) * osc;
+                    vv[k][3] = (y11 + bvv + e_r1[ct][2 * k + 1]) * osc;
+                }
+                if (co < a.Cout && e_valid) {
+                    const long o = ((long)e_b * a.Cout + co) * HW + pix;
+                    *reinterpret_cast<f32x4*>(ydst + o) = f32x4{vv[0][0], vv[0][1], vv[1][0], vv[1][1]};
+                    *reinterpret_cast<f32x4*>(ydst + o + W) = f32x4{vv[0][2], vv[0][3], vv[1][2], vv[1][3]};
+                }
+                if (a.stats && fin) {
+                    const int pl = (lane & (G8 ? 56 : 48)) << 2;
+                    const float pil = __builtin_bit_cast(float, __builtin_amdgcn_ds_bpermute(pl, __builtin_bit_cast(int, vv[0][0])));
+                    float sk[2], qk[2];
+#pragma unroll
+                    for (int k = 0; k < 2; ++k) {
+                        const float d0 = vv[k][0] - pil, d1 = vv[k][1] - pil, d2 = vv[k][2] - pil, d3 = vv[k][3] - pil;
+                        sk[k] = (d0 + d1) + (d2 + d3);
+                        qk[k] = (d0 * d0 + d1 * d1) + (d2 * d2 + d3 * d3);
+                    }
+                    float sm = sk[0] + sk[1], qm = qk[0] + qk[1];
+#define W3_MERGE(CTRL)                                                                                              \
+                    {                                                                                               \
+                        sm += __builtin_bit_cast(float, __builtin_amdgcn_update_dpp(0, __builtin_bit_cast(int, sm), CTRL, 0xf, 0xf, false)); \
+                        qm += __builtin_bit_cast(float, __builtin_amdgcn_update_dpp(0, __builtin_bit_cast(int, qm), CTRL, 0xf, 0xf, false)); \
+                    }
+#define W3_MERGE_LANE(SRC)                                                                                          \
+                    {                                                                                               \
+                        sm += __builtin_bit_cast(float, __builtin_amdgcn_ds_bpermute((SRC) << 2, __builtin_bit_cast(int, sm))); \
+                        qm += __builtin_bit_cast(float, __builtin_amdgcn_ds_bpermute((SRC) << 2, __builtin_bit_cast(int, qm))); \
+                    }
+                    W3_MERGE(0xB1)
+                    if constexpr (G8) {
+                        W3_MERGE_LANE((lane & 56) | ((lane - 2) & 7))
+                        W3_MERGE_LANE((lane & 56) | ((lane - 4) & 7))
+                    } else {
+                        W3_MERGE(0x4E)
+                        W3_MERGE(0x124)
+                        W3_MERGE(0x128)
+                    }
+#undef W3_MERGE
+#undef W3_MERGE_LANE
+                    const bool writer = G8 ? (e_pair & 7) == 0 : e_pair == 15;
+                    if (writer && co < a.Cout && e_valid) {
+                        constexpr float NPIX = G8 ? 64.0f : 128.0f;
+                        float* q = a.stats + (((long)e_b * a.Cout + co) * (rx_n * ry_n) + rr) * 2;
+                        q[0] = sm + NPIX * pil;
+                        q[1] = fmaxf(qm - sm * sm * (1.0f / NPIX), 0.0f);
+                    }
+                }
             }
-        asm volatile("s_waitcnt lgkmcnt(0)\n\ts_barrier" ::: "memory");
-#pragma unroll
-        for (int t2 = 0; t2 < 2; ++t2) {
-            const int e_col = e_col0 + 16 * t2;
-            const int co = co0 + ct * 32 + e_col;
-            const f32x2 r0 = e_r0[ct][t2], r1 = e_r1[ct][t2];
-            float mm[16];
-#pragma unroll
-            for (int xi = 0; xi < 16; ++xi) mm[xi] = sM[(xi * 32 + e_col) * T + e_tile];
-            float t0[4], t1[4];
-#pragma unroll
-            for (int l = 0; l < 4; ++l) {
-                t0[l] = mm[0 * 4 + l] + mm[1 * 4 + l] + mm[2 * 4 + l];
-                t1[l] = mm[1 * 4 + l] - mm[2 * 4 + l] - mm[3 * 4 + l];
-            }
-            const float y00 = t0[0] + t0[1] + t0[2], y01 = t0[1] - t0[2] - t0[3];
-            const float y10 = t1[0] + t1[1] + t1[2], y11 = t1[1] - t1[2] - t1[3];
-            const float bvv = e_bias[ct][t2];
-            const float osc = fin ? a.out_scale : 1.0f;
-            const float v00 = (y00 + bvv + r0.x) * osc, v01 = (y01 + bvv + r0.y) * osc;
-            const float v10 = (y10 + bvv + r1.x) * osc, v11 = (y11 + bvv + r1.y) * osc;
-            if (co < a.Cout && e_valid) {
-                const long o = ((long)e_b * a.Cout + co) * HW + pix;
-                *reinterpret_cast<float2*>(ydst + o) = make_float2(v00, v01);
-                *reinterpret_cast<float2*>(ydst + o + W) = make_float2(v10, v11);
-            }
-            if (a.stats && fin) {
-                float pil;
-                {
-                    const int pv = __builtin_bit_cast(int, v00);
-                    const int s0 = __builtin_amdgcn_readlane(pv, 0), s2 = __builtin_amdgcn_readlane(pv, 32);
-                    if (G8) {
-                        const int s1 = __builtin_amdgcn_readlane(pv, 16), s3 = __builtin_amdgcn_readlane(pv, 48);
-                        pil = __builtin_bit_cast(float, (lane & 32) ? ((lane & 16) ? s3 : s2) : ((lane & 16) ? s1 : s0));
-                    } else {
-                        pil = __builtin_bit_cast(float, (lane & 32) ? s2 : s0);
-                    }
-                }
-                const float d0 = v00 - pil, d1 = v01 - pil, d2 = v10 - pil, d3 = v11 - pil;
-                float sm = (d0 + d1) + (d2 + d3);
-                float qm = (d0 * d0 + d1 * d1) + (d2 * d2 + d3 * d3);
-#define W3_MERGE(CTRL, ROWMASK)                                                                                     \
-                {                                                                                                   \
-                    sm += __builtin_bit_cast(float, __builtin_amdgcn_update_dpp(0, __builtin_bit_cast(int, sm), CTRL, ROWMASK, 0xf, false)); \
-                    qm += __builtin_bit_cast(float, __builtin_amdgcn_update_dpp(0, __builtin_bit_cast(int, qm), CTRL, ROWMASK, 0xf, false)); \
-                }
-                W3_MERGE(0xB1, 0xf)
-                W3_MERGE(0x4E, 0xf)
-                W3_MERGE(0x124, 0xf)
-                W3_MERGE(0x128, 0xf)
-                if (!G8) W3_MERGE(0x142, 0xa)
-#undef W3_MERGE
-                const bool writer = G8 ? (e_tile & 15) == 0 : e_tile == 31;
-                if (writer && co < a.Cout && e_valid) {
-                    constexpr float NPIX = G8 ? 64.0f : 128.0f;
-                    float* q = a.stats + (((long)e_b * a.Cout + co) * (rx_n * ry_n) + rr) * 2;
-                    q[0] = sm + NPIX * pil;
-                    q[1] = fmaxf(qm - sm * sm * (1.0f / NPIX), 0.0f);
-                }
-            }
-        }
-        if (ct + 1 < COT) asm volatile("s_waitcnt lgkmcnt(0)\n\ts_barrier" ::: "memory");
+            if (ct + 1 < COT) asm volatile("s_waitcnt lgkmcnt(0)\n\ts_barrier" ::: "memory");
+        }
     }
     if (rec) {
         const unsigned long long now = __builtin_amdgcn_s_memtime();
@@ -570,15 +701,15 @@
 
 int launch_wino_ksplit_reduce(const ConvArgs& a, hipStream_t s);
 
-template <int COT, int PRO, bool G8, int EXP>
+template <int COT, int PRO, bool G8, bool EPT, int EXP>
 static int wino3_launch_k(const ConvArgs& k, dim3 grid, size_t lds, hipStream_t s) {
     static PerDeviceOnce raised;
     if (raised.first_use()) {
-        MCVD_HIP_CHECK(hipFuncSetAttribute(reinterpret_cast<const void*>(&conv_wino3_kernel<COT, PRO, G8, EXP>),
+        MCVD_HIP_CHECK(hipFuncSetAttribute(reinterpret_cast<const void*>(&conv_wino3_kernel<COT, PRO, G8, EPT, EXP>),
                                            hipFuncAttributeMaxDynamicSharedMemorySize, 160 * 1024));
         raised.done();
     }
-    hipLaunchKernelGGL((conv_wino3_kernel<COT, PRO, G8, EXP>), grid, dim3(W3_NT), lds, s, k);
+    hipLaunchKernelGGL((conv_wino3_kernel<COT, PRO, G8, EPT, EXP>), grid, dim3(W3_NT), lds, s, k);
     return 0;
 }
 
@@ -601,20 +732,20 @@
     const int e = exp_s ? atoi(exp_s) : 0;
     if (COT == 3 && PRO == 2 && !G8 && e != 0) {
         switch (e) {
-            case 1: rc = wino3_launch_k<3, 2, false, 1>(k, grid, lds, s); break;
-            case 2: rc = wino3_launch_k<3, 2, false, 2>(k, grid, lds, s); break;
-            case 3: rc = wino3_launch_k<3, 2, false, 3>(k, grid, lds, s); break;
-            case 4: rc = wino3_launch_k<3, 2, false, 4>(k, grid, lds, s); break;
-            case 16: rc = wino3_launch_k<3, 2, false, 16>(k, grid, lds, s); break;
-            case 15: rc = wino3_launch_k<3, 2, false, 15>(k, grid, lds, s); break;
-            case 27: rc = wino3_launch_k<3, 2, false, 27>(k, grid, lds, s); break;
-            case 11: rc = wino3_launch_k<3, 2, false, 11>(k, grid, lds, s); break;
+            case 1: rc = wino3_launch_k<3, 2, false, true, 1>(k, grid, lds, s); break;
+            case 2: rc = wino3_launch_k<3, 2, false, true, 2>(k, grid, lds, s); break;
+            case 3: rc = wino3_launch_k<3, 2, false, true, 3>(k, grid, lds, s); break;
+            case 4: rc = wino3_launch_k<3, 2, false, true, 4>(k, grid, lds, s); break;
+            case 16: rc = wino3_launch_k<3, 2, false, true, 16>(k, grid, lds, s); break;
+            case 15: rc = wino3_launch_k<3, 2, false, true, 15>(k, grid, lds, s); break;
+            case 27: rc = wino3_launch_k<3, 2, false, true, 27>(k, grid, lds, s); break;
+            case 11: rc = wino3_launch_k<3, 2, false, true, 11>(k, grid, lds, s); break;
             default: mcvd::set_error("MCVD_WINO3_EXP=%d is not a built ablation", e); return -1;
         }
     } else
 #endif
     {
-        rc = wino3_launch_k<COT, PRO, G8, 0>(k, grid, lds, s);
+        rc = a.old_epi ? wino3_launch_k<COT, PRO, G8, false, 0>(k, grid, lds, s) : wino3_launch_k<COT, PRO, G8, true, 0>(k, grid, lds, s);
     }
     if (rc) return rc;
     MCVD_HIP_CHECK(hipGetLastError());
diff --git a/mcvd_pytorch_amd/csrc/kernels/conv_wino3p.cpp b/mcvd_pytorch_amd/csrc/kernels/conv_wino3p.cpp
--- a/mcvd_pytorch_amd/csrc/kernels/conv_wino3p.cpp
+++ b/mcvd_pytorch_amd/csrc/kernels/conv_wino3p.cpp
@@ -38,7 +38,7 @@
     w3 = wp_cvt_pk(v.x, v.y);
 }
 
-template <int COT, int PRO>
+template <int COT, int PRO, bool EPT>
 __global__ __launch_bounds__(512) __attribute__((amdgpu_num_vgpr(86))) void conv_wino3p_kernel(ConvArgs a) {
     constexpr int NT = WP_NT, CK = WP_CK, T = WP_T, BCO = 32 * COT, PP = WP_PP, VW = WP_VW, PW = WP_PW;
     constexpr int PSZ = CK * 10 * PP;
@@ -133,7 +133,11 @@
 
 #define WP_QUADS(X, q, A1, A2) X(0, "v[184:187]", q, A1, A2) X(1, "v[188:191]", q, A1, A2) X(2, "v[192:195]", q, A1, A2) X(3, "v[196:199]", q, A1, A2) X(4, "v[200:203]", q, A1, A2) X(5, "v[204:207]", q, A1, A2) X(6, "v[208:211]", q, A1, A2) X(7, "v[212:215]", q, A1, A2) X(8, "v[216:219]", q, A1, A2) X(9, "v[220:223]", q, A1, A2) X(10, "v[224:227]", q, A1, A2) X(11, "v[228:231]", q, A1, A2) X(12, "v[232:235]", q, A1, A2) X(13, "v[236:239]", q, A1, A2) X(14, "v[240:243]", q, A1, A2) X(15, "v[244:247]", q, A1, A2) X(16, "v[248:251]", q, A1, A2) X(17, "v[252:255]", q, A1, A2)
 #define WP_LD1(K, R, q, P, UNUSED) if ((q) == K) asm volatile("global_load_dwordx4 " R ", %0, %1" :: "v"(wr_voff), "s"(P) : "memory");
-#define WP_MF1(K, R, q, ACC, BV) if ((q) == K) asm volatile("v_mfma_f32_32x32x16_bf16 %0, " R ", %1, %0" : "+v"(ACC) : "v"(BV));
+#define WP_MF1(K, R, q, ACC, BV)                                                                                 \
+    if ((q) == K) {                                                                                              \
+        if constexpr (EPT) asm volatile("v_mfma_f32_32x32x16_bf16 %0, %1, " R ", %0" : "+v"(ACC) : "v"(BV));    \
+        else asm volatile("v_mfma_f32_32x32x16_bf16 %0, " R ", %1, %0" : "+v"(ACC) : "v"(BV));                  \
+    }
 #define WP_LOAD_A_PIECE(WPTR, i, pc)                                                                            \
     {                                                                                                           \
         const unsigned* ua = (WPTR) + (i) * (NQ * 256);                                                         \
@@ -266,7 +270,7 @@
 #pragma unroll
             for (int r = 0; r < 16; ++r) acc[i][ct][r] = 0.0f;
 
-    const bool rec = a.dbg != nullptr && wave == (a.wdma & 7);
+    const bool rec = a.dbg != nullptr && wave_u == (a.wdma & 7);
     unsigned long long tprev = t_start, dt[3] = {0, 0, 0}, rt0 = 0;
     if (rec) rt0 = __builtin_amdgcn_s_memrealtime();
 #define WP_STAMP(i)                                                                                             \
@@ -290,9 +294,11 @@
             const int q0 = it - b * ips, kh = q0 % ksp, q1 = q0 / ksp, cotile = q1 % nct, rr = q1 / nct;
             const int oy0 = (rr / rx_n) * 8, ox0 = (rr % rx_n) * 16, cbeg = kh * nch;
             const unsigned* w0 = wpb_u + (((long)cotile * (nch * ksp) + cbeg) * 16 + 2 * wave_u) * (NQ * 256);
+            int tid_p;
+            asm volatile("v_mov_b32 %0, %1" : "=v"(tid_p) : "v"(tid));
             const float* co_src[2];
 #pragma unroll
-            for (int k = 0; k < 2; ++k) co_src[k] = a.coef + ((long)b * Cin + min(tid + k * NT, Cin - 1)) * 2;
+            for (int k = 0; k < 2; ++k) co_src[k] = a.coef + ((long)b * Cin + min(tid_p + k * NT, Cin - 1)) * 2;
             if (PRO)
                 asm volatile("global_load_dwordx2 v[172:173], %0, off\n\tglobal_load_dwordx2 v[174:175], %1, off"
                              :: "v"(co_src[0]), "v"(co_src[1]) : "memory");
@@ -310,7 +316,7 @@
                              : "=v"(cpre[0].x), "=v"(cpre[0].y), "=v"(cpre[1].x), "=v"(cpre[1].y) : "s"(vtok));
 #pragma unroll
                 for (int k = 0; k < 2; ++k)
-                    if (tid + k * NT < Cin) *reinterpret_cast<f32x2*>(sCo + (tid + k * NT) * 2) = cpre[k];
+                    if (tid_p + k * NT < Cin) *reinterpret_cast<f32x2*>(sCo + (tid_p + k * NT) * 2) = cpre[k];
                 cdep = cpre[0].x + cpre[1].x;
             }
             WP_LOAD_P(b, cbeg + 2, cdep, ofs)
@@ -322,6 +328,10 @@
 #define WP_HOOK1(e, v) WP_LOAD_A_RANGE(w0, (PQ + (NPV + (e)) * QR < NA ? PQ + (NPV + (e)) * QR : NA), (PQ + (NPV + (e) + 1) * QR < NA ? PQ + (NPV + (e) + 1) * QR : NA), v)
                 float pv0[NPV], pv1[NPV];
                 f32x2 cf0[NPL], cf1[NPL];
+                unsigned p_pk_run[NPL];
+#pragma unroll
+                for (int sl = 0; sl < NPL; ++sl) asm volatile("v_mov_b32 %0, %1" : "=v"(p_pk_run[sl]) : "v"(p_pk[sl]));
+                const unsigned p_pk[NPL] = {p_pk_run[0], p_pk_run[1], p_pk_run[2]};
                 WP_READ_C(cbeg, cf0)
                 WP_READ_C(cbeg + 1, cf1)
                 WP_WRITE_PR(0, cbeg, fl0, pv0, cf0, "v184", "v185", "v186", "v187", "v188", "v189", "v190", "v191", "v192", WP_HOOK0)
@@ -392,95 +402,208 @@
 
             float* sM0 = smem + ((par ^ 1) ? VW : 0);
             float* sM1 = sP + (par ? PBUF : 0);
-            int tid_e;
-            asm volatile("v_mov_b32 %0, %1" : "=v"(tid_e) : "v"(tid));
-            const int e_tile = tid_e & 31, e_col0 = tid_e >> 5;
-            const int e_ty = e_tile >> 3, e_tx = e_tile & 7;
-            const int oy0 = (rr / rx_n) * 8, ox0 = (rr % rx_n) * 16, co0 = cotile * BCO;
-            const long pix = (long)(oy0 + 2 * e_ty) * W + ox0 + 2 * e_tx;
-            float* const ydst = fin ? a.y : a.part + (long)kh * a.B * a.Cout * HW;
-            float e_bias[COT][2];
-            f32x2 e_r0[COT][2], e_r1[COT][2];
+            if constexpr (!EPT) {
+                int tid_e;
+                asm volatile("v_mov_b32 %0, %1" : "=v"(tid_e) : "v"(tid));
+                const int e_tile = tid_e & 31, e_col0 = tid_e >> 5;
+                const int e_ty = e_tile >> 3, e_tx = e_tile & 7;
+                const int oy0 = (rr / rx_n) * 8, ox0 = (rr % rx_n) * 16, co0 = cotile * BCO;
+                const long pix = (long)(oy0 + 2 * e_ty) * W + ox0 + 2 * e_tx;
+                float* const ydst = fin ? a.y : a.part + (long)kh * a.B * a.Cout * HW;
+                float e_bias[COT][2];
+                f32x2 e_r0[COT][2], e_r1[COT][2];
 #define WP_EPI_FETCH(ct)                                                                                        \
-            {                                                                                                   \
-                _Pragma("unroll") for (int t2 = 0; t2 < 2; ++t2) {                                              \
-                    const int co = co0 + (ct) * 32 + e_col0 + 16 * t2;                                          \
-                    e_bias[ct][t2] = fin ? a.bias[co] : 0.0f;                          \
-                    e_r0[ct][t2] = e_r1[ct][t2] = f32x2{0.0f, 0.0f};                                            \
+                {                                                                                                   \
+                    _Pragma("unroll") for (int t2 = 0; t2 < 2; ++t2) {                                              \
+                        const int co = co0 + (ct) * 32 + e_col0 + 16 * t2;                                          \
+                        e_bias[ct][t2] = fin ? a.bias[co] : 0.0f;                          \
+                        e_r0[ct][t2] = e_r1[ct][t2] = f32x2{0.0f, 0.0f};                                            \
+                        if (a.res && fin) {                                                                         \
+                            const long o = ((long)b * a.Cout + min(co, a.Cout - 1)) * HW + pix;                     \
+                            e_r0[ct][t2] = *reinterpret_cast<const f32x2*>(a.res + o);                              \
+                            e_r1[ct][t2] = *reinterpret_cast<const f32x2*>(a.res + o + W);                          \
+                        }                                                                                           \
+                    }                                                                                               \
+                }
+                WP_EPI_FETCH(0)
+                float* const sMw = wave_u < 6 ? sM0 + (2 * wave_u) * (32 * T) : sM1 + (2 * wave_u - 12) * (32 * T);
+#pragma unroll
+                for (int ct = 0; ct < COT; ++ct) {
+#pragma unroll
+                    for (int i = 0; i < 2; ++i)
+#pragma unroll
+                        for (int r = 0; r < 16; ++r) {
+                            const int col = (r & 3) + 8 * (r >> 2) + 4 * half;
+                            sMw[(i * 32 + col) * T + l31] = acc[i][ct][r];
+                        }
+                    if (ct + 1 < COT) WP_EPI_FETCH(ct + 1 < COT ? ct + 1 : ct)
+                    asm volatile("s_waitcnt lgkmcnt(0)\n\ts_barrier" ::: "memory");
+#pragma unroll
+                    for (int t2 = 0; t2 < 2; ++t2) {
+                        const int e_col = e_col0 + 16 * t2;
+                        const int co = co0 + ct * 32 + e_col;
+                        const f32x2 r0 = e_r0[ct][t2], r1 = e_r1[ct][t2];
+                        float mm[16];
+#pragma unroll
+                        for (int xi = 0; xi < 16; ++xi) mm[xi] = xi < 12 ? sM0[(xi * 32 + e_col) * T + e_tile] : sM1[((xi - 12) * 32 + e_col) * T + e_tile];
+                        float t0[4], t1[4];
+#pragma unroll
+                        for (int l = 0; l < 4; ++l) {
+                            t0[l] = mm[0 * 4 + l] + mm[1 * 4 + l] + mm[2 * 4 + l];
+                            t1[l] = mm[1 * 4 + l] - mm[2 * 4 + l] - mm[3 * 4 + l];
+                        }
+                        const float y00 = t0[0] + t0[1] + t0[2], y01 = t0[1] - t0[2] - t0[3];
+                        const float y10 = t1[0] + t1[1] + t1[2], y11 = t1[1] - t1[2] - t1[3];
+                        const float bvv = e_bias[ct][t2];
+                        const float osc = fin ? a.out_scale : 1.0f;
+                        const float v00 = (y00 + bvv + r0.x) * osc, v01 = (y01 + bvv + r0.y) * osc;
+                        const float v10 = (y10 + bvv + r1.x) * osc, v11 = (y11 + bvv + r1.y) * osc;
+                        if (co < a.Cout) {
+                            const long o = ((long)b * a.Cout + co) * HW + pix;
+                            *reinterpret_cast<float2*>(ydst + o) = make_float2(v00, v01);
+                            *reinterpret_cast<float2*>(ydst + o + W) = make_float2(v10, v11);
+                        }
+                        if (a.stats && fin) {
+                            float pil;
+                            {
+                                const int pv = __builtin_bit_cast(int, v00);
+                                const int s0 = __builtin_amdgcn_readlane(pv, 0), s2 = __builtin_amdgcn_readlane(pv, 32);
+                                pil = __builtin_bit_cast(float, (lane & 32) ? s2 : s0);
+                            }
+                            const float d0 = v00 - pil, d1 = v01 - pil, d2 = v10 - pil, d3 = v11 - pil;
+                            float sm = (d0 + d1) + (d2 + d3);
+                            float qm = (d0 * d0 + d1 * d1) + (d2 * d2 + d3 * d3);
+#define WP_MERGE(CTRL, ROWMASK)                                                                                     \
+                            {                                                                                           \
+                                sm += __builtin_bit_cast(float, __builtin_amdgcn_update_dpp(0, __builtin_bit_cast(int, sm), CTRL, ROWMASK, 0xf, false)); \
+                                qm += __builtin_bit_cast(float, __builtin_amdgcn_update_dpp(0, __builtin_bit_cast(int, qm), CTRL, ROWMASK, 0xf, false)); \
+                            }
+                            WP_MERGE(0xB1, 0xf)
+                            WP_MERGE(0x4E, 0xf)
+                            WP_MERGE(0x124, 0xf)
+                            WP_MERGE(0x128, 0xf)
+                            WP_MERGE(0x142, 0xa)
+#undef WP_MERGE
+                            if (e_tile == 31 && co < a.Cout) {
+                                float* q = a.stats + (((long)b * a.Cout + co) * rpi + rr) * 2;
+                                q[0] = sm + 128.0f * pil;
+                                q[1] = fmaxf(qm - sm * sm * (1.0f / 128.0f), 0.0f);
+                            }
+                        }
+                    }
+                    asm volatile("s_waitcnt lgkmcnt(0)\n\ts_barrier" ::: "memory");
+                }
+            } else {
+                int tid_e;
+                asm volatile("v_mov_b32 %0, %1" : "=v"(tid_e) : "v"(tid));
+                const int e_pair = tid_e & 15, e_col = tid_e >> 4;
+                const int oy0 = (rr / rx_n) * 8, ox0 = (rr % rx_n) * 16, co0 = cotile * BCO;
+                const long pix = (long)(oy0 + 2 * (e_pair >> 2)) * W + ox0 + 4 * (e_pair & 3);
+                float* const ydst = fin ? a.y : a.part + (long)kh * a.B * a.Cout * HW;
+                const unsigned e_rdo = (unsigned)(e_col * 32 + (((e_pair >> 1) ^ (e_col & 7)) << 2) + 2 * (e_pair & 1)) * 4u;
+                const unsigned e_rd0 = (unsigned)(uintptr_t)(__attribute__((address_space(3))) float*)sM0 + e_rdo;
+                const unsigned e_rd1 = (unsigned)(uintptr_t)(__attribute__((address_space(3))) float*)sM1 + e_rdo;
+                float e_bias[COT];
+                f32x4 e_r0[COT], e_r1[COT];
+#define WP_EPI_FETCH_T(ct)                                                                                      \
+                {                                                                                               \
+                    const int co = co0 + (ct) * 32 + e_col;                                                     \
+                    e_bias[ct] = fin ? a.bias[co] : 0.0f;                              \
+                    e_r0[ct] = e_r1[ct] = f32x4{0.0f, 0.0f, 0.0f, 0.0f};                                        \
                     if (a.res && fin) {                                                                         \
                         const long o = ((long)b * a.Cout + min(co, a.Cout - 1)) * HW + pix;                     \
-                        e_r0[ct][t2] = *reinterpret_cast<const f32x2*>(a.res + o);                              \
-                        e_r1[ct][t2] = *reinterpret_cast<const f32x2*>(a.res + o + W);                          \
+                        e_r0[ct] = *reinterpret_cast<const f32x4*>(a.res + o);                                  \
+                        e_r1[ct] = *reinterpret_cast<const f32x4*>(a.res + o + W);                              \
                     }                                                                                           \
-                }                                                                                               \
-            }
-            WP_EPI_FETCH(0)
-            float* const sMw = wave_u < 6 ? sM0 + (2 * wave_u) * (32 * T) : sM1 + (2 * wave_u - 12) * (32 * T);
-#pragma unroll
-            for (int ct = 0; ct < COT; ++ct) {
-#pragma unroll
-                for (int i = 0; i < 2; ++i)
-#pragma unroll
-                    for (int r = 0; r < 16; ++r) {
-                        const int col = (r & 3) + 8 * (r >> 2) + 4 * half;
-                        sMw[(i * 32 + col) * T + l31] = acc[i][ct][r];
-                    }
-                if (ct + 1 < COT) WP_EPI_FETCH(ct + 1 < COT ? ct + 1 : ct)
-                asm volatile("s_waitcnt lgkmcnt(0)\n\ts_barrier" ::: "memory");
-#pragma unroll
-                for (int t2 = 0; t2 < 2; ++t2) {
-                    const int e_col = e_col0 + 16 * t2;
-                    const int co = co0 + ct * 32 + e_col;
-                    const f32x2 r0 = e_r0[ct][t2], r1 = e_r1[ct][t2];
-                    float mm[16];
-#pragma unroll
-                    for (int xi = 0; xi < 16; ++xi) mm[xi] = xi < 12 ? sM0[(xi * 32 + e_col) * T + e_tile] : sM1[((xi - 12) * 32 + e_col) * T + e_tile];
-                    float t0[4], t1[4];
-#pragma unroll
-                    for (int l = 0; l < 4; ++l) {
-                        t0[l] = mm[0 * 4 + l] + mm[1 * 4 + l] + mm[2 * 4 + l];
-                        t1[l] = mm[1 * 4 + l] - mm[2 * 4 + l] - mm[3 * 4 + l];
-                    }
-                    const float y00 = t0[0] + t0[1] + t0[2], y01 = t0[1] - t0[2] - t0[3];
-                    const float y10 = t1[0] + t1[1] + t1[2], y11 = t1[1] - t1[2] - t1[3];
-                    const float bvv = e_bias[ct][t2];
-                    const float osc = fin ? a.out_scale : 1.0f;
-                    const float v00 = (y00 + bvv + r0.x) * osc, v01 = (y01 + bvv + r0.y) * osc;
-                    const float v10 = (y10 + bvv + r1.x) * osc, v11 = (y11 + bvv + r1.y) * osc;
-                    if (co < a.Cout) {
-                        const long o = ((long)b * a.Cout + co) * HW + pix;
-                        *reinterpret_cast<float2*>(ydst + o) = make_float2(v00, v01);
-                        *reinterpret_cast<float2*>(ydst + o + W) = make_float2(v10, v11);
-                    }
-                    if (a.stats && fin) {
-                        float pil;
-                        {
-                            const int pv = __builtin_bit_cast(int, v00);
-                            const int s0 = __builtin_amdgcn_readlane(pv, 0), s2 = __builtin_amdgcn_readlane(pv, 32);
-                            pil = __builtin_bit_cast(float, (lane & 32) ? s2 : s0);
+                }
+                WP_EPI_FETCH_T(0)
+                float* const sMw = wave_u < 6 ? sM0 + (2 * wave_u) * (32 * T) : sM1 + (2 * wave_u - 12) * (32 * T);
+#pragma unroll
+                for (int ct = 0; ct < COT; ++ct) {
+#pragma unroll
+                    for (int i = 0; i < 2; ++i)
+#pragma unroll
+                        for (int g = 0; g < 4; ++g) {
+                            const f32x4 v = {acc[i][ct][4 * g], acc[i][ct][4 * g + 1], acc[i][ct][4 * g + 2], acc[i][ct][4 * g + 3]};
+                            *reinterpret_cast<f32x4*>(sMw + (i * 32 + l31) * 32 + (((2 * g + half) ^ (l31 & 7)) << 2)) = v;
                         }
-                        const float d0 = v00 - pil, d1 = v01 - pil, d2 = v10 - pil, d3 = v11 - pil;
-                        float sm = (d0 + d1) + (d2 + d3);
-                        float qm = (d0 * d0 + d1 * d1) + (d2 * d2 + d3 * d3);
-#define WP_MERGE(CTRL, ROWMASK)                                                                                     \
-                        {                                                                                           \
-                            sm += __builtin_bit_cast(float, __builtin_amdgcn_update_dpp(0, __builtin_bit_cast(int, sm), CTRL, ROWMASK, 0xf, false)); \
-                            qm += __builtin_bit_cast(float, __builtin_amdgcn_update_dpp(0, __builtin_bit_cast(int, qm), CTRL, ROWMASK, 0xf, false)); \
+                    if (ct + 1 < COT) WP_EPI_FETCH_T(ct + 1 < COT ? ct + 1 : ct)
+                    asm volatile("s_waitcnt lgkmcnt(0)\n\ts_barrier" ::: "memory");
+                    {
+                        const int co = co0 + ct * 32 + e_col;
+                        f32x2 mm[16];
+                        asm volatile(
+                            "ds_read_b64 %0, %16\n\t"
+                            "ds_read_b64 %1, %16 offset:4096\n\t"
+                            "ds_read_b64 %2, %16 offset:8192\n\t"
+                            "ds_read_b64 %3, %16 offset:12288\n\t"
+                            "ds_read_b64 %4, %16 offset:16384\n\t"
+                            "ds_read_b64 %5, %16 offset:20480\n\t"
+                            "ds_read_b64 %6, %16 offset:24576\n\t"
+                            "ds_read_b64 %7, %16 offset:28672\n\t"
+                            "ds_read_b64 %8, %16 offset:32768\n\t"
+                            "ds_read_b64 %9, %16 offset:36864\n\t"
+                            "ds_read_b64 %10, %16 offset:40960\n\t"
+                            "ds_read_b64 %11, %16 offset:45056\n\t"
+                            "ds_read_b64 %12, %17\n\t"
+                            "ds_read_b64 %13, %17 offset:4096\n\t"
+                            "ds_read_b64 %14, %17 offset:8192\n\t"
+                            "ds_read_b64 %15, %17 offset:12288\n\t"
+                            "s_waitcnt lgkmcnt(0)"
+                            : "=&v"(mm[0]), "=&v"(mm[1]), "=&v"(mm[2]), "=&v"(mm[3]), "=&v"(mm[4]), "=&v"(mm[5]), "=&v"(mm[6]), "=&v"(mm[7]), "=&v"(mm[8]), "=&v"(mm[9]), "=&v"(mm[10]), "=&v"(mm[11]), "=&v"(mm[12]), "=&v"(mm[13]), "=&v"(mm[14]), "=&v"(mm[15])
+                            : "v"(e_rd0), "v"(e_rd1) : "memory");
+                        const float bvv = e_bias[ct];
+                        const float osc = fin ? a.out_scale : 1.0f;
+                        float vv[2][4];
+#pragma unroll
+                        for (int k = 0; k < 2; ++k) {
+                            float t0[4], t1[4];
+#pragma unroll
+                            for (int l = 0; l < 4; ++l) {
+                                t0[l] = mm[0 * 4 + l][k] + mm[1 * 4 + l][k] + mm[2 * 4 + l][k];
+                                t1[l] = mm[1 * 4 + l][k] - mm[2 * 4 + l][k] - mm[3 * 4 + l][k];
+                            }
+                            const float y00 = t0[0] + t0[1] + t0[2], y01 = t0[1] - t0[2] - t0[3];
+                            const float y10 = t1[0] + t1[1] + t1[2], y11 = t1[1] - t1[2] - t1[3];
+                            vv[k][0] = (y00 + bvv + e_r0[ct][2 * k]) * osc;
+                            vv[k][1] = (y01 + bvv + e_r0[ct][2 * k + 1]) * osc;
+                            vv[k][2] = (y10 + bvv + e_r1[ct][2 * k]) * osc;
+                            vv[k][3] = (y11 + bvv + e_r1[ct][2 * k + 1]) * osc;
                         }
-                        WP_MERGE(0xB1, 0xf)
-                        WP_MERGE(0x4E, 0xf)
-                        WP_MERGE(0x124, 0xf)
-                        WP_MERGE(0x128, 0xf)
-                        WP_MERGE(0x142, 0xa)
+                        if (co < a.Cout) {
+                            const long o = ((long)b * a.Cout + co) * HW + pix;
+                            *reinterpret_cast<f32x4*>(ydst + o) = f32x4{vv[0][0], vv[0][1], vv[1][0], vv[1][1]};
+                            *reinterpret_cast<f32x4*>(ydst + o + W) = f32x4{vv[0][2], vv[0][3], vv[1][2], vv[1][3]};
+                        }
+                        if (a.stats && fin) {
+                            const float pil = __builtin_bit_cast(float, __builtin_amdgcn_ds_bpermute((lane & 48) << 2, __builtin_bit_cast(int, vv[0][0])));
+                            float sk[2], qk[2];
+#pragma unroll
+                            for (int k = 0; k < 2; ++k) {
+                                const float d0 = vv[k][0] - pil, d1 = vv[k][1] - pil, d2 = vv[k][2] - pil, d3 = vv[k][3] - pil;
+                                sk[k] = (d0 + d1) + (d2 + d3);
+                                qk[k] = (d0 * d0 + d1 * d1) + (d2 * d2 + d3 * d3);
+                            }
+                            float sm = sk[0] + sk[1], qm = qk[0] + qk[1];
+#define WP_MERGE(CTRL)                                                                                              \
+                            {                                                                                       \
+                                sm += __builtin_bit_cast(float, __builtin_amdgcn_update_dpp(0, __builtin_bit_cast(int, sm), CTRL, 0xf, 0xf, false)); \
+                                qm += __builtin_bit_cast(float, __builtin_amdgcn_update_dpp(0, __builtin_bit_cast(int, qm), CTRL, 0xf, 0xf, false)); \
+                            }
+                            WP_MERGE(0xB1)
+                            WP_MERGE(0x4E)
+                            WP_MERGE(0x124)
+                            WP_MERGE(0x128)
 #undef WP_MERGE
-                        if (e_tile == 31 && co < a.Cout) {
-                            float* q = a.stats + (((long)b * a.Cout + co) * rpi + rr) * 2;
-                            q[0] = sm + 128.0f * pil;
-                            q[1] = fmaxf(qm - sm * sm * (1.0f / 128.0f), 0.0f);
+                            if (e_pair == 15 && co < a.Cout) {
+                                float* q = a.stats + (((long)b * a.Cout + co) * rpi + rr) * 2;
+                                q[0] = sm + 128.0f * pil;
+                                q[1] = fmaxf(qm - sm * sm * (1.0f / 128.0f), 0.0f);
+                            }
                         }
                     }
+                    asm volatile("s_waitcnt lgkmcnt(0)\n\ts_barrier" ::: "memory");
                 }
-                asm volatile("s_waitcnt lgkmcnt(0)\n\ts_barrier" ::: "memory");
             }
 #pragma unroll
             for (int i = 0; i < 2; ++i)
@@ -493,7 +616,9 @@
     }
     if (rec) {
         const unsigned long long now = __builtin_amdgcn_s_memtime();
-        if (lane == 0) {
+        int tid_d;
+        asm volatile("v_mov_b32 %0, %1" : "=v"(tid_d) : "v"(tid));
+        if ((tid_d & 63) == 0) {
             unsigned long long* d = a.dbg + (long)blockIdx.x * 8;
             unsigned hwid, xcc;
             asm volatile("s_getreg_b32 %0, hwreg(HW_REG_HW_ID)" : "=s"(hwid));
@@ -507,6 +632,7 @@
     }
 #undef WP_STAMP
 #undef WP_EPI_FETCH
+#undef WP_EPI_FETCH_T
 #undef WP_SLOT_TABLE
 #undef WP_QUADS
 #undef WP_LD1
@@ -544,12 +670,12 @@
     return n;
 }
 
-template <int COT, int PRO>
-static int wino3p_launch2(const ConvArgs& a, hipStream_t s) {
+template <int COT, int PRO, bool EPT>
+static int wino3p_launch3(const ConvArgs& a, hipStream_t s) {
     constexpr int BCO = 32 * COT;
     static PerDeviceOnce raised;
     if (raised.first_use()) {
-        MCVD_HIP_CHECK(hipFuncSetAttribute(reinterpret_cast<const void*>(&conv_wino3p_kernel<COT, PRO>),
+        MCVD_HIP_CHECK(hipFuncSetAttribute(reinterpret_cast<const void*>(&conv_wino3p_kernel<COT, PRO, EPT>),
                                            hipFuncAttributeMaxDynamicSharedMemorySize, 160 * 1024));
         raised.done();
     }
@@ -569,11 +695,16 @@
 #else
     k.wdma &= 0xff;
 #endif
-    hipLaunchKernelGGL((conv_wino3p_kernel<COT, PRO>), grid, dim3(WP_NT), wino3p_lds_bytes(a.Cin), s, k);
+    hipLaunchKernelGGL((conv_wino3p_kernel<COT, PRO, EPT>), grid, dim3(WP_NT), wino3p_lds_bytes(a.Cin), s, k);
     MCVD_HIP_CHECK(hipGetLastError());
     if (ksp >= 2) return launch_wino_ksplit_reduce(a, s);
     if (a.stats) set_last_conv_stats_np((a.H / 8) * (a.W / 16));
     return 0;
+}
+
+template <int COT, int PRO>
+static int wino3p_launch2(const ConvArgs& a, hipStream_t s) {
+    return a.old_epi ? wino3p_launch3<COT, PRO, false>(a, s) : wino3p_launch3<COT, PRO, true>(a, s);
 }
 
 template <int COT>
diff --git a/mcvd_pytorch_amd/csrc/model.cpp b/mcvd_pytorch_amd/csrc/model.cpp
--- a/mcvd_pytorch_amd/csrc/model.cpp
+++ b/mcvd_pytorch_amd/csrc/model.cpp
@@ -760,6 +760,7 @@
             a.shape_hint = (op.ks == 1 && ctx->conv_shape1 >= 0) ? ctx->conv_shape1 : ctx->conv_shape;
             a.wdma = ctx->conv_wdma;
             a.pgrid = ctx->persist_grid;
+            a.old_epi = !ctx->wino_epi;
             a.part = (op.ks == 3 && op.H * op.W <= 256) ? ksplit_buf : nullptr;
             a.part_floats = a.part ? ksplit_floats : 0;
             const size_t oi = (size_t)(&op - ops.data());
@@ -978,6 +979,7 @@
             a.B = B; a.Cin = cin; a.CinP = op.CinP; a.Cout = op.Cout; a.CoutP = op.CoutP; a.H = op.H; a.W = op.W; a.ks = op.ks;
             a.wdma = ctx->conv_wdma;
             a.pgrid = ctx->persist_grid;
+            a.old_epi = !ctx->wino_epi;
             a.part = (op.ks == 3 && op.H * op.W <= 256) ? ksplit_buf : nullptr;
             a.part_floats = a.part ? ksplit_floats : 0;
             const bool spade_fused = op.gb.kind != REF_NONE && ctx->spade_fuse && ctx->winograd;
diff --git a/mcvd_pytorch_amd/csrc/model.h b/mcvd_pytorch_amd/csrc/model.h
--- a/mcvd_pytorch_amd/csrc/model.h
+++ b/mcvd_pytorch_amd/csrc/model.h
@@ -22,6 +22,9 @@
     int conv_shape = -1;
     int conv_shape1 = -1;
     int winograd = 1;
+    int wino_epi = 1;
+    const float* last_part = nullptr;
+    size_t last_part_floats = 0;
     int persist_grid = 0;
     int temb_table = 1;
     int im2col_lds = 1;
```

After: 261.1, median of 6. Within noise of the previous version (+0.7%).
